# ATTron/astroz

Hardware: AMD Instinct MI355X
Metric: propagations/sec, 13,478 sats x 1,440 times, at 1/2/4/8 MI355X (higher is better)
Workload: dtype f64

## Files before the change

astroz_amd/_native.py:

```python
import ctypes as C
import os

import numpy as np

_HERE = os.path.dirname(os.path.abspath(__file__))
LIB_PATH = os.environ.get("ASTROZ_AMD_LIB") or os.path.join(_HERE, "libastroz_hip.so")

WGS84, WGS72 = 0, 1
OUT_TEME, OUT_ECEF, OUT_GEODETIC, OUT_TOPOCENTRIC = 0, 1, 2, 3
SAT_MAJOR, TIME_MAJOR = 0, 1
OUTPUT_MODES = {"teme": OUT_TEME, "ecef": OUT_ECEF, "geodetic": OUT_GEODETIC, "topocentric": OUT_TOPOCENTRIC}
PASS_DTYPE = np.dtype([("t_rise_min", "<f8"), ("t_culm_min", "<f8"), ("t_set_min", "<f8"), ("max_elevation_rad", "<f8"),
                       ("rise_azimuth_rad", "<f8"), ("set_azimuth_rad", "<f8"), ("flags", "<u4"), ("grid_rise", "<u4"),
                       ("grid_culm", "<u4"), ("grid_set", "<u4")])
PASS_UP_AT_START, PASS_UP_AT_END, PASS_CUT_BY_ERROR = 1, 2, 4
ECLIPSE_DTYPE = np.dtype([("t_entry_min", "<f8"), ("t_exit_min", "<f8"), ("flags", "<u4"), ("grid_entry", "<u4"),
                          ("grid_exit", "<u4"), ("reserved", "<u4")])
ECLIPSE_IN_AT_START, ECLIPSE_IN_AT_END, ECLIPSE_CUT_BY_ERROR = 1, 2, 4
SHADOW_UMBRA, SHADOW_PENUMBRA = 0, 1
SHADOW_KINDS = {"umbra": SHADOW_UMBRA, "penumbra": SHADOW_PENUMBRA}
ACCESS_DTYPE = np.dtype([("t_start_min", "<f8"), ("t_end_min", "<f8"), ("min_range_km", "<f8"), ("flags", "<u4"),
                         ("grid_start", "<u4"), ("grid_end", "<u4"), ("grid_min_range", "<u4")])
ACCESS_OPEN_AT_START, ACCESS_OPEN_AT_END, ACCESS_CUT_BY_ERROR = 1, 2, 4
CONJUNCTION_DTYPE = np.dtype([("t_tca_min", "<f8"), ("miss_km", "<f8"), ("rel_speed_km_s", "<f8"), ("target", "<u4"),
                              ("sat", "<u4"), ("grid_index", "<u4"), ("reserved", "<u4")])

COVERAGE_DTYPE = np.dtype([("mean_in_view", "<f8"), ("max_gap_min", "<f8"), ("n_covered", "<u4"), ("min_in_view", "<u4"),
                           ("max_in_view", "<u4"), ("n_gaps", "<u4"), ("grid_gap_start", "<u4"), ("grid_gap_end", "<u4"),
                           ("flags", "<u4"), ("reserved", "<u4")])
COVERAGE_GAP_AT_START, COVERAGE_GAP_AT_END = 1, 2

AZ_ERR_HIP = -200
PATH_ROWS_FAST, PATH_TILES_FAST, PATH_ROWS_GENERIC, PATH_LANE_SAT, PATH_DEEP_ROWS, PATH_QUASI_UNIFORM, PATH_COLS_FAST, PATH_HOST_STEP = 1, 2, 4, 8, 16, 32, 64, 128

EXPORTS = [
    "astroz_version", "astroz_init", "astroz_deinit", "tle_parse", "tle_free",
    "tle_get_satellite_number", "tle_get_epoch", "tle_get_inclination", "tle_get_eccentricity",
    "tle_get_mean_motion", "sgp4_init", "sgp4_free", "sgp4_propagate", "sgp4_propagate_batch",
    "azh_device_count", "azh_last_error", "azh_parse_tle_lines", "azh_constellation_from_tle_text",
    "azh_constellation_from_tle_lines", "azh_constellation_from_elements", "azh_constellation_subset", "azh_constellation_free",
    "azh_num_satellites", "azh_num_sgp4", "azh_num_sdp4", "azh_get_epochs", "azh_get_status",
    "azh_get_field", "azh_propagate_host", "azh_propagate_device", "azh_propagate_device_cached", "azh_propagate_device_window",
    "azh_propagate_jd_host", "azh_synchronize", "azh_propagate_one_host", "azh_set_time_tile", "azh_set_timing", "azh_set_fast_path", "azh_set_tile_kernel", "azh_set_graphs", "azh_set_f32_arithmetic", "azh_set_f32_mode",
    "azh_last_kernel_ms", "azh_last_path", "azh_last_one_stats", "azh_set_host_copy_threads", "azh_set_host_points", "azh_get_host_points", "azh_selftest_coords", "azh_selftest_host_step", "azh_host_alloc", "azh_host_free", "azh_host_pool_stats", "azh_host_pool_trim", "azh_propagate_device_f32", "azh_propagate_device_cached_f32",
    "azh_screen_target_host", "azh_screen_target_device", "azh_coarse_screen_device", "azh_coarse_screen_host",
    "azh_screen_all_host", "azh_constellation_from_omm_json", "azh_propagate_one_device", "azh_selftest_math",
    "azh_parse_tle_text", "azh_parse_omm_json", "azh_set_parse_threads", "coords_julian_to_gmst",
    "azh_group_create_from_tle_text", "azh_group_create_from_omm_json", "azh_group_free", "azh_group_num_satellites",
    "azh_group_num_devices", "azh_group_padded_rows", "azh_group_get_epochs", "azh_group_propagate_host",
    "azh_group_propagate_allgather", "azh_group_screen_target_host", "azh_group_screen_target_device", "azh_group_shard_size",
    "azh_group_shard_rows", "azh_group_synchronize", "azh_screen_track_device", "coords_eci_to_ecef", "coords_ecef_to_geodetic",
    "orbital_hohmann", "orbital_velocity", "orbital_period", "orbital_escape_velocity",
    "azh_coords_topocentric", "azh_set_observer", "azh_find_passes_host", "azh_find_passes_device",
    "azh_find_passes_stations_host", "azh_find_passes_stations_device",
    "azh_coverage_host", "azh_coverage_device",
    "azh_sun_position_teme", "azh_selftest_sun", "azh_shadow_state", "azh_find_eclipses_host", "azh_find_eclipses_device",
    "azh_line_of_sight", "azh_find_access_host", "azh_find_access_device", "azh_find_access_track_device",
    "azh_closest_approach", "azh_find_conjunctions_host", "azh_find_conjunctions_device",
]


def _stations(stations, min_elevation_deg):
    st = np.ascontiguousarray(stations, dtype=np.float64).reshape(-1, 3)
    mk = np.ascontiguousarray(np.broadcast_to(np.asarray(min_elevation_deg, dtype=np.float64), (len(st),)))
    return st, mk


def _targets(targets):
    a = np.atleast_1d(np.asarray(targets))
    if a.ndim != 1 or a.size == 0 or a.dtype == np.bool_ or not np.issubdtype(a.dtype, np.integer) or (a < 0).any():
        raise ValueError("targets must be a satellite index or a non-empty sequence of them")
    return np.ascontiguousarray(a, dtype=np.uintp)


def _min_satellites(k):
    if isinstance(k, bool) or not isinstance(k, (int, np.integer)) or not 1 <= int(k) <= 0xFFFFFFFF:
        raise ValueError("min_satellites must be an integer >= 1")
    return int(k)


class NativeError(RuntimeError):
    def __init__(self, code, what):
        self.code = code
        super().__init__("%s failed with code %d%s" % (what, code, _detail(code)))


_lib = None


def _detail(code):
    if _lib is not None and code == AZ_ERR_HIP:
        msg = _lib.azh_last_error().decode(errors="replace")
        return " (%s)" % msg if msg else " (HIP runtime error: is an MI355X visible?)"
    return ""


def _share_hip_runtime_with_torch():
    if os.environ.get("ASTROZ_AMD_SYSTEM_HIP"):
        return
    import importlib.util
    try:
        spec = importlib.util.find_spec("torch")
    except (ImportError, ValueError):
        spec = None
    if spec is None or not spec.origin:
        return
    cand = os.path.join(os.path.dirname(spec.origin), "lib", "libamdhip64.so")
    if os.path.exists(cand):
        C.CDLL(cand, mode=C.RTLD_GLOBAL)


def lib():
    global _lib
    if _lib is not None:
        return _lib
    if not os.path.exists(LIB_PATH):
        raise ImportError(
            "astroz_amd: %s not found -- build it with `python -c 'import __graft_entry__ as g; "
            "g.build()'` (hipcc --offload-arch=gfx950). There is no CPU fallback." % LIB_PATH)
    _share_hip_runtime_with_torch()
    L = C.CDLL(LIB_PATH)
    vp, sz, dbl, i32, u32 = C.c_void_p, C.c_size_t, C.c_double, C.c_int32, C.c_uint32
    L.astroz_version.restype = u32
    L.tle_parse.argtypes = [C.c_char_p, C.POINTER(vp)]
    L.tle_parse.restype = i32
    L.tle_free.argtypes = [vp]
    L.tle_get_satellite_number.argtypes = [vp]
    L.tle_get_satellite_number.restype = u32
    for f in ("tle_get_epoch", "tle_get_inclination", "tle_get_eccentricity", "tle_get_mean_motion"):
        getattr(L, f).argtypes = [vp]
        getattr(L, f).restype = dbl
    L.sgp4_init.argtypes = [vp, i32, C.POINTER(vp)]
    L.sgp4_init.restype = i32
    L.sgp4_free.argtypes = [vp]
    L.sgp4_propagate.argtypes = [vp, dbl, vp, vp]
    L.sgp4_propagate.restype = i32
    L.sgp4_propagate_batch.argtypes = [vp, vp, vp, u32]
    L.sgp4_propagate_batch.restype = i32
    L.azh_device_count.restype = C.c_int
    L.azh_last_error.restype = C.c_char_p
    L.azh_parse_tle_lines.argtypes = [C.c_char_p, C.c_char_p, vp]
    L.azh_parse_tle_lines.restype = i32
    L.azh_constellation_from_tle_text.argtypes = [C.c_char_p, sz, i32, i32, C.POINTER(vp)]
    L.azh_constellation_from_tle_text.restype = i32
    for f in ("azh_parse_tle_text", "azh_parse_omm_json"):
        getattr(L, f).argtypes = [C.c_char_p, sz, vp, sz, C.POINTER(sz)]
        getattr(L, f).restype = i32
    L.azh_set_parse_threads.argtypes = [i32]
    L.azh_set_parse_threads.restype = None
    for f in ("azh_group_create_from_tle_text", "azh_group_create_from_omm_json"):
        getattr(L, f).argtypes = [C.c_char_p, sz, i32, vp, i32, i32, C.POINTER(vp)]
        getattr(L, f).restype = i32
    L.azh_group_free.argtypes = [vp]
    L.azh_group_num_satellites.argtypes = [vp]
    L.azh_group_num_satellites.restype = sz
    L.azh_group_num_devices.argtypes = [vp]
    L.azh_group_num_devices.restype = i32
    L.azh_group_padded_rows.argtypes = [vp]
    L.azh_group_padded_rows.restype = sz
    L.azh_group_get_epochs.argtypes = [vp, vp]
    L.azh_group_get_epochs.restype = i32
    L.azh_group_propagate_host.argtypes = [vp, vp, sz, vp, sz, vp, vp, i32, dbl, vp]
    L.azh_group_propagate_host.restype = i32
    L.azh_group_propagate_allgather.argtypes = [vp, vp, sz, vp, sz, vp, vp]
    L.azh_group_propagate_allgather.restype = i32
    L.azh_group_screen_target_host.argtypes = [vp, vp, sz, vp, sz, sz, dbl, dbl, vp, vp]
    L.azh_group_screen_target_host.restype = i32
    L.azh_group_screen_target_device.argtypes = [vp, vp, sz, vp, sz, sz, dbl, dbl, vp, vp]
    L.azh_group_screen_target_device.restype = i32
    L.azh_group_shard_size.argtypes = [vp, i32]
    L.azh_group_shard_size.restype = sz
    L.azh_group_shard_rows.argtypes = [vp, i32, vp]
    L.azh_group_shard_rows.restype = i32
    L.azh_group_synchronize.argtypes = [vp]
    L.azh_group_synchronize.restype = i32
    L.azh_constellation_from_omm_json.argtypes = [C.c_char_p, sz, i32, i32, C.POINTER(vp)]
    L.azh_constellation_from_omm_json.restype = i32
    L.azh_propagate_one_device.argtypes = [vp, sz, vp, sz, vp, vp, vp, vp]
    L.azh_propagate_one_device.restype = i32
    L.azh_selftest_math.argtypes = [vp, sz, vp, i32]
    L.azh_selftest_math.restype = i32
    L.coords_julian_to_gmst.argtypes = [dbl]
    L.coords_julian_to_gmst.restype = dbl
    L.coords_eci_to_ecef.argtypes = [vp, dbl, vp]
    L.coords_eci_to_ecef.restype = None
    L.coords_ecef_to_geodetic.argtypes = [vp, vp]
    L.coords_ecef_to_geodetic.restype = None
    L.azh_constellation_from_tle_lines.argtypes = [vp, vp, sz, i32, i32, C.POINTER(vp)]
    L.azh_constellation_from_tle_lines.restype = i32
    L.azh_constellation_from_elements.argtypes = [sz] + [vp] * 8 + [i32, i32, C.POINTER(vp)]
    L.azh_constellation_from_elements.restype = i32
    L.azh_constellation_subset.argtypes = [vp, vp, sz, i32, C.POINTER(vp)]
    L.azh_constellation_subset.restype = i32
    L.azh_constellation_free.argtypes = [vp]
    for f in ("azh_num_satellites", "azh_num_sgp4", "azh_num_sdp4"):
        getattr(L, f).argtypes = [vp]
        getattr(L, f).restype = sz
    L.azh_get_epochs.argtypes = [vp, vp]
    L.azh_get_epochs.restype = i32
    L.azh_get_status.argtypes = [vp, vp, vp, vp]
    L.azh_get_status.restype = i32
    L.azh_get_field.argtypes = [vp, C.c_char_p, vp]
    L.azh_get_field.restype = i32
    L.azh_propagate_host.argtypes = [vp, vp, sz, vp, vp, vp, i32, dbl, vp, i32, sz, vp]
    L.azh_propagate_host.restype = i32
    L.azh_propagate_device.argtypes = [vp, vp, sz, vp, vp, vp, i32, dbl, vp, i32, sz, vp, vp]
    L.azh_propagate_device.restype = i32
    L.azh_propagate_device_cached.argtypes = [vp, vp, vp, i32, sz, vp, vp]
    L.azh_propagate_device_cached.restype = i32
    L.azh_propagate_device_window.argtypes = [vp, sz, sz, vp, vp, i32, sz, vp, vp]
    L.azh_propagate_device_window.restype = i32
    L.azh_propagate_jd_host.argtypes = [vp, vp, vp, sz, vp, vp, i32, i32, vp]
    L.azh_propagate_jd_host.restype = i32
    L.azh_synchronize.argtypes = [vp]
    L.azh_synchronize.restype = i32
    L.azh_propagate_one_host.argtypes = [vp, sz, vp, sz, vp, vp, vp]
    L.azh_propagate_one_host.restype = i32
    L.azh_set_time_tile.argtypes = [vp, u32, u32]
    L.azh_set_time_tile.restype = i32
    L.azh_set_timing.argtypes = [vp, i32]
    L.azh_set_timing.restype = i32
    L.azh_set_fast_path.argtypes = [vp, i32]
    L.azh_set_fast_path.restype = i32
    L.azh_set_tile_kernel.argtypes = [vp, i32]
    L.azh_set_tile_kernel.restype = i32
    L.azh_set_graphs.argtypes = [vp, i32]
    L.azh_set_graphs.restype = i32
    L.azh_set_f32_arithmetic.argtypes = [vp, i32]
    L.azh_set_f32_arithmetic.restype = i32
    L.azh_set_f32_mode.argtypes = [vp, i32]
    L.azh_set_f32_mode.restype = i32
    L.azh_last_kernel_ms.argtypes = [vp]
    L.azh_last_kernel_ms.restype = dbl
    L.azh_set_host_copy_threads.argtypes = [i32]
    L.azh_set_host_copy_threads.restype = None
    L.azh_set_host_points.argtypes = [sz]
    L.azh_set_host_points.restype = None
    L.azh_get_host_points.argtypes = []
    L.azh_get_host_points.restype = sz
    L.azh_host_alloc.argtypes = [C.c_size_t, C.POINTER(C.c_void_p)]
    L.azh_host_alloc.restype = i32
    L.azh_host_free.argtypes = [C.c_void_p]
    L.azh_host_free.restype = None
    L.azh_host_pool_stats.argtypes = [C.POINTER(C.c_size_t), C.POINTER(C.c_size_t)]
    L.azh_host_pool_stats.restype = None
    L.azh_host_pool_trim.argtypes = []
    L.azh_host_pool_trim.restype = None
    L.azh_last_path.argtypes = [vp]
    L.azh_last_path.restype = u32
    L.azh_last_one_stats.argtypes = [vp, vp, vp]
    L.azh_last_one_stats.restype = C.c_int32
    L.azh_propagate_device_f32.argtypes = L.azh_propagate_device.argtypes
    L.azh_propagate_device_f32.restype = i32
    L.azh_propagate_device_cached_f32.argtypes = L.azh_propagate_device_cached.argtypes
    L.azh_propagate_device_cached_f32.restype = i32
    L.azh_screen_target_host.argtypes = [vp, vp, sz, vp, sz, dbl, dbl, vp, vp]
    L.azh_screen_target_host.restype = i32
    L.azh_screen_target_device.argtypes = [vp, vp, sz, vp, sz, dbl, dbl, vp, vp, vp]
    L.azh_screen_target_device.restype = i32
    L.azh_screen_track_device.argtypes = [vp, vp, sz, vp, vp, sz, dbl, vp, vp, vp]
    L.azh_screen_track_device.restype = i32
    L.azh_coarse_screen_device.argtypes = [vp, sz, sz, i32, sz, dbl, vp, vp, vp, sz, C.POINTER(sz), vp]
    L.azh_coarse_screen_device.restype = i32
    L.azh_coarse_screen_host.argtypes = [vp, sz, sz, i32, sz, dbl, vp, vp, vp, sz, C.POINTER(sz), i32]
    L.azh_coarse_screen_host.restype = i32
    L.azh_screen_all_host.argtypes = [vp, vp, sz, vp, dbl, vp, vp, sz, C.POINTER(sz)]
    L.azh_screen_all_host.restype = i32
    L.azh_coords_topocentric.argtypes = [vp, vp, dbl, vp, vp, vp]
    L.azh_coords_topocentric.restype = None
    L.azh_set_observer.argtypes = [vp, dbl, dbl, dbl]
    L.azh_set_observer.restype = i32
    L.azh_find_passes_host.argtypes = [vp, vp, sz, vp, dbl, dbl, vp, sz, vp]
    L.azh_find_passes_host.restype = i32
    L.azh_find_passes_device.argtypes = [vp, vp, sz, vp, dbl, dbl, vp, sz, vp, vp]
    L.azh_find_passes_device.restype = i32
    L.azh_find_passes_stations_host.argtypes = [vp, vp, sz, vp, dbl, vp, vp, sz, vp, sz, vp]
    L.azh_find_passes_stations_host.restype = i32
    L.azh_find_passes_stations_device.argtypes = [vp, vp, sz, vp, dbl, vp, vp, sz, vp, sz, vp, vp]
    L.azh_find_passes_stations_device.restype = i32
    L.azh_coverage_host.argtypes = [vp, vp, sz, vp, dbl, vp, vp, sz, u32, vp, vp]
    L.azh_coverage_host.restype = i32
    L.azh_coverage_device.argtypes = [vp, vp, sz, vp, dbl, vp, vp, sz, u32, vp, vp, vp]
    L.azh_coverage_device.restype = i32
    L.azh_sun_position_teme.argtypes = [dbl, vp]
    L.azh_sun_position_teme.restype = None
    L.azh_selftest_sun.argtypes = [vp, sz, vp, i32]
    L.azh_selftest_sun.restype = i32
    L.azh_shadow_state.argtypes = [vp, vp, vp, vp]
    L.azh_shadow_state.restype = i32
    L.azh_find_eclipses_host.argtypes = [vp, vp, sz, vp, dbl, i32, vp, sz, vp, vp]
    L.azh_find_eclipses_host.restype = i32
    L.azh_find_eclipses_device.argtypes = [vp, vp, sz, vp, dbl, i32, vp, sz, vp, vp, vp]
    L.azh_find_eclipses_device.restype = i32
    L.azh_line_of_sight.argtypes = [vp, vp, dbl, vp, vp]
    L.azh_line_of_sight.restype = i32
    L.azh_find_access_host.argtypes = [vp, vp, sz, vp, sz, dbl, dbl, vp, sz, vp, vp]
    L.azh_find_access_host.restype = i32
    L.azh_find_access_device.argtypes = [vp, vp, sz, vp, sz, dbl, dbl, vp, sz, vp, vp, vp]
    L.azh_find_access_device.restype = i32
    L.azh_find_access_track_device.argtypes = [vp, vp, sz, vp, vp, vp, sz, dbl, dbl, vp, sz, vp, vp, vp]
    L.azh_find_access_track_device.restype = i32
    L.azh_closest_approach.argtypes = [vp, vp, vp, vp, dbl, vp, vp, vp]
    L.azh_closest_approach.restype = i32
    L.azh_find_conjunctions_host.argtypes = [vp, vp, sz, vp, vp, sz, dbl, vp, sz, vp]
    L.azh_find_conjunctions_host.restype = i32
    L.azh_find_conjunctions_device.argtypes = [vp, vp, sz, vp, vp, sz, dbl, vp, sz, vp, vp]
    L.azh_find_conjunctions_device.restype = i32
    L.orbital_hohmann.argtypes = [dbl, dbl, dbl, vp]
    L.orbital_hohmann.restype = i32
    for f, n in (("orbital_velocity", 3), ("orbital_period", 2), ("orbital_escape_velocity", 2)):
        getattr(L, f).argtypes = [dbl] * n
        getattr(L, f).restype = dbl
    _lib = L
    return L


def check(code, what):
    if code != 0:
        raise NativeError(code, what)


def _f64(a):
    return np.ascontiguousarray(a, dtype=np.float64)


def _ptr(a):
    return None if a is None else a.ctypes.data


class DeviceConstellation:

    def __init__(self, handle):
        self._h = handle
        L = lib()
        self.n = L.azh_num_satellites(handle)
        self.n_sgp4 = L.azh_num_sgp4(handle)
        self.n_sdp4 = L.azh_num_sdp4(handle)
        self._epochs = None
        self._status = None

    @classmethod
    def from_tle_text(cls, text, grav=WGS72, device=0):
        b = text.encode() if isinstance(text, str) else bytes(text)
        h = C.c_void_p()
        check(lib().azh_constellation_from_tle_text(b, len(b), grav, device, C.byref(h)),
              "azh_constellation_from_tle_text")
        return cls(h)

    @classmethod
    def from_omm_json(cls, text, grav=WGS72, device=0):
        b = text.encode() if isinstance(text, str) else bytes(text)
        h = C.c_void_p()
        check(lib().azh_constellation_from_omm_json(b, len(b), grav, device, C.byref(h)),
              "azh_constellation_from_omm_json")
        return cls(h)

    @classmethod
    def from_tle_lines(cls, pairs, grav=WGS72, device=0):
        n = len(pairs)
        a1 = (C.c_char_p * n)(*[p[0].encode() for p in pairs])
        a2 = (C.c_char_p * n)(*[p[1].encode() for p in pairs])
        h = C.c_void_p()
        check(lib().azh_constellation_from_tle_lines(a1, a2, n, grav, device, C.byref(h)),
              "azh_constellation_from_tle_lines")
        return cls(h)

    @classmethod
    def from_elements(cls, epoch_jd, mm_revday, ecc, incl_deg, raan_deg, argp_deg, ma_deg, bstar,
                      grav=WGS72, device=0):
        cols = [_f64(x) for x in (epoch_jd, mm_revday, ecc, incl_deg, raan_deg, argp_deg, ma_deg, bstar)]
        n = len(cols[0])
        assert all(len(c) == n for c in cols)
        h = C.c_void_p()
        check(lib().azh_constellation_from_elements(n, *[c.ctypes.data for c in cols], grav, device,
                                                    C.byref(h)), "azh_constellation_from_elements")
        return cls(h)

    def subset(self, indices, device=-1):
        idx = np.ascontiguousarray(indices, dtype=np.uint32)
        h = C.c_void_p()
        check(lib().azh_constellation_subset(self._h, idx.ctypes.data, len(idx), device, C.byref(h)),
              "azh_constellation_subset")
        return type(self)(h)

    def handle_address(self):
        return int(self._h.value)

    def close(self):
        if getattr(self, "_h", None):
            lib().azh_constellation_free(self._h)
            self._h = None

    def __del__(self):
        try:
            self.close()
        except Exception:
            pass

    @property
    def epochs(self):
        if self._epochs is None:
            e = np.empty(self.n, dtype=np.float64)
# ... 132 lines not shown
                                                    stream), "azh_find_passes_stations_device")

    def coverage(self, times_min, offsets_min, points, min_elevation_deg, *, reference_jd=0.0, min_satellites=1, counts=False):
        times = _f64(times_min)
        off = None if offsets_min is None else _f64(offsets_min)
        if off is not None and len(off) < self.n:
            raise ValueError("epoch_offsets must have at least num_satellites elements")
        pt, mk = _stations(points, min_elevation_deg)
        stats = np.zeros(len(pt), dtype=COVERAGE_DTYPE)
        cnt = np.zeros((len(pt), len(times)), dtype=np.uint32) if counts else None
        check(lib().azh_coverage_host(self._h, times.ctypes.data, len(times), _ptr(off), float(reference_jd), pt.ctypes.data,
                                      mk.ctypes.data, len(pt), _min_satellites(min_satellites), stats.ctypes.data,
                                      None if cnt is None else cnt.ctypes.data), "azh_coverage_host")
        return (stats, cnt) if counts else stats

    def coverage_device(self, times_min, offsets_min, points, min_elevation_deg, d_stats, d_counts=None, *, reference_jd=0.0,
                        min_satellites=1, stream=None):
        times = _f64(times_min)
        off = None if offsets_min is None else _f64(offsets_min)
        if off is not None and len(off) < self.n:
            raise ValueError("epoch_offsets must have at least num_satellites elements")
        pt, mk = _stations(points, min_elevation_deg)
        check(lib().azh_coverage_device(self._h, times.ctypes.data, len(times), _ptr(off), float(reference_jd), pt.ctypes.data,
                                        mk.ctypes.data, len(pt), _min_satellites(min_satellites), d_stats, d_counts, stream),
              "azh_coverage_device")

    def find_eclipses(self, times_min, offsets_min=None, *, reference_jd, kind=SHADOW_UMBRA, max_eclipses=32, state=False):
        times = _f64(times_min)
        off = None if offsets_min is None else _f64(offsets_min)
        if off is not None and len(off) < self.n:
            raise ValueError("epoch_offsets must have at least num_satellites elements")
        out = np.zeros((self.n, int(max_eclipses)), dtype=ECLIPSE_DTYPE)
        cnt = np.zeros(self.n, dtype=np.uint32)
        st = np.zeros((self.n, len(times)), dtype=np.uint8) if state else None
        check(lib().azh_find_eclipses_host(self._h, times.ctypes.data, len(times), _ptr(off), float(reference_jd), int(kind),
                                           out.ctypes.data if max_eclipses else None, int(max_eclipses), cnt.ctypes.data,
                                           st.ctypes.data if state and st.size else None), "azh_find_eclipses_host")
        return (out, cnt, st) if state else (out, cnt)

    def find_eclipses_device(self, times_min, offsets_min, d_out, max_eclipses, d_n_eclipses, *, reference_jd, kind=SHADOW_UMBRA,
                             d_state=None, stream=None):
        times = _f64(times_min)
        off = None if offsets_min is None else _f64(offsets_min)
        check(lib().azh_find_eclipses_device(self._h, times.ctypes.data, len(times), _ptr(off), float(reference_jd), int(kind),
                                             d_out, int(max_eclipses), d_n_eclipses, d_state, stream), "azh_find_eclipses_device")

    def find_access(self, times_min, target, offsets_min=None, *, grazing_alt_km=0.0, max_range_km=None, max_windows=32,
                    state=False):
        times = _f64(times_min)
        off = None if offsets_min is None else _f64(offsets_min)
        if off is not None and len(off) < self.n:
            raise ValueError("epoch_offsets must have at least num_satellites elements")
        out = np.zeros((self.n, int(max_windows)), dtype=ACCESS_DTYPE)
        cnt = np.zeros(self.n, dtype=np.uint32)
        st = np.zeros((self.n, len(times)), dtype=np.uint8) if state else None
        check(lib().azh_find_access_host(self._h, times.ctypes.data, len(times), _ptr(off), int(target), float(grazing_alt_km),
                                         _max_range(max_range_km), out.ctypes.data if max_windows else None, int(max_windows),
                                         cnt.ctypes.data, st.ctypes.data if state and st.size else None), "azh_find_access_host")
        return (out, cnt, st) if state else (out, cnt)

    def find_access_device(self, times_min, target, offsets_min, d_out, max_windows, d_n_windows, *, grazing_alt_km=0.0,
                           max_range_km=None, d_state=None, stream=None):
        times = _f64(times_min)
        off = None if offsets_min is None else _f64(offsets_min)
        check(lib().azh_find_access_device(self._h, times.ctypes.data, len(times), _ptr(off), int(target), float(grazing_alt_km),
                                           _max_range(max_range_km), d_out, int(max_windows), d_n_windows, d_state, stream),
              "azh_find_access_device")

    def find_access_track_device(self, times_min, d_track_pos, d_track_vel, offsets_min, d_out, max_windows, d_n_windows, *,
                                 exclude=None, grazing_alt_km=0.0, max_range_km=None, d_state=None, stream=None):
        times = _f64(times_min)
        off = None if offsets_min is None else _f64(offsets_min)
        ex = C.c_size_t(-1).value if exclude is None else int(exclude)
        check(lib().azh_find_access_track_device(self._h, times.ctypes.data, len(times), _ptr(off), d_track_pos, d_track_vel, ex,
                                                 float(grazing_alt_km), _max_range(max_range_km), d_out, int(max_windows),
                                                 d_n_windows, d_state, stream), "azh_find_access_track_device")

    def find_conjunctions(self, times_min, targets, threshold_km, offsets_min=None, *, max_events=65536):
        times = _f64(times_min)
        off = None if offsets_min is None else _f64(offsets_min)
        if off is not None and len(off) < self.n:
            raise ValueError("epoch_offsets must have at least num_satellites elements")
        tg = _targets(targets)
        out = np.zeros(int(max_events), dtype=CONJUNCTION_DTYPE)
        cnt = np.zeros(1, dtype=np.uint32)
        check(lib().azh_find_conjunctions_host(self._h, times.ctypes.data, len(times), _ptr(off), tg.ctypes.data, len(tg),
                                               float(threshold_km), out.ctypes.data if max_events else None, int(max_events),
                                               cnt.ctypes.data), "azh_find_conjunctions_host")
        return out[:min(int(cnt[0]), int(max_events))], int(cnt[0])

    def find_conjunctions_device(self, times_min, targets, threshold_km, offsets_min, d_out, max_events, d_n_events, *, stream=None):
        times = _f64(times_min)
        off = None if offsets_min is None else _f64(offsets_min)
        tg = _targets(targets)
        check(lib().azh_find_conjunctions_device(self._h, times.ctypes.data, len(times), _ptr(off), tg.ctypes.data, len(tg),
                                                 float(threshold_km), d_out, int(max_events), d_n_events, stream),
              "azh_find_conjunctions_device")

    def screen_all(self, times_min, threshold=10.0, offsets_min=None, max_results=10_000_000):
        times = _f64(times_min)
        off = None if offsets_min is None else _f64(offsets_min)
        pairs = np.empty((max_results, 2), dtype=np.uint32)
        tt = np.empty(max_results, dtype=np.uint32)
        k = C.c_size_t(0)
        check(lib().azh_screen_all_host(self._h, times.ctypes.data, len(times), _ptr(off), float(threshold),
                                        pairs.ctypes.data, tt.ctypes.data, max_results, C.byref(k)),
              "azh_screen_all_host")
        return pairs[:k.value].copy(), tt[:k.value].copy()

    def propagate_one(self, sat_index, tsince_min):
        t = _f64(np.atleast_1d(tsince_min))
        n = len(t)
        pos = result_empty((n, 3))
        vel = result_empty((n, 3))
        err = result_empty((n,), np.uint8)
        check(lib().azh_propagate_one_host(self._h, sat_index, t.ctypes.data, n, pos.ctypes.data, vel.ctypes.data,
                                           err.ctypes.data), "azh_propagate_one_host")
        return err, pos, vel

    def propagate_one_device(self, sat_index, d_tsince, n, d_pos, d_vel=None, d_err=None, stream=None):
        check(lib().azh_propagate_one_device(self._h, sat_index, d_tsince, n, d_pos, d_vel, d_err, stream),
              "azh_propagate_one_device")

    F32_MODES = {"mixed": 0, "packed": 1, "fp64": 2}

    def set_f32_arithmetic(self, mode):
        if isinstance(mode, (bool, np.bool_)):
            check(lib().azh_set_f32_arithmetic(self._h, 1 if mode else 0), "azh_set_f32_arithmetic")
            return
        m = self.F32_MODES[mode] if isinstance(mode, str) else int(mode)
        check(lib().azh_set_f32_mode(self._h, m), "azh_set_f32_mode")

    def set_fast_path(self, enabled):
        check(lib().azh_set_fast_path(self._h, 1 if enabled else 0), "azh_set_fast_path")

    def set_tile_kernel(self, enabled):
        check(lib().azh_set_tile_kernel(self._h, int(enabled) if not isinstance(enabled, bool) else (1 if enabled else 0)), "azh_set_tile_kernel")

    def set_graphs(self, enabled):
        check(lib().azh_set_graphs(self._h, 1 if enabled else 0), "azh_set_graphs")

    def set_timing(self, enabled):
        check(lib().azh_set_timing(self._h, 1 if enabled else 0), "azh_set_timing")

    def synchronize(self):
        check(lib().azh_synchronize(self._h), "azh_synchronize")

    def last_kernel_ms(self):
        return lib().azh_last_kernel_ms(self._h)

    def last_path(self):
        return int(lib().azh_last_path(self._h))

    def last_one_stats(self):
        a, b = C.c_uint32(0), C.c_uint32(0)
        check(lib().azh_last_one_stats(self._h, C.byref(a), C.byref(b)), "azh_last_one_stats")
        return int(a.value), int(b.value)


class DeviceGroup:

    def __init__(self, text, devices, grav=WGS72, n_chunks=4):
        b = text.encode() if isinstance(text, str) else bytes(text)
        dv = (C.c_int32 * len(devices))(*devices)
        h = C.c_void_p()
        fn = lib().azh_group_create_from_omm_json if b.lstrip()[:1] in (b"{", b"[") else lib().azh_group_create_from_tle_text
        check(fn(b, len(b), grav, dv, len(devices), n_chunks, C.byref(h)), "azh_group_create")
        self._h = h
        self.n = lib().azh_group_num_satellites(h)
        self.n_devices = lib().azh_group_num_devices(h)
        self.padded_rows = lib().azh_group_padded_rows(h)
        self.epochs = np.empty(self.n)
        check(lib().azh_group_get_epochs(h, self.epochs.ctypes.data), "azh_group_get_epochs")

    def close(self):
        if getattr(self, "_h", None):
            lib().azh_group_free(self._h)
            self._h = None

    def __del__(self):
        try:
            self.close()
        except Exception:
            pass

    def _offsets(self, offsets_min):
        if offsets_min is None:
            return None
        off = _f64(offsets_min)
        if off.ndim != 1 or len(off) < self.n:
            raise ValueError("epoch_offsets must have at least num_satellites elements")
        return off

    def propagate_host(self, times_min, offsets_min=None, *, velocities=True, mode=OUT_TEME, reference_jd=0.0, errors=False):
        t = _f64(times_min)
        off = self._offsets(offsets_min)
        pos = result_empty((self.n, len(t), 3))
        vel = result_empty((self.n, len(t), 3)) if velocities else None
        big = self.n * len(t) >= PINNED_MIN_BYTES
        err = (result_empty((self.n, len(t)), np.uint8) if big else np.zeros((self.n, len(t)), dtype=np.uint8)) if errors else None
        check(lib().azh_group_propagate_host(self._h, t.ctypes.data, len(t), _ptr(off), 0 if off is None else len(off), pos.ctypes.data, _ptr(vel), mode,
                                             float(reference_jd), _ptr(err)), "azh_group_propagate_host")
        return pos, vel, err

    def screen_target(self, times_min, target, threshold_km, offsets_min=None, reference_jd=0.0):
        t = _f64(times_min)
        off = self._offsets(offsets_min)
        d = np.empty(self.n)
        ti = np.empty(self.n, dtype=np.uint32)
        check(lib().azh_group_screen_target_host(self._h, t.ctypes.data, len(t), _ptr(off), 0 if off is None else len(off), int(target),
                                                 float(threshold_km), float(reference_jd), d.ctypes.data, ti.ctypes.data),
              "azh_group_screen_target_host")
        return d, ti

    def screen_target_device(self, times_min, target, threshold_km, d_dist_ptrs, d_t_ptrs, offsets_min=None):
        t = _f64(times_min)
        off = self._offsets(offsets_min)
        dd = (C.c_void_p * self.n_devices)(*d_dist_ptrs)
        tt = (C.c_void_p * self.n_devices)(*d_t_ptrs)
        check(lib().azh_group_screen_target_device(self._h, t.ctypes.data, len(t), _ptr(off), 0 if off is None else len(off), int(target),
                                                   float(threshold_km), 0.0, dd, tt), "azh_group_screen_target_device")

    def shard_size(self, slot):
        return int(lib().azh_group_shard_size(self._h, int(slot)))

    def shard_rows(self, slot):
        out = np.empty(self.shard_size(slot), dtype=np.uint32)
        check(lib().azh_group_shard_rows(self._h, int(slot), out.ctypes.data), "azh_group_shard_rows")
        return out

    def synchronize(self):
        check(lib().azh_group_synchronize(self._h), "azh_group_synchronize")

    def propagate_allgather(self, times_min, offsets_min, d_pos_ptrs, d_vel_ptrs=None):
        t = _f64(times_min)
        off = self._offsets(offsets_min)
        pp = (C.c_void_p * self.n_devices)(*d_pos_ptrs)
        vv = (C.c_void_p * self.n_devices)(*d_vel_ptrs) if d_vel_ptrs is not None else None
        check(lib().azh_group_propagate_allgather(self._h, t.ctypes.data, len(t), _ptr(off), 0 if off is None else len(off), pp, vv),
              "azh_group_propagate_allgather")


class _PinnedBlock:
    __slots__ = ("ptr", "_free", "__weakref__")

    def __init__(self, nbytes):
        self.ptr = None
        q = C.c_void_p(0)
        check(lib().azh_host_alloc(int(nbytes), C.byref(q)), "azh_host_alloc")
        self.ptr, self._free = q.value, lib().azh_host_free

    def __del__(self):
        if self.ptr:
            self._free(self.ptr)
            self.ptr = None


_PINNED_RESULTS = True
PINNED_MIN_BYTES = 8 << 20
_PINNED_LIVE_BUDGET = int(os.environ.get("ASTROZ_AMD_PINNED_LIVE_MB", "8192")) << 20


def set_pinned_budget(nbytes):
    global _PINNED_LIVE_BUDGET
    _PINNED_LIVE_BUDGET = max(0, int(nbytes))


def set_pinned_results(enabled):
    global _PINNED_RESULTS
    _PINNED_RESULTS = bool(enabled)


def result_empty(shape, dtype=np.float64, pinned=None):
    n = 1
    for d in shape:
        n *= int(d)
    if n * 8 < PINNED_MIN_BYTES and dtype is np.float64:
        return np.empty(shape)
    dt = np.dtype(dtype)
    nbytes = n * dt.itemsize
    use = _PINNED_RESULTS if pinned is None else pinned
    if not use or nbytes < PINNED_MIN_BYTES:
        return np.empty(shape, dtype=dt)
    if host_pool_stats()[0] + nbytes > _PINNED_LIVE_BUDGET:
        return np.empty(shape, dtype=dt)
    try:
        blk = _PinnedBlock(nbytes)
    except NativeError:
        return np.empty(shape, dtype=dt)
    buf = (C.c_char * nbytes).from_address(blk.ptr)
    buf._az_owner = blk
    return np.frombuffer(buf, dtype=dt).reshape(shape)


_fast_mod = False


def fast_scalar():
    global _fast_mod
    if _fast_mod is False:
        try:
            from . import _azfast
            _azfast.bind(C.cast(lib().azh_propagate_one_host, C.c_void_p).value)
            _fast_mod = _azfast
        except Exception:
            _fast_mod = None
# ... 156 lines not shown
```

astroz_amd/csrc/astroz_hip.hip:

```cpp
#include "../../include/astroz_hip.h"

#include <hip/hip_runtime.h>
#include <dlfcn.h>
#include <rccl/rccl.h>

#include <algorithm>
#include <atomic>
#include <cmath>
#include <condition_variable>
#include <deque>
#include <map>
#include <cstdio>
#include <cstdlib>
#include <cstring>
#include <mutex>
#include <new>
#include <memory>
#include <string>
#include <thread>
#include <type_traits>
#include <vector>

#include "kernels.h"
#include "passes_kernel.h"
// ... 20 lines not shown
}
#define HIP_TRY(expr)                                                                                       \
    do {                                                                                                    \
        if (!hip_ok((expr), #expr)) return AZ_ERR_HIP;                                                      \
    } while (0)

AzGrav make_grav(int which)
{
    AzGrav g;
    if (which == AZ_WGS72) {
        g.radius_km = 6378.135;
        g.j2 = 0.001082616;
        g.j4 = -0.00000165597;
        g.xke = 0.0743669161331734132;
        g.j3oj2 = -0.00234506972242078;
    } else {
        g.radius_km = 6378.137;
        g.j2 = 0.00108262998905;
        g.j4 = -0.00000161098761;
        g.xke = 0.07436685316871385;
        g.j3oj2 = -0.00233899967218727;
    }
    g.vkmpersec = g.xke * g.radius_km / 60.0;
    g.half_j2 = 0.5 * g.j2;
    return g;
}

const char *const kFieldNames[] = {
#define X(n) #n,
    AZ_SGP4_FIELDS(X) AZ_DEEP_FIELDS(X)
#undef X
};


template <class T>
struct DevBuf {
    T *p = nullptr;
    size_t cap = 0;
    DevBuf() = default;
    DevBuf(DevBuf &&o) noexcept { swap(o); }
    DevBuf &operator=(DevBuf &&o) noexcept { swap(o); return *this; }
    ~DevBuf() { if (p) (void)hipFree(p); }
    void swap(DevBuf &o) noexcept { std::swap(p, o.p); std::swap(cap, o.cap); }
    int ensure(size_t n)
    {
        if (n <= cap) return AZ_OK;
        if (p) (void)hipFree(p);
        p = nullptr;
        cap = 0;
        size_t want = std::max<size_t>(n, 64);
        if (!hip_ok(hipMalloc((void **)&p, want * sizeof(T)), "hipMalloc")) return AZ_ERR_HIP;
        cap = want;
        return AZ_OK;
    }
};

struct PinnedBuf {
    void *p = nullptr;
    size_t cap = 0;
    PinnedBuf() = default;
    PinnedBuf(PinnedBuf &&o) noexcept { swap(o); }
    PinnedBuf &operator=(PinnedBuf &&o) noexcept { swap(o); return *this; }
    ~PinnedBuf() { if (p) (void)hipHostFree(p); }
    void swap(PinnedBuf &o) noexcept { std::swap(p, o.p); std::swap(cap, o.cap); }
    int32_t ensure(size_t bytes)
    {
        if (bytes <= cap) return AZ_OK;
        size_t want = std::max<size_t>(cap, 65536);
        while (want < bytes) want *= 2;
        if (p) (void)hipHostFree(p);
        p = nullptr;
        cap = 0;
        if (!hip_ok(hipHostMalloc(&p, want, hipHostMallocDefault), "hipHostMalloc")) return AZ_ERR_HIP;
        cap = want;
        return AZ_OK;
    }
};

template <class H, hipError_t (*Create)(H *, unsigned), hipError_t (*Destroy)(H)>
class HipHandle {
  public:
    HipHandle() = default;
    HipHandle(HipHandle &&o) noexcept { swap(o); }
    HipHandle &operator=(HipHandle &&o) noexcept { swap(o); return *this; }
    ~HipHandle() { reset(); }
    void swap(HipHandle &o) noexcept { std::swap(h_, o.h_); std::swap(own_, o.own_); }
    hipError_t create(unsigned flags)
    {
        reset();
        own_ = true;
        return Create(&h_, flags);
    }
    void borrow(H h)
    {
        reset();
        h_ = h;
        own_ = false;
    }
    void reset()
    {
        if (h_ && own_) (void)Destroy(h_);
        h_ = nullptr;
    }
    bool owned() const { return h_ && own_; }
    operator H() const { return h_; }

  private:
    H h_ = nullptr;
    bool own_ = false;
};
using Stream = HipHandle<hipStream_t, hipStreamCreateWithFlags, hipStreamDestroy>;
using Event = HipHandle<hipEvent_t, hipEventCreateWithFlags, hipEventDestroy>;

constexpr int kStageSlots = 3;
constexpr size_t kStageChunk = size_t(16) << 20;
struct HostStager {
    Event ev[kStageSlots];
    PinnedBuf slot[kStageSlots];
    int32_t ensure()
    {
        for (int k = 0; k < kStageSlots; ++k) {
            if (slot[k].ensure(kStageChunk) != AZ_OK) return AZ_ERR_HIP;
            if (!ev[k] && !hip_ok(ev[k].create(hipEventDisableTiming), "hipEventCreate")) return AZ_ERR_HIP;
        }
        return AZ_OK;
    }
};
}

struct azh_constellation {
    int device = 0;
    size_t n = 0, n_pad = 0;
    AzGrav g{};
    Stream s_main, s_deep, s_ecc;
    Event ev_fork, ev_join, ev_fork2, ev_join2, ev_t0, ev_t1;
    Event ev_one;
    Event ev_graph;
    DevBuf<double> d_el;
    DevBuf<unsigned> d_flags;
    std::vector<unsigned> h_flags;
    std::vector<double> h_epoch;
    std::vector<double> h_raw[AZ_NUM_RAW];
    DevBuf<unsigned> d_list;
    std::vector<unsigned> h_list;
    unsigned n_sgp4 = 0, n_sdp4 = 0, n_bad = 0;
    DevBuf<double> d_times, d_offsets, d_sin, d_cos, d_seeds;
    DevBuf<double> d_node_cache;
    struct FastPlan {
        bool valid = false, mixed32 = false;
        unsigned tile_c = 0, tile_e = 0, n_list = 0, n_seg = 0, parity = 0;
        DevBuf<double> win;
        DevBuf<unsigned char> flag;
        DevBuf<unsigned> redo;
    } plan[4];
    DevBuf<double> d_inc;
    DevBuf<double> d_fast_rec;
    double uniform_step = 0.0;
    DevBuf<float> d_delta;
    double delta_max = 0.0;
    std::vector<float> h_delta;
    DevBuf<double> d_delta64;
    std::vector<double> h_delta64;
    bool delta_wide = false;
    double grid_t0 = 0.0;
    unsigned last_path = 0;
    DevBuf<double> d_tgt, d_part_d2, d_out_d;
    DevBuf<unsigned> d_part_t, d_out_t;
    DevBuf<double> d_one_t, d_one_o;
    DevBuf<unsigned char> d_one_e;
    DevBuf<unsigned> d_one_items;
    unsigned one_segments = 0;
    PinnedBuf h_stage;
    std::vector<double> h_times, h_offsets;
    std::vector<uint8_t> h_mask;
    double staged_ref_jd = 0.0;
    hipStream_t staged_stream = nullptr;
    bool staged_valid = false;
    PinnedBuf h_small;
    HostStager stager;
    bool seeds_valid = false;
    unsigned seeds_tile = 0;
    bool seeds_rows = false;
    DevBuf<unsigned char> d_mask;
    DevBuf<double> d_host_pos, d_host_vel;
    DevBuf<unsigned char> d_host_err;
    bool have_offsets = false, have_mask = false;
    AzObserver obs{};
    DevBuf<AzObserver> d_obs;
    bool have_observer = false, obs_dirty = false;
    DevBuf<double> d_pass_pos, d_pass_vel;
    DevBuf<unsigned char> d_pass_err;
    DevBuf<azh_pass> d_pass_out;
    DevBuf<uint32_t> d_pass_n;
    std::vector<AzStation> h_stations;
    DevBuf<AzStation> d_stations;
    DevBuf<azh_coverage> d_cov_stats;
    DevBuf<uint32_t> d_cov_counts;
    DevBuf<AzSunPoint> d_sun;
    DevBuf<azh_eclipse> d_ecl_out;
    DevBuf<unsigned char> d_ecl_state;
    DevBuf<double> d_acc_track;
    DevBuf<azh_access> d_acc_out;
    DevBuf<unsigned char> d_acc_state;
    DevBuf<double> d_conj_track;
    std::vector<unsigned> h_conj_slots;
    DevBuf<unsigned> d_conj_slots;
    DevBuf<azh_conjunction> d_conj_out;
    unsigned cached_n_times = 0;
    int cached_mode = 0;
    unsigned off_cat = 0;
    unsigned off_deep_cat = 0;
    unsigned off_rowmap = 0;
    unsigned off_rowmap2 = 0;
    struct LaunchGraph {
        const void *pos, *vel, *err;
        int layout, f32;
        size_t stride, row_lo, row_hi;
        hipStream_t st;
        unsigned sig_before, sig_after;
        unsigned path;
        unsigned seen;
        unsigned fails;
        hipGraph_t graph;
        hipGraphExec_t exec;
    };
    std::vector<LaunchGraph> graphs;
    int graphs_on = 0;
    bool capturing = false;
    int cols_kernel = 0;
    DevBuf<double> d_deep_tmp;
    bool tile_kernel = true;
    unsigned off_circ = 0, n_circ = 0;
    bool timed = false;
    bool timing = true;
    unsigned tile_sgp4 = 0, tile_sdp4 = 0;
    int f32_mode = 0;
    bool fast_path = true;
    std::vector<double> h_el;
    std::vector<std::pair<size_t, std::vector<double>>> h_cols;
    size_t h_cols_next = 0;
    ~azh_constellation();
};

namespace {

constexpr size_t kHostMirrorPad = 64;
constexpr size_t kHostCols = 256;
constexpr size_t kHostColsBeforeTable = 8;
constexpr size_t kHostTableMax = size_t(64) << 20;
std::atomic<size_t> g_host_points{[] {
    const char *e = getenv("ASTROZ_AMD_HOST_POINTS");
    return e ? (size_t)strtoull(e, nullptr, 10) : size_t(128);
}()};
inline size_t host_points() { return azhost::cpu_ok() ? g_host_points.load(std::memory_order_relaxed) : 0; }

constexpr int32_t AZ_RC_EAGER = 0x7a5eca9;
int set_device(const azh_constellation *c) { return hip_ok(hipSetDevice(c->device), "hipSetDevice") ? AZ_OK : AZ_ERR_HIP; }

hipStream_t small_stream(int device)
{
    static std::mutex mu;
    static std::map<int, hipStream_t> streams;
    std::lock_guard<std::mutex> lk(mu);
    auto it = streams.find(device);
    if (it != streams.end()) return it->second;
    hipStream_t s = nullptr;
    if (!hip_ok(hipStreamCreateWithFlags(&s, hipStreamNonBlocking), "hipStreamCreate")) return nullptr;
    streams[device] = s;
    return s;
}

void drop_graphs(azh_constellation *c);

int32_t build(const std::vector<double> (&cols)[AZ_NUM_RAW], size_t n, int grav, int device, azh_constellation **out)
{
    if (!out) return AZ_ERR_NULL_POINTER;
    *out = nullptr;
    if (n == 0) return AZ_ERR_VALUE;
    if (n > 0x7fffffffu) return AZ_ERR_VALUE;
    int ndev = 0;
    HIP_TRY(hipGetDeviceCount(&ndev));
    if (device < 0 || device >= ndev) {
        g_last_error = "no such HIP device";
        return AZ_ERR_HIP;
    }
    std::unique_ptr<azh_constellation> c(new (std::nothrow) azh_constellation());
    if (!c) return AZ_ERR_ALLOC_FAILED;
    c->device = device;
    c->n = n;
    c->n_pad = (n + 63) / 64 * 64;
    c->g = make_grav(grav);
    if (set_device(c.get()) != AZ_OK) return AZ_ERR_HIP;
    if (n > 16) {
        if (!hip_ok(c->s_main.create(hipStreamNonBlocking), "hipStreamCreate") ||
            !hip_ok(c->s_deep.create(hipStreamNonBlocking), "hipStreamCreate") ||
            !hip_ok(c->s_ecc.create(hipStreamNonBlocking), "hipStreamCreate") ||
            !hip_ok(c->ev_graph.create(hipEventDisableTiming | hipEventDisableSystemFence), "hipEventCreate"))
            return AZ_ERR_HIP;
    } else {
        c->s_main.borrow(small_stream(device));
        if (!c->s_main) return AZ_ERR_HIP;
        c->s_deep.borrow(c->s_main);
        c->s_ecc.borrow(c->s_main);
    }
    for (Event *e : {&c->ev_fork2, &c->ev_join2, &c->ev_fork, &c->ev_join, &c->ev_one})
        if (!hip_ok(e->create(hipEventDisableTiming), "hipEventCreate")) return AZ_ERR_HIP;
    if (!hip_ok(c->ev_t0.create(hipEventDefault), "hipEventCreate") || !hip_ok(c->ev_t1.create(hipEventDefault), "hipEventCreate"))
        return AZ_ERR_HIP;
    const size_t np = c->n_pad;
    DevBuf<double> d_raw;
    if (c->d_el.ensure((size_t)AZ_NUM_FIELDS * np) != AZ_OK || c->d_flags.ensure(np) != AZ_OK || d_raw.ensure((size_t)AZ_NUM_RAW * np) != AZ_OK)
        return AZ_ERR_HIP;
    std::vector<double> staging((size_t)AZ_NUM_RAW * np, 0.0);
    for (int k = 0; k < AZ_NUM_RAW; ++k) memcpy(&staging[(size_t)k * np], cols[k].data(), sizeof(double) * n);
    if (!hip_ok(hipMemcpyAsync(d_raw.p, staging.data(), sizeof(double) * staging.size(), hipMemcpyHostToDevice, c->s_main), "H2D raw") ||
        !hip_ok(hipMemsetAsync(c->d_el.p, 0, sizeof(double) * AZ_NUM_FIELDS * np, c->s_main), "memset el") ||
        !hip_ok(hipMemsetAsync(c->d_flags.p, 0, sizeof(unsigned) * np, c->s_main), "memset flags"))
        return AZ_ERR_HIP;
    hipLaunchKernelGGL(k_init, dim3((unsigned)(np / 64)), dim3(64), 0, c->s_main, d_raw.p, n, np, c->g, c->d_el.p, c->d_flags.p);
    if (!hip_ok(hipGetLastError(), "k_init launch")) return AZ_ERR_HIP;
    c->h_flags.resize(n);
    if (np <= kHostMirrorPad) {
        c->h_el.resize((size_t)AZ_NUM_FIELDS * np);
        if (!hip_ok(hipMemcpyAsync(c->h_el.data(), c->d_el.p, sizeof(double) * c->h_el.size(), hipMemcpyDeviceToHost, c->s_main), "D2H el"))
            return AZ_ERR_HIP;
    }
    if (!hip_ok(hipMemcpyAsync(c->h_flags.data(), c->d_flags.p, sizeof(unsigned) * n, hipMemcpyDeviceToHost, c->s_main), "D2H flags") ||
        !hip_ok(hipStreamSynchronize(c->s_main), "sync(init)"))
        return AZ_ERR_HIP;
    c->h_epoch = cols[R_epoch_jd];
    for (int k = 0; k < AZ_NUM_RAW; ++k) c->h_raw[k] = cols[k];
    std::vector<unsigned> list;
    list.reserve(n);
    for (size_t s = 0; s < n; ++s)
        if (AZ_FLAG_ERR(c->h_flags[s]) == 0 && !(c->h_flags[s] & AZ_FLAG_DEEP)) list.push_back((unsigned)s);
    c->n_sgp4 = (unsigned)list.size();
    for (size_t g0 = 0; g0 < list.size(); g0 += AZ_BLOCK) {
        const size_t g1 = std::min(g0 + (size_t)AZ_BLOCK, list.size());
        std::stable_sort(list.begin() + g0, list.begin() + g1, [&](unsigned x, unsigned y) {
            return AZ_FLAG_ECLASS(c->h_flags[x]) < AZ_FLAG_ECLASS(c->h_flags[y]);
        });
    }
    {
        std::vector<unsigned> deep;
        for (size_t s = 0; s < n; ++s)
            if (AZ_FLAG_ERR(c->h_flags[s]) == 0 && (c->h_flags[s] & AZ_FLAG_DEEP)) deep.push_back((unsigned)s);
        const std::vector<double> &incl = cols[R_incl_deg];
        auto key = [&](unsigned s) {
            const unsigned f = c->h_flags[s];
            const unsigned low = incl[s] < 12.5 ? 1u : 0u;
            return (AZ_FLAG_IREZ(f) << 4) | (low << 2) | AZ_FLAG_ECLASS(f);
        };
        std::stable_sort(deep.begin(), deep.end(), [&](unsigned x, unsigned y) { return key(x) < key(y); });
        list.insert(list.end(), deep.begin(), deep.end());
    }
    c->n_sdp4 = (unsigned)list.size() - c->n_sgp4;
    for (size_t s = 0; s < n; ++s)
        if (AZ_FLAG_ERR(c->h_flags[s]) != 0) list.push_back((unsigned)s);
    c->n_bad = (unsigned)list.size() - c->n_sgp4 - c->n_sdp4;
    c->off_circ = (unsigned)list.size();
    for (size_t s = 0; s < n; ++s)
        if (AZ_FLAG_ERR(c->h_flags[s]) == 0 && !(c->h_flags[s] & AZ_FLAG_DEEP) && AZ_FLAG_ECLASS(c->h_flags[s]) == 0)
            list.push_back((unsigned)s);
    c->n_circ = (unsigned)list.size() - c->off_circ;
    for (size_t s = 0; s < n; ++s)
        if (AZ_FLAG_ERR(c->h_flags[s]) == 0 && !(c->h_flags[s] & AZ_FLAG_DEEP) && AZ_FLAG_ECLASS(c->h_flags[s]) != 0)
            list.push_back((unsigned)s);
    c->off_cat = (unsigned)list.size();
    for (size_t s = 0; s < n; ++s)
        if (AZ_FLAG_ERR(c->h_flags[s]) == 0 && !(c->h_flags[s] & AZ_FLAG_DEEP)) list.push_back((unsigned)s);
    c->off_deep_cat = (unsigned)list.size();
    for (size_t s = 0; s < n; ++s)
        if (AZ_FLAG_ERR(c->h_flags[s]) == 0 && (c->h_flags[s] & AZ_FLAG_DEEP)) list.push_back((unsigned)s);
    c->off_rowmap = (unsigned)list.size();
    {
        unsigned near = 0, deepn = 0;
        for (size_t s = 0; s < n; ++s) {
            const unsigned f = c->h_flags[s];
            if (AZ_FLAG_ERR(f) != 0) list.push_back((unsigned)AZ_ROW_ZERO << 30);
            else if (f & AZ_FLAG_DEEP) list.push_back(((unsigned)AZ_ROW_COPY << 30) | deepn++);
            else list.push_back(((unsigned)AZ_ROW_NEAR << 30) | near++);
        }
    }
    c->off_rowmap2 = (unsigned)list.size();
    {
        unsigned circ = 0, eccn = 0, deepn = 0;
        for (size_t s = 0; s < n; ++s) {
            const unsigned f = c->h_flags[s];
            if (AZ_FLAG_ERR(f) != 0) list.push_back((unsigned)AZ_ROW_ZERO << 30);
            else if (f & AZ_FLAG_DEEP) list.push_back(((unsigned)AZ_ROW_COPY << 30) | deepn++);
            else if (AZ_FLAG_ECLASS(f) == 0) list.push_back(((unsigned)AZ_ROW_NEAR << 30) | circ++);
            else list.push_back(((unsigned)AZ_ROW_NEAR << 30) | (c->n_circ + eccn++));
        }
    }
    if (const char *e = getenv("ASTROZ_AMD_COLS")) c->cols_kernel = atoi(e);
    if (const char *e = getenv("ASTROZ_AMD_GRAPHS")) c->graphs_on = atoi(e);
    c->h_list = list;
    if (c->d_list.ensure(list.size()) != AZ_OK ||
        !hip_ok(hipMemcpy(c->d_list.p, list.data(), sizeof(unsigned) * list.size(), hipMemcpyHostToDevice), "H2D list"))
        return AZ_ERR_HIP;
    *out = c.release();
    return AZ_OK;
}

int32_t build_from_records(const std::vector<azh::TleRecord> &recs, int grav, int device, azh_constellation **out)
{
    std::vector<double> cols[AZ_NUM_RAW];
    for (auto &v : cols) v.resize(recs.size());
    azh::parallel_ranges(recs.size(), azh::parse_threads_for(recs.size() * 140), [&](size_t a, size_t b) {
        for (size_t i = a; i < b; ++i) {
            const azh::TleRecord &r = recs[i];
            cols[R_epoch_jd][i] = r.epoch_jd;
            cols[R_mm_revday][i] = r.mm_revday;
            cols[R_ecc][i] = r.ecc;
            cols[R_incl_deg][i] = r.incl_deg;
            cols[R_raan_deg][i] = r.raan_deg;
            cols[R_argp_deg][i] = r.argp_deg;
            cols[R_ma_deg][i] = r.ma_deg;
            cols[R_bstar][i] = r.bstar;
        }
    });
    return build(cols, recs.size(), grav, device, out);
}

unsigned auto_tile(unsigned n_list, unsigned n_times, unsigned forced, unsigned min_tile)
{
    if (forced) return std::min(std::max(forced, 1u), std::max(n_times, 1u));
    const unsigned waves_x = (n_list + 63) / 64;
    unsigned n_tiles = (16384 + waves_x - 1) / std::max(waves_x, 1u);
    n_tiles = std::max(1u, std::min(n_tiles, n_times));
    unsigned tile = (n_times + n_tiles - 1) / n_tiles;
    tile = std::max(tile, std::min(min_tile, n_times));
    return std::max(tile, 1u);
}

inline unsigned pad8(unsigned n) { return (n + 7) / 8 * 8; }
inline unsigned cgrid_y(unsigned n_times, unsigned tile) { return (n_times + tile - 1) / tile; }

template <int V>
using int_c = std::integral_constant<int, V>;
template <class F>
void with_bool(bool b, F &&f)
{
    if (b) f(std::true_type{});
    else f(std::false_type{});
}
template <class F>
void with_vel_frame(bool vel, int mode, F &&f)
{
    const int frame = mode == AZ_OUT_TOPOCENTRIC ? 3 : (mode == AZ_OUT_GEODETIC ? 2 : (mode != AZ_OUT_TEME ? 1 : 0));
    with_bool(vel, [&](auto VEL) {
        if (frame == 3) f(VEL, int_c<3>{});
        else if (frame == 2) f(VEL, int_c<2>{});
        else if (frame == 1) f(VEL, int_c<1>{});
        else f(VEL, int_c<0>{});
    });
}
constexpr int gen_frame(int frame) { return frame == 3 ? 3 : (frame != 0 ? 1 : 0); }
template <class F>
void with_outputs(const PropArgs &a, bool vel, F &&f)
{
    if (a.screen_target) return f(std::false_type{}, int_c<0>{}, int_c<AZ_SINK_SCREEN>{});
    with_vel_frame(vel, a.mode, [&](auto VEL, auto FRAME) {
        if (a.f32) f(VEL, FRAME, int_c<AZ_SINK_F32>{});
        else f(VEL, FRAME, int_c<AZ_SINK_F64>{});
    });
}
template <class F>
void with_delta(int form, F &&f)
{
    if (form == 2) f(int_c<2>{});
    else if (form == 1) f(int_c<1>{});
    else f(int_c<0>{});
}

int32_t stream_after(hipStream_t to, hipStream_t from, hipEvent_t ev)
{
    HIP_TRY(hipEventRecord(ev, from));
    HIP_TRY(hipStreamWaitEvent(to, ev, 0));
    return AZ_OK;
}

unsigned rows_tile(unsigned n_list, unsigned n_times, unsigned forced)
{
    unsigned segs = std::max(1u, std::min((16384u + n_list - 1) / std::max(n_list, 1u), (n_times + 255) / 256));
    if (forced) segs = std::max(1u, (n_times + forced - 1) / forced);
    return ((n_times + segs - 1) / segs + 63) / 64 * 64;
}

bool use_rows(const PropArgs &a, int layout, bool deep)
{
    if (deep && layout == AZ_LAYOUT_TIME_MAJOR && a.n_times >= 32) return true;
    return (layout == AZ_LAYOUT_SAT_MAJOR || a.screen_target) && a.n_times >= 32;
}

unsigned screen_parts(const PropArgs &a, bool deep)
{
    if (use_rows(a, AZ_LAYOUT_SAT_MAJOR, deep)) {
        unsigned tile = rows_tile(a.n_list, a.n_times, a.tile_forced);
        if (deep) tile = std::min(tile, 64u * (unsigned)AZ_DEEP_SEED_MAX);
        return cgrid_y(a.n_times, tile);
    }
    return cgrid_y(a.n_times, a.tile);
}

struct EccSide {
    hipStream_t stream = nullptr;
    hipEvent_t fork = nullptr, join = nullptr;
};

struct FastShape {
    unsigned tile_c = 0, tile_e = 0;
    bool packed32 = false;
    bool mixed32 = false;
    int kind = 0;
};
unsigned fast_window_cap(double step)
{
    const double span = 3000.0 / std::max(std::fabs(step), 1e-9);
    return span >= 4.0e9 ? 0xffffffc0u : std::max(64u, (unsigned)span / 64u * 64u);
}
FastShape fast_shape_rows(const PropArgs &a, unsigned n_sgp4, unsigned n_circ)
{
    FastShape f;
    const unsigned cap = fast_window_cap(a.uniform_step);
    const unsigned n_ecc = n_sgp4 - n_circ;
    f.tile_c = std::min(rows_tile(n_sgp4, a.n_times, a.tile_forced), cap);
    f.tile_e = n_circ >= 4u * n_ecc ? f.tile_c : std::min(rows_tile(std::max(n_ecc, 1u), a.n_times, 256), cap);
    if (a.delta || a.delta64) {
        f.tile_c = std::min(f.tile_c, (unsigned)AZ_DELTA_SEG);
        f.tile_e = std::min(f.tile_e, (unsigned)AZ_DELTA_SEG);
    }
    f.packed32 = a.f32 && a.mode == AZ_OUT_TEME && a.arith32 != 2 && cap >= 128u && !a.delta_wide;
    f.mixed32 = f.packed32 && a.arith32 == 0;
    if (f.packed32) f.tile_c = std::max(128u, f.tile_c / 128u * 128u);
    f.kind = f.packed32 ? 1 : 0;
    return f;
}
FastShape fast_shape_tiles(const PropArgs &a, unsigned n_rows)
{
    FastShape f;
    unsigned tile = std::min(rows_tile(std::max((n_rows + 15u) / 16u, 1u) * 16u, a.n_times, a.tile_forced), fast_window_cap(a.uniform_step));
    if (a.mode != AZ_OUT_TEME) tile = std::min(tile, (unsigned)AZ_TILE_SEG_MAX);
    if (a.delta || a.delta64) tile = std::min(tile, (unsigned)AZ_DELTA_SEG);
    f.tile_c = f.tile_e = tile;
    f.kind = 2;
    return f;
}

template <bool VEL, int FRAME, int SINK, bool ECC>
void launch_rows_fast(const PropArgs &a, unsigned n_slots, hipStream_t st)
{
    with_delta(a.delta_wide ? 2 : (a.delta ? 1 : 0), [&](auto DELTA) {
        hipLaunchKernelGGL((k_rows_fast<VEL, FRAME, SINK, ECC, DELTA>), dim3(pad8(n_slots), cgrid_y(a.n_times, a.tile)), dim3(64), 0, st, a);
    });
}
PropArgs ecc_part(const PropArgs &a, unsigned tile)
{
    PropArgs e = a;
    e.list = a.list + a.n_circ;
    e.n_list = a.n_list - a.n_circ;
    e.tile = tile;
    e.redo_slot0 = a.n_circ;
    return e;
}
template <bool VEL, int FRAME, int SINK>
void launch_redo(const PropArgs &a, dim3 grid, hipStream_t st)
{
    hipLaunchKernelGGL((k_rows<VEL, gen_frame(FRAME), SINK, true>), grid, dim3(64), 0, st, a);
}

int32_t launch_near_fast(const PropArgs &a, bool vel, const FastShape &shape, dim3 rgrid, hipStream_t st, const EccSide &side)
{
    PropArgs e = ecc_part(a, shape.tile_e), c = a;
    c.n_list = a.n_circ;
    c.tile = shape.tile_c;
    unsigned n_e = e.n_list, n_c = c.n_list;
    if (a.row_lo > 0 || a.row_hi < a.n_rows) {
        c.slot_lo = a.win_circ_lo; c.slot_hi = a.win_circ_hi; n_c = c.slot_hi - c.slot_lo;
        e.slot_lo = a.win_ecc_lo; e.slot_hi = a.win_ecc_hi; n_e = e.slot_hi - e.slot_lo;
        if (c.slot_hi == 0) c.n_list = n_c = 0;
        if (e.slot_hi == 0) e.n_list = n_e = 0;
    }
    const bool beside = side.stream != nullptr && n_c;
    const hipStream_t se = beside ? side.stream : st;
    if (beside)
        if (int32_t rc = stream_after(se, st, side.fork); rc != AZ_OK) return rc;
    with_outputs(a, vel, [&](auto VEL, auto FRAME, auto SINK) {
        if (n_e) launch_rows_fast<VEL, FRAME, SINK, true>(e, n_e, se);
        launch_redo<VEL, FRAME, SINK>(a, rgrid, se);
        if (n_c && FRAME == 0 && shape.packed32)
            with_bool(shape.mixed32, [&](auto MIXED) {
                with_bool(a.delta != nullptr, [&](auto DELTA) {
                    hipLaunchKernelGGL((k_rows_fast32<VEL, MIXED, DELTA>), dim3(pad8(n_c), cgrid_y(a.n_times, c.tile)), dim3(64), 0, st, c);
                });
            });
        else if (n_c)
            launch_rows_fast<VEL, FRAME, SINK, false>(c, n_c, st);
    });
    return beside ? stream_after(st, se, side.join) : AZ_OK;
}

void launch_tiles(const PropArgs &a0, bool vel, hipStream_t st, const FastShape &shape)
{
    PropArgs a = a0, r = a0;
    a.tile = r.tile = shape.tile_c;
    r.tm_rows = 1;
    const dim3 grid(pad8((a.n_rows + 15u) / 16u), cgrid_y(a.n_times, a.tile));
    with_vel_frame(vel, a.mode, [&](auto VEL, auto FRAME) {
        with_bool(a.delta64 != nullptr, [&](auto WIDE) {
            hipLaunchKernelGGL((k_tiles_fast<VEL, FRAME, WIDE ? 2 : 0>), grid, dim3(1024), 0, st, a);
        });
        launch_redo<VEL, FRAME, AZ_SINK_F64>(r, dim3(256, 4), st);
    });
}
unsigned cols_tile(unsigned n_rows, unsigned n_times, unsigned forced, double step)
{
    const unsigned cap = fast_window_cap(step);
    if (forced) return std::min(std::max(forced, 1u), std::min(std::max(n_times, 1u), cap));
    const unsigned groups = (n_rows + 63u) / 64u, places = 1024u * (unsigned)AZ_COLS_WAVES;
    const unsigned segs = std::max(1u, places / std::max(groups, 1u));
    unsigned tile = (n_times + segs - 1u) / segs;
    if (tile < 32u) tile = std::min(128u, std::max(n_times, 1u));
    return std::max(1u, std::min(tile, cap));
}
FastShape fast_shape_cols(const PropArgs &a, unsigned n_rows, unsigned n_sgp4, unsigned n_circ)
{
    FastShape f = fast_shape_rows(a, n_sgp4, n_circ);
    f.tile_e = std::min(rows_tile(std::max(n_sgp4 - n_circ, 1u), a.n_times, a.tile_forced ? a.tile_forced : 256u), fast_window_cap(a.uniform_step));
    if (a.delta || a.delta64) f.tile_e = std::min(f.tile_e, (unsigned)AZ_DELTA_SEG);
    f.tile_c = cols_tile(n_rows, a.n_times, a.tile_forced, a.uniform_step);
    f.packed32 = f.mixed32 = false;
    f.kind = 3;
    return f;
}
int32_t launch_cols(const PropArgs &a0, bool vel, hipStream_t st, const FastShape &shape, const EccSide &side, unsigned ecc_row0)
{
    PropArgs a = a0;
    PropArgs e = ecc_part(a, shape.tile_e);
    e.pos = const_cast<double *>(a.tmp_pos);
    e.vel = vel ? const_cast<double *>(a.tmp_vel) : nullptr;
    e.rows_compact = 1;
    e.ecc_row0 = ecc_row0;
    if (e.n_list) {
        const hipStream_t se = side.stream ? side.stream : st;
        if (se != st)
            if (int32_t rc = stream_after(se, st, side.fork); rc != AZ_OK) return rc;
        with_vel_frame(vel, a.mode, [&](auto VEL, auto FRAME) { launch_rows_fast<VEL, FRAME, AZ_SINK_F64, true>(e, e.n_list, se); });
        if (se != st)
            if (int32_t rc = stream_after(st, se, side.join); rc != AZ_OK) return rc;
    }
    a.tile = shape.tile_c;
    a.ecc_row0 = ecc_row0;
    PropArgs r = a;
    r.tm_rows = 1;
    const dim3 grid(pad8((a.n_rows + 63u) / 64u), cgrid_y(a.n_times, a.tile));
    with_vel_frame(vel, a.mode, [&](auto VEL, auto FRAME) {
        with_bool(a.delta64 != nullptr, [&](auto WIDE) {
            hipLaunchKernelGGL((k_cols_fast<VEL, FRAME, WIDE ? 2 : 0>), grid, dim3(64), 0, st, a);
        });
        launch_redo<VEL, FRAME, AZ_SINK_F64>(r, dim3(256, 4), st);
    });
    return AZ_OK;
}

unsigned launch_propagate(const PropArgs &a, int layout, bool vel, bool deep, hipStream_t st)
{
    if (use_rows(a, layout, deep)) {
        PropArgs b = a;
        b.tile = rows_tile(a.n_list, a.n_times, a.tile_forced);
        if (deep) b.tile = std::min(b.tile, 64u * (unsigned)AZ_DEEP_SEED_MAX);
        const unsigned n_slots = a.slot_hi ? a.slot_hi - a.slot_lo : a.n_list;
        const dim3 grid(pad8(n_slots), cgrid_y(a.n_times, b.tile));
        with_outputs(a, vel, [&](auto VEL, auto FRAME, auto SINK) {
            if (deep) hipLaunchKernelGGL((k_rows_deep<VEL, gen_frame(FRAME), SINK>), grid, dim3(64), 0, st, b);
            else hipLaunchKernelGGL((k_rows<VEL, gen_frame(FRAME), SINK>), grid, dim3(64), 0, st, b);
        });
        return deep ? AZH_PATH_DEEP_ROWS : AZH_PATH_ROWS_GENERIC;
    }
    const dim3 grid(pad8((a.n_list + AZ_BLOCK - 1) / AZ_BLOCK), cgrid_y(a.n_times, a.tile));
    with_bool(deep, [&](auto DEEP) {
        if (a.screen_target)
            hipLaunchKernelGGL((k_propagate<0, false, DEEP, 0, true>), grid, dim3(AZ_BLOCK), 0, st, a);
        else
            with_bool(layout == AZ_LAYOUT_TIME_MAJOR, [&](auto TIME_MAJOR) {
                with_vel_frame(vel, a.mode, [&](auto VEL, auto FRAME) {
                    hipLaunchKernelGGL((k_propagate<TIME_MAJOR, VEL, DEEP, gen_frame(FRAME)>), grid, dim3(AZ_BLOCK), 0, st, a);
                });
            });
    });
    return AZH_PATH_LANE_SAT;
}

int32_t stage_inputs(azh_constellation *c, const double *times, size_t n_times, const double *offsets,
                     const uint8_t *mask, int mode, double reference_jd, hipStream_t st)
{
    if (n_times > 0xffffffffu) return AZ_ERR_VALUE;
    {
        const bool same = c->staged_valid && st == c->staged_stream && n_times == c->h_times.size() && mode == c->cached_mode &&
                          (mode == AZ_OUT_TEME || reference_jd == c->staged_ref_jd) &&
                          (offsets != nullptr) == c->have_offsets && (mask != nullptr) == c->have_mask &&
                          (n_times == 0 || memcmp(times, c->h_times.data(), sizeof(double) * n_times) == 0) &&
                          (!offsets || (c->h_offsets.size() == c->n && memcmp(offsets, c->h_offsets.data(), sizeof(double) * c->n) == 0)) &&
                          (!mask || (c->h_mask.size() == c->n && memcmp(mask, c->h_mask.data(), c->n) == 0));
        if (same) return AZ_OK;
        c->staged_valid = false;
    }
    if (c->d_times.ensure(n_times) != AZ_OK) return AZ_ERR_HIP;
    HIP_TRY(hipMemcpyAsync(c->d_times.p, times, sizeof(double) * n_times, hipMemcpyHostToDevice, st));
    c->have_offsets = offsets != nullptr;
    if (offsets) {
        if (c->d_offsets.ensure(c->n) != AZ_OK) return AZ_ERR_HIP;
        HIP_TRY(hipMemcpyAsync(c->d_offsets.p, offsets, sizeof(double) * c->n, hipMemcpyHostToDevice, st));
    }
    c->have_mask = mask != nullptr;
    if (mask) {
        if (c->d_mask.ensure(c->n) != AZ_OK) return AZ_ERR_HIP;
        HIP_TRY(hipMemcpyAsync(c->d_mask.p, mask, c->n, hipMemcpyHostToDevice, st));
    }
    if (mode != AZ_OUT_TEME) {
        if (c->d_sin.ensure(n_times) != AZ_OK || c->d_cos.ensure(n_times) != AZ_OK) return AZ_ERR_HIP;
        hipLaunchKernelGGL(k_gmst, dim3((unsigned)((n_times + 255) / 256)), dim3(256), 0, st, c->d_times.p,
                           (unsigned)n_times, reference_jd, c->d_sin.p, c->d_cos.p);
        HIP_TRY(hipGetLastError());
    }
    c->cached_n_times = (unsigned)n_times;
    c->cached_mode = mode;
    c->seeds_valid = false;
    drop_graphs(c);
    for (auto &pl : c->plan) pl.valid = false;
    c->uniform_step = 0.0;
    c->delta_max = 0.0;
    c->delta_wide = false;
    c->grid_t0 = n_times ? times[0] : 0.0;
    if (n_times >= 2) {
        double t0 = times[0], step = (times[n_times - 1] - t0) / (double)(n_times - 1);
        double tmax = std::max(std::fabs(t0), std::fabs(times[n_times - 1]));
        const double tol = 4.0 * 2.220446049250313e-16 * std::max(tmax, std::fabs(step));
        bool uni = std::isfinite(step) && step != 0.0;
        double dmax = 0.0;
        for (size_t i = 1; uni && i < n_times; ++i) {
            dmax = std::max(dmax, std::fabs(times[i] - std::fma((double)i, step, t0)));
            uni = dmax <= AZ_DELTA_MAX;
        }
        if (uni && dmax > tol) {
            c->h_delta.assign(n_times + AZ_DELTA_SEG, 0.0f);
            for (size_t i = 0; i < n_times; ++i) c->h_delta[i] = (float)(times[i] - std::fma((double)i, step, t0));
            if (c->d_delta.ensure(c->h_delta.size()) != AZ_OK) return AZ_ERR_HIP;
            HIP_TRY(hipMemcpyAsync(c->d_delta.p, c->h_delta.data(), sizeof(float) * c->h_delta.size(), hipMemcpyHostToDevice, st));
            c->h_delta64.assign(n_times + AZ_DELTA_SEG, 0.0);
            for (size_t i = 0; i < n_times; ++i) c->h_delta64[i] = times[i] - std::fma((double)i, step, t0);
            if (c->d_delta64.ensure(c->h_delta64.size()) != AZ_OK) return AZ_ERR_HIP;
            HIP_TRY(hipMemcpyAsync(c->d_delta64.p, c->h_delta64.data(), sizeof(double) * c->h_delta64.size(), hipMemcpyHostToDevice, st));
            c->delta_max = dmax * (1.0 + 1e-6) + 1e-12;
        }
        if (!uni && n_times >= 64) {
            const double nn = (double)n_times, im = 0.5 * (nn - 1.0);
            double tm = 0.0;
            for (size_t i = 0; i < n_times; ++i) tm += times[i];
            tm /= nn;
            double sxy = 0.0, sxx = 0.0;
            for (size_t i = 0; i < n_times; ++i) {
                sxy += ((double)i - im) * (times[i] - tm);
                sxx += ((double)i - im) * ((double)i - im);
            }
            step = sxy / sxx;
            t0 = tm - step * im;
            bool ok = std::isfinite(step) && std::isfinite(t0) && step != 0.0;
            dmax = 0.0;
            for (size_t i = 0; ok && i < n_times; ++i) {
                dmax = std::max(dmax, std::fabs(times[i] - std::fma((double)i, step, t0)));
                ok = dmax <= AZ_DELTA_WIDE_MAX;
            }
            if (ok && dmax <= 0.5 * std::fabs(step)) {
                c->h_delta64.assign(n_times + AZ_DELTA_SEG, 0.0);
                for (size_t i = 0; i < n_times; ++i) c->h_delta64[i] = times[i] - std::fma((double)i, step, t0);
                if (c->d_delta64.ensure(c->h_delta64.size()) != AZ_OK) return AZ_ERR_HIP;
                HIP_TRY(hipMemcpyAsync(c->d_delta64.p, c->h_delta64.data(), sizeof(double) * c->h_delta64.size(), hipMemcpyHostToDevice, st));
                c->delta_max = dmax * (1.0 + 1e-6) + 1e-12;
                c->delta_wide = true;
                c->grid_t0 = t0;
                uni = true;
            }
        }
        if (uni) {
            if (c->d_inc.ensure((size_t)2 * AZ_INC_NUM * c->n_pad) != AZ_OK) return AZ_ERR_HIP;
            hipLaunchKernelGGL(k_prep_inc, dim3((unsigned)((c->n + 255) / 256)), dim3(256), 0, st, c->d_el.p, c->n, c->n_pad,
                               step, c->d_inc.p);
            HIP_TRY(hipGetLastError());
            if (c->d_fast_rec.ensure((size_t)FR_NUM * c->n_pad) != AZ_OK) return AZ_ERR_HIP;
            hipLaunchKernelGGL(k_prep_rec, dim3((unsigned)((c->n + 255) / 256)), dim3(256), 0, st, c->d_el.p, c->d_flags.p, c->n, c->n_pad,
                               c->d_inc.p, c->d_fast_rec.p);
            HIP_TRY(hipGetLastError());
            c->uniform_step = step;
        }
    }
    try {
        c->h_times.assign(times, times + n_times);
        if (offsets) c->h_offsets.assign(offsets, offsets + c->n);
        if (mask) c->h_mask.assign(mask, mask + c->n);
        c->staged_ref_jd = reference_jd;
        c->staged_stream = st;
        c->staged_valid = true;
    } catch (const std::bad_alloc &) {
        c->staged_valid = false;
    }
    return AZ_OK;
}

int32_t prepare_deep(azh_constellation *c, PropArgs &d, hipStream_t st, bool rows, bool beside_bulk = false)
{
    const unsigned n_times = d.n_times;
    d.list = c->d_list.p + (rows ? c->off_deep_cat : c->n_sgp4);
    d.n_list = c->n_sdp4;
    d.tile = auto_tile(c->n_sdp4, n_times, c->tile_sdp4, 8);
    d.tile_forced = c->tile_sdp4 ? c->tile_sdp4 : (rows && beside_bulk && c->n_sgp4 >= 4u * c->n_sdp4 ? rows_tile(c->n_sgp4, n_times, c->tile_sgp4) : 0u);
    const unsigned seed_tile = rows ? 64u : d.tile;
    const unsigned n_tiles = (n_times + seed_tile - 1) / seed_tile;
    if (!c->seeds_valid || c->seeds_tile != seed_tile || c->seeds_rows != rows) {
        if (c->capturing) return AZ_RC_EAGER;
        drop_graphs(c);
        if (c->d_seeds.ensure((size_t)n_tiles * 3 * c->n_sdp4) != AZ_OK) return AZ_ERR_HIP;
        if (c->d_node_cache.p == nullptr) {
            if (c->d_node_cache.ensure(3 * c->n_pad) != AZ_OK) return AZ_ERR_HIP;
            HIP_TRY(hipMemsetAsync(c->d_node_cache.p, 0, sizeof(double) * 3 * c->n_pad, st));
        }
        hipLaunchKernelGGL(k_deep_seed, dim3((c->n_sdp4 + 63) / 64), dim3(64), 0, st, c->d_el.p, c->d_flags.p, c->n_pad,
                           d.list, c->n_sdp4, d.times, n_times, d.offsets, seed_tile, c->d_seeds.p, rows ? 1 : 0, c->d_node_cache.p);
        HIP_TRY(hipGetLastError());
        c->seeds_valid = true;
        c->seeds_tile = seed_tile;
        c->seeds_rows = rows;
    }
    d.seeds = c->d_seeds.p;
    return AZ_OK;
}

int32_t ensure_plan(azh_constellation *c, PropArgs &a, const FastShape &shape, hipStream_t st)
{
    azh_constellation::FastPlan &pl = c->plan[shape.kind];
    const unsigned n_list = a.n_list;
    const unsigned n_seg = (a.n_times + std::min(shape.tile_c, shape.tile_e) - 1) / std::min(shape.tile_c, shape.tile_e);
    if (!pl.valid || pl.tile_c != shape.tile_c || pl.tile_e != shape.tile_e || pl.n_list != n_list || pl.mixed32 != shape.mixed32) {
        if (c->capturing) return AZ_RC_EAGER;
        drop_graphs(c);
        const size_t items = (size_t)n_list * n_seg + ((size_t)a.n_times + 63) / 64 * (c->n_sgp4 - c->n_circ);
        if (pl.redo.cap < 4 + 3 * items || pl.win.cap < (size_t)n_list * n_seg * AZ_PLAN_NUM) HIP_TRY(hipStreamSynchronize(st));
        if (pl.redo.ensure(4 + 3 * items) != AZ_OK || pl.win.ensure((size_t)n_list * n_seg * AZ_PLAN_NUM) != AZ_OK ||
            pl.flag.ensure((size_t)n_list * n_seg) != AZ_OK)
            return AZ_ERR_HIP;
        HIP_TRY(hipMemsetAsync(pl.redo.p, 0, 4 * sizeof(unsigned), st));
        PlanArgs q{};
        q.el = a.el; q.flags = a.flags; q.n_pad = a.n_pad; q.list = a.list; q.n_list = n_list; q.n_circ = a.n_circ;
        q.n_times = a.n_times; q.tile_c = shape.tile_c; q.tile_e = shape.tile_e; q.by_flags = shape.kind == 2 ? 1u : 0u;
        q.times = a.times; q.offsets = a.offsets; q.inc = a.inc; q.step = a.uniform_step; q.dt_mult = shape.kind == 1 ? 128.0 : 64.0;
        q.delta_max = (a.delta || a.delta64) ? a.delta_max : 0.0;
        q.grid_t0 = a.grid_t0;
        q.f32_mixed = shape.mixed32 ? 1u : 0u;
        q.win = pl.win.p; q.flag = pl.flag.p;
        q.redo_static = pl.redo.p + 2; q.redo_c0 = pl.redo.p; q.redo_c1 = pl.redo.p + 1; q.redo_items = pl.redo.p + 4;
        q.g = a.g;
        hipLaunchKernelGGL(k_plan_windows, dim3((n_list + 255) / 256, n_seg), dim3(256), 0, st, q);
        hipLaunchKernelGGL(k_plan_arm, dim3(1), dim3(64), 0, st, q.redo_static, q.redo_c0, q.redo_c1);
        HIP_TRY(hipGetLastError());
        pl.valid = true;
        pl.tile_c = shape.tile_c; pl.tile_e = shape.tile_e; pl.n_list = n_list; pl.n_seg = n_seg; pl.parity = 0; pl.mixed32 = shape.mixed32;
    }
    a.plan_win = pl.win.p;
    a.plan_flag = pl.flag.p;
    a.plan_stride = n_list;
    a.redo_static = pl.redo.p + 2;
    a.redo_count = pl.redo.p + pl.parity;
    a.redo_next = pl.redo.p + (pl.parity ^ 1u);
    a.redo_items = pl.redo.p + 4;
    pl.parity ^= 1u;
    return AZ_OK;
}

void drop_graphs(azh_constellation *c)
{
    if (c->graphs.empty()) return;
    if (hipEventSynchronize(c->ev_graph) != hipSuccess) (void)hipGetLastError();
    for (auto &g : c->graphs) {
        if (g.exec) (void)hipGraphExecDestroy(g.exec);
        if (g.graph) (void)hipGraphDestroy(g.graph);
    }
    c->graphs.clear();
}
}

azh_constellation::~azh_constellation()
{
    (void)hipSetDevice(device);
    drop_graphs(this);
}

namespace {
unsigned plan_sig(const azh_constellation *c)
{
    unsigned s = 0;
    for (unsigned k = 0; k < 4; ++k) s |= (c->plan[k].parity & 1u) << k;
    return s;
}

int32_t launch_all(azh_constellation *c, double *d_pos, double *d_vel, int layout, size_t stride, uint8_t *d_err,
                   hipStream_t st, int f32 = 0, size_t row_lo = 0, size_t row_hi = ~(size_t)0)
{
    const unsigned n_times = c->cached_n_times;
    if (n_times == 0) return AZ_OK;
    row_hi = std::min(row_hi, c->n);
    if (row_lo >= row_hi) return AZ_OK;
    if (stride == 0) stride = c->n;
    if (layout == AZ_LAYOUT_TIME_MAJOR && stride < c->n) return AZ_ERR_VALUE;

    PropArgs a{};
    a.el = c->d_el.p;
    a.flags = c->d_flags.p;
    a.n_pad = c->n_pad;
    a.times = c->d_times.p;
    a.n_times = n_times;
    a.offsets = c->have_offsets ? c->d_offsets.p : nullptr;
    a.pos = d_pos;
    a.vel = d_vel;
    a.sin_g = c->d_sin.p;
    a.cos_g = c->d_cos.p;
    a.mask = c->have_mask ? c->d_mask.p : nullptr;
    a.err = d_err;
    a.stride_sats = stride;
    a.mode = c->cached_mode;
    if (a.mode == AZ_OUT_TOPOCENTRIC) {
        if (c->obs_dirty) {
            if (c->capturing) return AZ_RC_EAGER;
            if (c->d_obs.ensure(1) != AZ_OK) return AZ_ERR_HIP;
            HIP_TRY(hipMemcpyAsync(c->d_obs.p, &c->obs, sizeof(AzObserver), hipMemcpyHostToDevice, st));
            c->obs_dirty = false;
        }
        a.obs = c->d_obs.p;
    }
    a.f32 = f32;
    a.arith32 = f32 ? c->f32_mode : 2;
    a.g = c->g;
    a.uniform_step = c->fast_path ? c->uniform_step : 0.0;
    a.inc = (a.uniform_step != 0.0) ? c->d_inc.p : nullptr;
    a.fast_rec = (a.uniform_step != 0.0) ? c->d_fast_rec.p : nullptr;
    a.delta = (a.uniform_step != 0.0 && c->delta_max > 0.0 && !c->delta_wide) ? c->d_delta.p : nullptr;
    a.delta64 = (a.uniform_step != 0.0 && c->delta_max > 0.0) ? c->d_delta64.p : nullptr;
    a.delta_wide = c->delta_wide ? 1 : 0;
    a.grid_t0 = c->grid_t0;
    a.delta_max = c->delta_max;
    a.grid_exact_uniform = (c->uniform_step != 0.0 && c->delta_max == 0.0) ? 1 : 0;
    a.row_lo = (unsigned)row_lo;
    a.row_hi = (unsigned)row_hi;
    const bool windowed = row_lo > 0 || row_hi < c->n;
    auto slots_of = [&](unsigned off, unsigned cnt, unsigned &lo, unsigned &hi) {
        const unsigned *b = c->h_list.data() + off, *e = b + cnt;
        lo = (unsigned)(std::lower_bound(b, e, (unsigned)row_lo) - b);
        hi = (unsigned)(std::lower_bound(b, e, (unsigned)row_hi) - b);
    };
    unsigned deep_lo = 0, deep_hi = 0;
    if (windowed) {
        slots_of(c->off_circ, c->n_circ, a.win_circ_lo, a.win_circ_hi);
        slots_of(c->off_circ + c->n_circ, c->n_sgp4 - c->n_circ, a.win_ecc_lo, a.win_ecc_hi);
        slots_of(c->off_deep_cat, c->n_sdp4, deep_lo, deep_hi);
    }

    unsigned path = 0;
    if (c->timing) HIP_TRY(hipEventRecord(c->ev_t0, st));
    if (d_err) HIP_TRY(hipMemsetAsync(d_err + row_lo * (size_t)n_times, 0, (row_hi - row_lo) * (size_t)n_times, st));
    const bool tiles = c->n_sgp4 > 0 && c->tile_kernel && a.inc != nullptr && layout == AZ_LAYOUT_TIME_MAJOR && !f32 &&
                       n_times >= 64 &&
                       (size_t)stride * 64 * 24 < 0xf0000000ull;
    const bool cols = tiles && c->cols_kernel != 0 && a.mask == nullptr;
    const unsigned n_ecc = c->n_sgp4 - c->n_circ;
    const size_t scratch_rows = (size_t)c->n_sdp4 + (cols ? n_ecc : 0u);
    const size_t scratch_per = scratch_rows * n_times * 3, scratch_words = f32 ? (scratch_per + 1) / 2 : scratch_per;
    auto ensure_scratch = [&](hipStream_t user) -> int32_t {
        if (c->capturing && c->d_deep_tmp.cap < scratch_words * (d_vel ? 2 : 1)) return AZ_RC_EAGER;
        if (c->d_deep_tmp.cap < scratch_words * (d_vel ? 2 : 1)) {
            drop_graphs(c);
            HIP_TRY(hipStreamSynchronize(user));
        }
        if (c->d_deep_tmp.ensure(scratch_words * (d_vel ? 2 : 1)) != AZ_OK) return AZ_ERR_HIP;
        a.tmp_pos = c->d_deep_tmp.p;
        a.tmp_vel = d_vel ? c->d_deep_tmp.p + scratch_words : nullptr;
        return AZ_OK;
    };
    const bool fork = c->n_sdp4 > 0;
    if (cols && !fork && n_ecc)
        if (int32_t rc = ensure_scratch(st); rc != AZ_OK) return rc;
    if (fork) {
        if (int32_t rc = stream_after(c->s_deep, st, c->ev_fork); rc != AZ_OK) return rc;
        PropArgs d = a;
        const bool deep_rows = use_rows(d, layout, true);
        const bool deep_skip = windowed && deep_rows && deep_hi == deep_lo;
        if (windowed && deep_rows) { d.slot_lo = deep_lo; d.slot_hi = deep_hi; }
        if (int32_t rc = prepare_deep(c, d, c->s_deep, deep_rows, !tiles && a.inc != nullptr); rc != AZ_OK) return rc;
        if (deep_rows && layout == AZ_LAYOUT_TIME_MAJOR) {
            if (int32_t rc = ensure_scratch(c->s_deep); rc != AZ_OK) return rc;
            PropArgs t = d;
            t.pos = const_cast<double *>(a.tmp_pos);
            t.vel = const_cast<double *>(a.tmp_vel);
            t.rows_compact = 1;
            if (!deep_skip) path |= launch_propagate(t, AZ_LAYOUT_SAT_MAJOR, d_vel != nullptr, true, c->s_deep);
            HIP_TRY(hipGetLastError());
            dim3 tg((c->n_sdp4 + AZ_TR_ROWS - 1) / AZ_TR_ROWS, (n_times + 63) / 64);
            if (tiles || deep_skip) {  }
            else if (f32)
                hipLaunchKernelGGL((k_deep_transpose<float>), tg, dim3(192), 0, c->s_deep, reinterpret_cast<const float *>(t.pos),
                                   reinterpret_cast<const float *>(t.vel), reinterpret_cast<float *>(d_pos), reinterpret_cast<float *>(d_vel),
                                   d.list, c->n_sdp4, n_times, stride, d.mask, d.row_lo, d.row_hi);
            else
                hipLaunchKernelGGL((k_deep_transpose<double>), tg, dim3(192), 0, c->s_deep, t.pos, t.vel, d_pos, d_vel, d.list, c->n_sdp4,
                                   n_times, stride, d.mask, d.row_lo, d.row_hi);
        } else if (!deep_skip) {
            path |= launch_propagate(d, layout, d_vel != nullptr, true, c->s_deep);
        }
        HIP_TRY(hipGetLastError());
        HIP_TRY(hipEventRecord(c->ev_join, c->s_deep));
    }
    if (c->n_sgp4 > 0) {
        a.list = c->d_list.p;
        a.n_list = c->n_sgp4;
        a.tile = auto_tile(c->n_sgp4, n_times, c->tile_sgp4, 8);
        a.tile_forced = c->tile_sgp4;
        if (tiles && fork) HIP_TRY(hipStreamWaitEvent(st, c->ev_join, 0));
        if (tiles && !cols) a.list = c->d_list.p + c->off_cat;
        FastShape shape;
        const bool fast = a.inc != nullptr && (tiles || use_rows(a, layout, false));
        if (fast) {
            if (!tiles || cols) a.list = c->d_list.p + c->off_circ;
            a.n_list = c->n_sgp4;
            a.n_circ = c->n_circ;
            a.rowmap = c->d_list.p + (cols ? c->off_rowmap2 : c->off_rowmap);
            a.n_rows = (unsigned)c->n;
            shape = cols ? fast_shape_cols(a, (unsigned)c->n, c->n_sgp4, c->n_circ)
                         : (tiles ? fast_shape_tiles(a, (unsigned)c->n) : fast_shape_rows(a, c->n_sgp4, c->n_circ));
            if (int32_t rc = ensure_plan(c, a, shape, st); rc != AZ_OK) return rc;
        }
        const EccSide side{c->s_ecc, c->ev_fork2, c->ev_join2};
        if (a.n_list > 0 && cols) {
            if (int32_t rc = launch_cols(a, d_vel != nullptr, st, shape, side, c->n_sdp4); rc != AZ_OK) return rc;
            path |= AZH_PATH_COLS_FAST;
        } else if (a.n_list > 0 && tiles) {
            launch_tiles(a, d_vel != nullptr, st, shape);
            path |= AZH_PATH_TILES_FAST;
        } else if (a.n_list > 0 && fast) {
            const dim3 rgrid(std::min(8192u, std::max(256u, (a.n_list * cgrid_y(a.n_times, shape.tile_c) + 63u) / 64u)), 4);
            if (int32_t rc = launch_near_fast(a, d_vel != nullptr, shape, rgrid, st, side); rc != AZ_OK) return rc;
            path |= AZH_PATH_ROWS_FAST;
        } else if (a.n_list > 0) {
            path |= launch_propagate(a, layout, d_vel != nullptr, false, st);
        }
        if ((a.delta || a.delta64) && (path & (AZH_PATH_TILES_FAST | AZH_PATH_ROWS_FAST | AZH_PATH_COLS_FAST))) path |= AZH_PATH_QUASI_UNIFORM;
        HIP_TRY(hipGetLastError());
    }
    if (c->n_bad > 0) {
        hipLaunchKernelGGL(k_fill_bad, dim3((n_times + 255) / 256, c->n_bad), dim3(256), 0, st,
                           c->d_list.p + c->n_sgp4 + c->n_sdp4, c->n_bad, c->d_flags.p, n_times, d_pos, d_vel, d_err,
                           c->have_mask ? c->d_mask.p : nullptr, layout, stride, f32, a.row_lo, a.row_hi);
        HIP_TRY(hipGetLastError());
    }
    if (fork && !tiles) HIP_TRY(hipStreamWaitEvent(st, c->ev_join, 0));
    c->last_path = path;
    if (c->timing) {
        HIP_TRY(hipEventRecord(c->ev_t1, st));
        c->timed = true;
    }
    return AZ_OK;
}

int32_t launch_cached(azh_constellation *c, double *d_pos, double *d_vel, int layout, size_t stride, uint8_t *d_err, hipStream_t st,
                      int f32 = 0, size_t row_lo = 0, size_t row_hi = ~(size_t)0)
{
    if (!c->graphs_on || c->timing || c->cached_n_times == 0 || !c->s_main.owned()) return launch_all(c, d_pos, d_vel, layout, stride, d_err, st, f32, row_lo, row_hi);
    const unsigned sig = plan_sig(c);
    azh_constellation::LaunchGraph *hit = nullptr, *pending = nullptr;
    for (auto &g : c->graphs)
        if (g.pos == d_pos && g.vel == d_vel && g.err == d_err && g.layout == layout && g.f32 == f32 && g.stride == stride &&
            g.row_lo == row_lo && g.row_hi == row_hi && g.st == st) {
            if (g.fails >= 2) return launch_all(c, d_pos, d_vel, layout, stride, d_err, st, f32, row_lo, row_hi);
            if (g.exec && g.sig_before == sig) { hit = &g; break; }
            if (!g.exec && g.sig_before == sig) pending = &g;
        }
    if (hit) {
        HIP_TRY(hipGraphLaunch(hit->exec, st));
        for (unsigned k = 0; k < 4; ++k) c->plan[k].parity = (hit->sig_after >> k) & 1u;
        c->last_path = hit->path;
        HIP_TRY(hipEventRecord(c->ev_graph, st));
        return AZ_OK;
    }
    if (!pending) {
        if (c->graphs.size() >= 24) drop_graphs(c);
        const int32_t rc = launch_all(c, d_pos, d_vel, layout, stride, d_err, st, f32, row_lo, row_hi);
        if (rc == AZ_OK) {
            try {
                c->graphs.push_back({d_pos, d_vel, d_err, layout, f32, stride, row_lo, row_hi, st, sig, plan_sig(c), c->last_path, 1u, 0u, nullptr, nullptr});
            } catch (const std::bad_alloc &) {
            }
        }
        return rc;
    }
    if (hipStreamBeginCapture(st, hipStreamCaptureModeThreadLocal) != hipSuccess) {
        (void)hipGetLastError();
        return launch_all(c, d_pos, d_vel, layout, stride, d_err, st, f32, row_lo, row_hi);
    }
    unsigned parity0[4];
    for (unsigned k = 0; k < 4; ++k) parity0[k] = c->plan[k].parity;
    c->capturing = true;
    const int32_t rc = launch_all(c, d_pos, d_vel, layout, stride, d_err, st, f32, row_lo, row_hi);
    c->capturing = false;
    hipGraph_t graph = nullptr;
    const hipError_t e_end = hipStreamEndCapture(st, &graph);
    hipGraphExec_t exec = nullptr;
    if (rc != AZ_OK || e_end != hipSuccess || !graph || hipGraphInstantiate(&exec, graph, nullptr, nullptr, 0) != hipSuccess) {
        (void)hipGetLastError();
        if (graph) (void)hipGraphDestroy(graph);
        for (unsigned k = 0; k < 4; ++k) c->plan[k].parity = parity0[k];
        pending->fails += 1;
        if (rc != AZ_OK && rc != AZ_RC_EAGER) return rc;
        return launch_all(c, d_pos, d_vel, layout, stride, d_err, st, f32, row_lo, row_hi);
    }
    pending->graph = graph;
    pending->exec = exec;
    pending->sig_after = plan_sig(c);
    pending->path = c->last_path;
    HIP_TRY(hipGraphLaunch(exec, st));
    HIP_TRY(hipEventRecord(c->ev_graph, st));
    return AZ_OK;
}

class HostPool {
  public:
    int32_t alloc(size_t bytes, void **out)
    {
        if (!out) return AZ_ERR_NULL_POINTER;
        *out = nullptr;
        const size_t need = std::max<size_t>((bytes + kGrain - 1) / kGrain * kGrain, kGrain);
        {
            std::lock_guard<std::mutex> lock(mu_);
            auto it = free_.lower_bound(need);
            if (it != free_.end() && it->first <= need + need / 4 + kGrain) {
                void *q = it->second;
                free_bytes_ -= it->first;
                live_[static_cast<char *>(q)] = it->first;
                free_.erase(it);
                *out = q;
                return AZ_OK;
            }
        }
        void *q = nullptr;
        if (hipHostMalloc(&q, need, hipHostMallocPortable) != hipSuccess || !q) {
            (void)hipGetLastError();
            trim(0);
            if (!hip_ok(hipHostMalloc(&q, need, hipHostMallocPortable), "hipHostMalloc(result)")) return AZ_ERR_ALLOC_FAILED;
        }
        std::lock_guard<std::mutex> lock(mu_);
        live_[static_cast<char *>(q)] = need;
        *out = q;
        return AZ_OK;
    }
    void release(void *q)
    {
        if (!q) return;
        {
            std::lock_guard<std::mutex> lock(mu_);
            auto it = live_.find(static_cast<char *>(q));
            if (it == live_.end()) return;
            free_.emplace(it->second, q);
            free_bytes_ += it->second;
            live_.erase(it);
        }
        trim(cap());
    }
    bool owns(const void *q, size_t len)
    {
        if (!q) return false;
        std::lock_guard<std::mutex> lock(mu_);
        auto it = live_.upper_bound(const_cast<char *>(static_cast<const char *>(q)));
        if (it == live_.begin()) return false;
        --it;
        return static_cast<const char *>(q) + len <= it->first + it->second;
    }
    void stats(size_t *live_bytes, size_t *free_bytes)
    {
        std::lock_guard<std::mutex> lock(mu_);
        size_t l = 0;
        for (auto &kv : live_) l += kv.second;
        if (live_bytes) *live_bytes = l;
        if (free_bytes) *free_bytes = free_bytes_;
    }
    void trim(size_t keep)
    {
        std::vector<void *> drop;
        {
            std::lock_guard<std::mutex> lock(mu_);
            while (free_bytes_ > keep && !free_.empty()) {
                auto it = std::prev(free_.end());
                drop.push_back(it->second);
                free_bytes_ -= it->first;
                free_.erase(it);
            }
        }
        for (void *q : drop) (void)hipHostFree(q);
    }

  private:
    static constexpr size_t kGrain = size_t(2) << 20;
    static size_t cap()
    {
        static const size_t c = [] {
            const char *e = getenv("ASTROZ_AMD_HOST_POOL_MB");
            return (size_t)(e ? std::max(0L, atol(e)) : 4096L) << 20;
        }();
        return c;
    }
    std::mutex mu_;
    std::map<char *, size_t> live_;
    std::multimap<size_t, void *> free_;
    size_t free_bytes_ = 0;
};
HostPool &host_pool()
{
    static HostPool *p = new HostPool();
    return *p;
}

class CopyPool {
  public:
    explicit CopyPool(unsigned k)
    {
        for (unsigned i = 0; i < k; ++i) {
            try {
                th_.emplace_back([this, i] { work(i); });
            } catch (const std::system_error &) {
                break;
            }
        }
    }
    unsigned size() const { return (unsigned)th_.size(); }
    size_t submit(char *dst, const char *src, size_t len)
    {
        std::lock_guard<std::mutex> lock(mu_);
        jobs_.push_back({dst, src, len, (unsigned)th_.size()});
        cv_.notify_all();
        return jobs_.size() - 1;
    }
    void wait(size_t ticket)
    {
        std::unique_lock<std::mutex> lock(mu_);
        done_cv_.wait(lock, [&] { return jobs_[ticket].left == 0; });
    }
    ~CopyPool()
    {
        {
            std::lock_guard<std::mutex> lock(mu_);
            stop_ = true;
            cv_.notify_all();
        }
        for (auto &t : th_) t.join();
    }

  private:
    struct Job {
        char *dst;
        const char *src;
        size_t len;
        unsigned left;
    };
    void work(unsigned me)
    {
        size_t next = 0;
        for (;;) {
            Job j;
            {
                std::unique_lock<std::mutex> lock(mu_);
                cv_.wait(lock, [&] { return stop_ || next < jobs_.size(); });
                if (next >= jobs_.size()) return;
                j = jobs_[next];
// ... 505 lines not shown
{
    if (!c) return AZ_ERR_NULL_POINTER;
    c->graphs_on = enabled != 0;
    if (!c->graphs_on) drop_graphs(c);
    return AZ_OK;
}

static int32_t propagate_device(azh_constellation *c, const double *times, size_t n_times, const double *offsets, double *d_pos,
                                double *d_vel, int32_t mode, double reference_jd, const uint8_t *mask, int32_t layout, size_t stride,
                                uint8_t *d_err, void *stream, int f32)
{
    return guarded([&]() -> int32_t {
        if (!c || !d_pos || (n_times && !times)) return AZ_ERR_NULL_POINTER;
        if (mode < 0 || mode > AZ_OUT_TOPOCENTRIC || layout < 0 || layout > 1) return AZ_ERR_VALUE;
        if (mode == AZ_OUT_TOPOCENTRIC && !c->have_observer) return AZ_ERR_VALUE;
        if (n_times == 0) return AZ_OK;
        if (set_device(c) != AZ_OK) return AZ_ERR_HIP;
        hipStream_t st = stream ? (hipStream_t)stream : c->s_main;
        int32_t rc = stage_inputs(c, times, n_times, offsets, mask, mode, reference_jd, st);
        if (rc != AZ_OK) return rc;
        return launch_all(c, d_pos, d_vel, layout, stride, d_err, st, f32);
    });
}
int32_t azh_propagate_device(azh_constellation *c, const double *times, size_t n_times, const double *offsets,
                             double *d_pos, double *d_vel, int32_t mode, double reference_jd, const uint8_t *mask,
                             int32_t layout, size_t stride, uint8_t *d_err, void *stream)
{
    return propagate_device(c, times, n_times, offsets, d_pos, d_vel, mode, reference_jd, mask, layout, stride, d_err, stream, 0);
}
int32_t azh_propagate_device_f32(azh_constellation *c, const double *times, size_t n_times, const double *offsets,
                                 float *d_pos, float *d_vel, int32_t mode, double reference_jd, const uint8_t *mask,
                                 int32_t layout, size_t stride, uint8_t *d_err, void *stream)
{
    return propagate_device(c, times, n_times, offsets, reinterpret_cast<double *>(d_pos), reinterpret_cast<double *>(d_vel), mode,
                            reference_jd, mask, layout, stride, d_err, stream, 1);
}

static int32_t propagate_cached(azh_constellation *c, size_t row_lo, size_t row_hi, double *d_pos, double *d_vel, int32_t layout,
                                size_t stride, uint8_t *d_err, void *stream, int f32)
{
    return guarded([&]() -> int32_t {
        if (!c || !d_pos) return AZ_ERR_NULL_POINTER;
        if (layout < 0 || layout > 1) return AZ_ERR_VALUE;
        if (c->cached_n_times == 0) return AZ_ERR_NOT_INITIALIZED;
        if (set_device(c) != AZ_OK) return AZ_ERR_HIP;
        return launch_cached(c, d_pos, d_vel, layout, stride, d_err, stream ? (hipStream_t)stream : c->s_main, f32, row_lo, row_hi);
    });
}
int32_t azh_propagate_device_cached(azh_constellation *c, double *d_pos, double *d_vel, int32_t layout,
                                    size_t stride, uint8_t *d_err, void *stream)
{
    return propagate_cached(c, 0, ~(size_t)0, d_pos, d_vel, layout, stride, d_err, stream, 0);
}
int32_t azh_propagate_device_window(azh_constellation *c, size_t row_lo, size_t row_hi, double *d_pos, double *d_vel,
                                    int32_t layout, size_t stride, uint8_t *d_err, void *stream)
{
    return propagate_cached(c, row_lo, row_hi, d_pos, d_vel, layout, stride, d_err, stream, 0);
}
int32_t azh_propagate_device_cached_f32(azh_constellation *c, float *d_pos, float *d_vel, int32_t layout, size_t stride,
                                        uint8_t *d_err, void *stream)
{
    return propagate_cached(c, 0, ~(size_t)0, reinterpret_cast<double *>(d_pos), reinterpret_cast<double *>(d_vel), layout, stride,
                            d_err, stream, 1);
}

constexpr size_t kNoTarget = ~(size_t)0;
static int32_t screen_core(azh_constellation *c, const double *times, size_t n_times, const double *offsets, size_t target,
                           const double *d_track, double threshold_km, double *d_min_dist, uint32_t *d_min_t, void *stream)
{
    if (!c || !d_min_dist || !d_min_t || (n_times && !times)) return AZ_ERR_NULL_POINTER;
    if (!d_track && target >= c->n) return AZ_ERR_VALUE;
    if (d_track && target != kNoTarget && target >= c->n) return AZ_ERR_VALUE;
    if (set_device(c) != AZ_OK) return AZ_ERR_HIP;
    hipStream_t st = stream ? (hipStream_t)stream : c->s_main;
    int32_t rc = AZ_OK;
    if (n_times > 0 && (rc = stage_inputs(c, times, n_times, offsets, nullptr, AZ_OUT_TEME, 0.0, st)) != AZ_OK) return rc;
    const unsigned nt = (unsigned)n_times;
    if (c->timing) HIP_TRY(hipEventRecord(c->ev_t0, st));
    const unsigned nb_fill = ((unsigned)c->n + 255) / 256;
    if (nt == 0) {
        hipLaunchKernelGGL(k_screen_prep, dim3(nb_fill), dim3(64), 0, st, c->d_el.p, c->d_flags.p, c->n_pad, 0u, (const double *)nullptr, 0u,
                           (const double *)nullptr, c->g, (double *)nullptr, 0u, (size_t)0, (double *)nullptr, (unsigned *)nullptr, 0u,
                           (unsigned)c->n, threshold_km, d_min_dist, d_min_t);
        HIP_TRY(hipGetLastError());
    }
    if (nt > 0) {
        if (!d_track && c->d_tgt.ensure((size_t)nt * 3) != AZ_OK) return AZ_ERR_HIP;
        PropArgs a{};
        a.el = c->d_el.p;
        a.flags = c->d_flags.p;
        a.n_pad = c->n_pad;
        a.times = c->d_times.p;
        a.n_times = nt;
        a.offsets = c->have_offsets ? c->d_offsets.p : nullptr;
        a.stride_sats = c->n;
        a.mode = AZ_OUT_TEME;
        a.g = c->g;
        a.uniform_step = c->fast_path ? c->uniform_step : 0.0;
        a.inc = (a.uniform_step != 0.0) ? c->d_inc.p : nullptr;
        a.fast_rec = (a.uniform_step != 0.0) ? c->d_fast_rec.p : nullptr;
        a.delta = (a.uniform_step != 0.0 && c->delta_max > 0.0 && !c->delta_wide) ? c->d_delta.p : nullptr;
        a.delta64 = (a.uniform_step != 0.0 && c->delta_max > 0.0) ? c->d_delta64.p : nullptr;
        a.delta_wide = c->delta_wide ? 1 : 0;
        a.grid_t0 = c->grid_t0;
        a.delta_max = c->delta_max;
        a.grid_exact_uniform = (c->uniform_step != 0.0 && c->delta_max == 0.0) ? 1 : 0;
        a.row_lo = 0;
        a.row_hi = 0xffffffffu;
        a.screen_target = d_track ? d_track : c->d_tgt.p;
        PropArgs near = a, deep = a;
        unsigned parts_near = 0, parts_deep = 0;
        c->last_path = 0;
        const bool fast_screen = c->n_sgp4 > 0 && a.inc != nullptr && nt >= 32;
        FastShape shape;
        if (c->n_sgp4 > 0) {
            near.list = c->d_list.p;
            near.n_list = c->n_sgp4;
            near.tile = auto_tile(c->n_sgp4, nt, c->tile_sgp4, 8);
            near.tile_forced = c->tile_sgp4;
            parts_near = screen_parts(near, false);
            if (fast_screen) {
                near.list = c->d_list.p + c->off_circ;
                near.n_circ = c->n_circ;
                shape = fast_shape_rows(near, c->n_sgp4, c->n_circ);
                if ((rc = ensure_plan(c, near, shape, st)) != AZ_OK) return rc;
                near.tile = shape.tile_c;
                near.tile_e = shape.tile_e;
                near.screen_nseg = cgrid_y(nt, std::min(shape.tile_c, shape.tile_e));
                parts_near = 5u * near.screen_nseg;
            }
        }
        if (c->n_sdp4 > 0) {
            if ((rc = prepare_deep(c, deep, st, use_rows(deep, AZ_LAYOUT_SAT_MAJOR, true))) != AZ_OK) return rc;
            parts_deep = screen_parts(deep, true);
        }
        const size_t np_near = (size_t)parts_near * c->n_sgp4, np_deep = (size_t)parts_deep * c->n_sdp4;
        if (c->d_part_d2.ensure(np_near + np_deep) != AZ_OK || c->d_part_t.ensure(np_near + np_deep) != AZ_OK) return AZ_ERR_HIP;
        const double thr2 = threshold_km * threshold_km;
        near.part_d2 = c->d_part_d2.p;
        near.part_t = c->d_part_t.p;
        deep.part_d2 = c->d_part_d2.p + np_near;
        deep.part_t = c->d_part_t.p + np_near;
        {
            const unsigned nb_track = d_track ? 0u : (nt + 63) / 64;
            const size_t n_clear = fast_screen ? np_near : 0;
            const unsigned nb_clear = (unsigned)((n_clear + 255) / 256);
            hipLaunchKernelGGL(k_screen_prep, dim3(nb_track + nb_clear + nb_fill), dim3(64), 0, st, c->d_el.p, c->d_flags.p, c->n_pad,
                               (unsigned)(d_track ? 0 : target), c->d_times.p, nt, c->have_offsets ? c->d_offsets.p : (const double *)nullptr, c->g,
                               c->d_tgt.p, nb_track, n_clear, near.part_d2, near.part_t, nb_clear, (unsigned)c->n, threshold_km, d_min_dist, d_min_t);
            HIP_TRY(hipGetLastError());
        }
        if (c->n_sgp4 > 0) {
            if (fast_screen) {
                if ((rc = launch_near_fast(near, false, shape, dim3(256, 4), st, EccSide{c->s_ecc, c->ev_fork2, c->ev_join2})) != AZ_OK) return rc;
                c->last_path = AZH_PATH_ROWS_FAST | ((near.delta || near.delta64) ? AZH_PATH_QUASI_UNIFORM : 0u);
            } else {
                c->last_path = launch_propagate(near, AZ_LAYOUT_SAT_MAJOR, false, false, st);
            }
            HIP_TRY(hipGetLastError());
        }
        if (c->n_sdp4 > 0) {
            c->last_path |= launch_propagate(deep, AZ_LAYOUT_SAT_MAJOR, false, true, st);
            HIP_TRY(hipGetLastError());
        }
        const unsigned n_fin = c->n_sgp4 + c->n_sdp4;
        if (n_fin > 0) {
            hipLaunchKernelGGL(k_screen_finalize2, dim3((n_fin + 255) / 256), dim3(256), 0, st, near.part_d2, near.part_t, parts_near, near.list, c->n_sgp4,
                               deep.part_d2, deep.part_t, parts_deep, deep.list, c->n_sdp4, thr2, (unsigned)target, d_min_dist, d_min_t);
            HIP_TRY(hipGetLastError());
        }
    }
    if (c->timing) {
        HIP_TRY(hipEventRecord(c->ev_t1, st));
        c->timed = true;
    }
    return AZ_OK;
}
int32_t azh_screen_target_device(azh_constellation *c, const double *times, size_t n_times, const double *offsets,
                                 size_t target, double threshold_km, double reference_jd, double *d_min_dist,
                                 uint32_t *d_min_t, void *stream)
{
    (void)reference_jd;
    return guarded([&]() -> int32_t {
        if (c && target >= c->n) return AZ_ERR_VALUE;
        return screen_core(c, times, n_times, offsets, target, nullptr, threshold_km, d_min_dist, d_min_t, stream);
    });
}
int32_t azh_screen_track_device(azh_constellation *c, const double *times, size_t n_times, const double *offsets, const double *d_track,
                                size_t exclude_index, double threshold_km, double *d_min_dist, uint32_t *d_min_t, void *stream)
{
    return guarded([&]() -> int32_t {
        if (!d_track) return AZ_ERR_NULL_POINTER;
        return screen_core(c, times, n_times, offsets, exclude_index, d_track, threshold_km, d_min_dist, d_min_t, stream);
    });
}

int32_t azh_screen_target_host(azh_constellation *c, const double *times, size_t n_times, const double *offsets,
                               size_t target, double threshold_km, double reference_jd, double *min_dist,
                               uint32_t *min_t)
{
    return guarded([&]() -> int32_t {
        if (!c || !min_dist || !min_t) return AZ_ERR_NULL_POINTER;
        if (set_device(c) != AZ_OK) return AZ_ERR_HIP;
        const size_t small_total = c->n * (sizeof(double) + sizeof(uint32_t)) + 64;
        if (small_total <= kSmallOut) {
            if (c->h_small.cap < small_total) HIP_TRY(hipStreamSynchronize(c->s_main));
            if (c->h_small.ensure(small_total) != AZ_OK) return AZ_ERR_HIP;
            double *hd = static_cast<double *>(c->h_small.p);
            uint32_t *ht = reinterpret_cast<uint32_t *>(hd + ((c->n + 7) & ~size_t(7)));
            double *dd = nullptr;
            HIP_TRY(hipHostGetDevicePointer((void **)&dd, hd, 0));
            uint32_t *dt = reinterpret_cast<uint32_t *>(dd + (reinterpret_cast<double *>(ht) - hd));
            int32_t rc = azh_screen_target_device(c, times, n_times, offsets, target, threshold_km, reference_jd, dd, dt, nullptr);
            if (rc != AZ_OK) return rc;
            HIP_TRY(hipStreamSynchronize(c->s_main));
            memcpy(min_dist, hd, sizeof(double) * c->n);
            memcpy(min_t, ht, sizeof(uint32_t) * c->n);
            return AZ_OK;
        }
        if (c->d_out_d.ensure(c->n) != AZ_OK || c->d_out_t.ensure(c->n) != AZ_OK) return AZ_ERR_HIP;
        int32_t rc = azh_screen_target_device(c, times, n_times, offsets, target, threshold_km, reference_jd, c->d_out_d.p,
                                              c->d_out_t.p, nullptr);
        if (rc != AZ_OK) return rc;
        HIP_TRY(hipMemcpyAsync(min_dist, c->d_out_d.p, sizeof(double) * c->n, hipMemcpyDeviceToHost, c->s_main));
        HIP_TRY(hipMemcpyAsync(min_t, c->d_out_t.p, sizeof(uint32_t) * c->n, hipMemcpyDeviceToHost, c->s_main));
        HIP_TRY(hipStreamSynchronize(c->s_main));
        return AZ_OK;
    });
}

namespace {
int32_t coarse_screen(const double *d_pos, size_t n_sats, size_t n_times, int32_t layout, size_t stride,
                      double threshold_km, const uint8_t *valid_mask, uint32_t *out_pairs, uint32_t *out_t,
                      size_t max_results, size_t *n_found, void *stream, int skip_zero)
{
    if (!d_pos || !n_found || (max_results && (!out_pairs || !out_t))) return AZ_ERR_NULL_POINTER;
    *n_found = 0;
    if (layout < 0 || layout > 1 || !(threshold_km > 0.0)) return AZ_ERR_VALUE;
    if (n_sats == 0 || n_times == 0) return AZ_OK;
    if (n_sats > 0x7fffffffu || n_times > 0xffffffffu) return AZ_ERR_VALUE;
    if (stride == 0) stride = n_sats;
    hipStream_t st = (hipStream_t)stream;
    if (st == nullptr) HIP_TRY(hipDeviceSynchronize());
    unsigned bits = 16;
    while (bits < 24 && ((size_t)1 << bits) < 2 * n_sats) ++bits;
    const size_t table = (size_t)1 << bits;
    const unsigned chunk = (unsigned)std::max<size_t>(1, std::min<size_t>(std::min<size_t>(n_times, 64), ((size_t)1 << 25) / (table + n_sats)));
    int dev_id = 0;
    HIP_TRY(hipGetDevice(&dev_id));
    struct Scratch {
        std::mutex mu;
        DevBuf<unsigned> head, occupied, next, pairs, t;
        DevBuf<unsigned long long> count;
        DevBuf<uint8_t> valid;
    };
    static std::mutex table_mu;
    static auto *per_device = new std::map<int, std::unique_ptr<Scratch>>();
    Scratch *S = nullptr;
    {
        std::lock_guard<std::mutex> lk(table_mu);
        auto &slot = (*per_device)[dev_id];
        if (!slot) slot.reset(new Scratch());
        S = slot.get();
    }
    std::lock_guard<std::mutex> lock(S->mu);
    int32_t rc = AZ_OK;
    std::vector<uint32_t> hp, ht;
    size_t cap = std::max<size_t>(std::min<size_t>(max_results, (size_t)1 << 20), 1 << 16);
    unsigned long long total = 0;
    do {
        if (S->head.ensure(table * chunk) != AZ_OK || S->occupied.ensure(table / 32 * chunk) != AZ_OK || S->next.ensure(n_sats * chunk) != AZ_OK ||
            S->count.ensure(1) != AZ_OK) { rc = AZ_ERR_HIP; break; }
        uint8_t *d_valid = nullptr;
        if (valid_mask) {
            if (S->valid.ensure(n_sats) != AZ_OK ||
                !hip_ok(hipMemcpyAsync(S->valid.p, valid_mask, n_sats, hipMemcpyHostToDevice, st), "H2D valid")) { rc = AZ_ERR_HIP; break; }
            d_valid = S->valid.p;
        }
        for (int pass = 0; pass < 2 && rc == AZ_OK; ++pass) {
            if (S->pairs.ensure(2 * cap) != AZ_OK || S->t.ensure(cap) != AZ_OK ||
                !hip_ok(hipMemsetAsync(S->count.p, 0, sizeof(unsigned long long), st), "memset count")) { rc = AZ_ERR_HIP; break; }
            CellArgs a{};
            a.pos = d_pos;
            a.n_sats = (unsigned)n_sats;
            a.n_times = (unsigned)n_times;
            a.layout = layout;
            a.stride_sats = stride;
            a.valid = d_valid;
            a.inv_cell = 1.0 / threshold_km;
            a.thr2 = threshold_km * threshold_km;
            a.table_mask = (unsigned)(table - 1);
            a.head = S->head.p;
            a.occupied = S->occupied.p;
            a.next = S->next.p;
            a.out_pairs = S->pairs.p;
            a.out_t = S->t.p;
            a.count = S->count.p;
            a.max_results = cap;
            a.skip_zero = skip_zero;
            for (size_t t0 = 0; t0 < n_times && rc == AZ_OK; t0 += chunk) {
                a.t0 = (unsigned)t0;
                a.n_steps = (unsigned)std::min<size_t>(chunk, n_times - t0);
                if (!hip_ok(hipMemsetAsync(S->head.p, 0xff, sizeof(unsigned) * table * a.n_steps, st), "memset head")) { rc = AZ_ERR_HIP; break; }
                dim3 grid(8u * (unsigned)((n_sats + 255) / 256) * ((a.n_steps + 7u) / 8u));
                hipLaunchKernelGGL(k_cells_build, grid, dim3(256), 0, st, a);
                hipLaunchKernelGGL(k_cells_bits, dim3((unsigned)(table * a.n_steps / 256)), dim3(256), 0, st, S->head.p, S->occupied.p, table * a.n_steps);
                hipLaunchKernelGGL(k_cells_probe, grid, dim3(256), (table / 32 <= AZ_CELL_BITMAP_WORDS) ? (unsigned)(table / 32 * sizeof(unsigned)) : 0u, st, a);
// ... 779 lines not shown
{
    return guarded([&]() -> int32_t {
        if (int32_t rc = conjunction_args(times, n_times, n_targets, threshold_km, max_events); rc != AZ_OK) return rc;
        if (!c || !n_events || !targets || (n_times && !times) || (max_events && !out)) return AZ_ERR_NULL_POINTER;
        if (int32_t rc = conjunction_targets(c, targets, n_targets); rc != AZ_OK) return rc;
        if (set_device(c) != AZ_OK) return AZ_ERR_HIP;
        if (c->d_conj_out.cap < max_events || c->d_pass_n.cap < 1) HIP_TRY(hipStreamSynchronize(c->s_main));
        if ((max_events && c->d_conj_out.ensure(max_events) != AZ_OK) || c->d_pass_n.ensure(1) != AZ_OK) return AZ_ERR_HIP;
        int32_t rc = find_conjunctions(c, times, n_times, offsets, targets, n_targets, threshold_km, max_events ? c->d_conj_out.p : nullptr,
                                       max_events, c->d_pass_n.p, c->s_main);
        if (rc == AZ_OK && !hip_ok(hipMemcpyAsync(n_events, c->d_pass_n.p, sizeof(uint32_t), hipMemcpyDeviceToHost, c->s_main), "D2H"))
            rc = AZ_ERR_HIP;
        if (!hip_ok(hipStreamSynchronize(c->s_main), "sync") && rc == AZ_OK) rc = AZ_ERR_HIP;
        if (rc != AZ_OK) return rc;
        const size_t kept = std::min<size_t>(*n_events, max_events);
        if (kept == 0) return AZ_OK;
        HIP_TRY(hipMemcpyAsync(out, c->d_conj_out.p, sizeof(azh_conjunction) * kept, hipMemcpyDeviceToHost, c->s_main));
        HIP_TRY(hipStreamSynchronize(c->s_main));
        std::sort(out, out + kept, [](const azh_conjunction &a, const azh_conjunction &b) {
            if (a.target != b.target) return a.target < b.target;
            if (a.sat != b.sat) return a.sat < b.sat;
            return a.t_tca_min < b.t_tca_min;
        });
        return AZ_OK;
    });
}

int32_t azh_propagate_host(azh_constellation *c, const double *times, size_t n_times, const double *offsets,
                           double *pos, double *vel, int32_t mode, double reference_jd, const uint8_t *mask,
                           int32_t layout, size_t stride, uint8_t *err)
{
    return guarded([&]() -> int32_t {
        if (!c || !pos || (n_times && !times)) return AZ_ERR_NULL_POINTER;
        if (n_times == 0) return AZ_OK;
        if (set_device(c) != AZ_OK) return AZ_ERR_HIP;
        if (stride == 0) stride = c->n;
        const size_t rows = (layout == AZ_LAYOUT_TIME_MAJOR) ? stride : c->n;
        const size_t bytes = rows * n_times * 3 * sizeof(double);
        const size_t words = bytes / sizeof(double);
        if (c->n > 1 && !c->h_el.empty() && mode == AZ_OUT_TEME && mask == nullptr && host_points() > 0) {
            size_t cost = 0;
            for (size_t sidx = 0; sidx < c->n; ++sidx) cost += n_times * ((c->h_flags[sidx] & AZ_FLAG_DEEP) ? 2 : 1);
            if (cost <= host_points()) {
                std::vector<double> ts(n_times), p(3 * n_times), v(3 * n_times);
                std::vector<uint8_t> e(n_times);
                for (size_t sidx = 0; sidx < c->n; ++sidx) {
                    const double o = offsets ? offsets[sidx] : 0.0;
                    for (size_t t = 0; t < n_times; ++t) ts[t] = times[t] + o;
                    azhost::propagate_points(c->h_el.data(), c->n_pad, sidx, c->h_flags[sidx], c->g, ts.data(), n_times, 0, nullptr, p.data(),
                                             vel ? v.data() : nullptr, e.data());
                    for (size_t t = 0; t < n_times; ++t) {
                        const size_t at = (layout == AZ_LAYOUT_TIME_MAJOR ? t * stride + sidx : sidx * n_times + t) * 3;
                        memcpy(pos + at, &p[3 * t], 3 * sizeof(double));
                        if (vel) memcpy(vel + at, &v[3 * t], 3 * sizeof(double));
                        if (err) err[sidx * n_times + t] = e[t];
                    }
                }
                c->last_path = AZH_PATH_HOST_STEP;
                c->cached_n_times = 0;
                c->staged_valid = false;
                c->timed = false;
                return AZ_OK;
            }
        }
        if (c->n == 1 && mode == AZ_OUT_TEME && mask == nullptr && (layout == AZ_LAYOUT_SAT_MAJOR || stride <= 1) && n_times <= kOneStage &&
            AZ_FLAG_ERR(c->h_flags[0]) == 0) {
            std::vector<double> ts(times, times + n_times);
            if (offsets)
                for (auto &t : ts) t += offsets[0];
            c->last_path = 0;
            c->cached_n_times = 0;
            c->staged_valid = false;
            c->timed = false;
            return run_one_satellite(c, 0, ts.data(), n_times, 0, nullptr, pos, vel, err);
        }
        const size_t err_bytes = err ? c->n * n_times : 0, small_total = bytes * (vel ? 2 : 1) + ((err_bytes + 63) & ~size_t(63));
        if (small_total <= kSmallOut && mask == nullptr && !(layout == AZ_LAYOUT_TIME_MAJOR && stride > c->n)) {
            if (c->h_small.ensure(small_total) != AZ_OK) return AZ_ERR_HIP;
            char *dev = nullptr;
            HIP_TRY(hipHostGetDevicePointer((void **)&dev, c->h_small.p, 0));
            const size_t o_vel = bytes, o_err = bytes * (vel ? 2 : 1);
            int32_t rc = azh_propagate_device(c, times, n_times, offsets, reinterpret_cast<double *>(dev), vel ? reinterpret_cast<double *>(dev + o_vel) : nullptr,
                                              mode, reference_jd, mask, layout, stride, err ? reinterpret_cast<uint8_t *>(dev + o_err) : nullptr, nullptr);
            if (rc == AZ_OK && !hip_ok(hipStreamSynchronize(c->s_main), "sync")) rc = AZ_ERR_HIP;
            if (rc != AZ_OK) {
                (void)hipStreamSynchronize(c->s_main);
                return rc;
            }
            const char *h = static_cast<const char *>(c->h_small.p);
            memcpy(pos, h, bytes);
            if (vel) memcpy(vel, h + o_vel, bytes);
            if (err) memcpy(err, h + o_err, err_bytes);
            return AZ_OK;
        }
        if (c->d_host_pos.ensure(words) != AZ_OK || (vel && c->d_host_vel.ensure(words) != AZ_OK) ||
            (err && c->d_host_err.ensure(c->n * n_times) != AZ_OK))
            return AZ_ERR_HIP;
        double *d_pos = c->d_host_pos.p, *d_vel = vel ? c->d_host_vel.p : nullptr;
        uint8_t *d_err = err ? c->d_host_err.p : nullptr;
        int32_t rc = AZ_OK;
        do {
            const bool partial = mask != nullptr || (layout == AZ_LAYOUT_TIME_MAJOR && stride > c->n);
            if (partial) {
                if (!hip_ok(hipMemcpyAsync(d_pos, pos, bytes, hipMemcpyHostToDevice, c->s_main), "H2D pos")) { rc = AZ_ERR_HIP; break; }
                if (vel && !hip_ok(hipMemcpyAsync(d_vel, vel, bytes, hipMemcpyHostToDevice, c->s_main), "H2D vel")) { rc = AZ_ERR_HIP; break; }
            }
            rc = azh_propagate_device(c, times, n_times, offsets, d_pos, d_vel, mode, reference_jd, mask, layout, stride, d_err, nullptr);
            if (rc != AZ_OK) break;
            void *const dst[3] = {pos, vel, err};
            const void *const src[3] = {d_pos, d_vel, d_err};
            const size_t len[3] = {bytes, vel ? bytes : 0, err ? c->n * n_times : 0};
            const unsigned thr = host_copy_threads();
            const bool pinned_out = host_pool().owns(pos, bytes) && (!vel || host_pool().owns(vel, bytes));
            if (!pinned_out && thr > 0 && len[0] + len[1] + len[2] >= (size_t(8) << 20)) {
                if ((rc = copy_back_staged(c->stager, dst, src, len, 3, c->s_main, thr)) != AZ_OK) break;
            } else {
                for (int k = 0; k < 3 && rc == AZ_OK; ++k)
                    if (len[k] && !hip_ok(hipMemcpyAsync(dst[k], src[k], len[k], hipMemcpyDeviceToHost, c->s_main), "D2H")) rc = AZ_ERR_HIP;
                if (rc != AZ_OK) break;
            }
            if (!hip_ok(hipStreamSynchronize(c->s_main), "sync")) { rc = AZ_ERR_HIP; break; }
        } while (0);
        if (rc != AZ_OK) (void)hipStreamSynchronize(c->s_main);
        return rc;
    });
}

int32_t azh_propagate_jd_host(azh_constellation *c, const double *jd, const double *fr, size_t n_times, double *pos,
                              double *vel, int32_t mode, int32_t layout, uint8_t *err)
{
    return guarded([&]() -> int32_t {
        if (!c || !jd || !fr || !pos) return AZ_ERR_NULL_POINTER;
        double ref = c->h_epoch.empty() ? 0.0 : c->h_epoch[0];
        for (size_t s = 0; s < c->n; ++s)
            if (AZ_FLAG_ERR(c->h_flags[s]) == 0 && !(c->h_flags[s] & AZ_FLAG_DEEP)) { ref = c->h_epoch[s]; break; }
        std::vector<double> times(n_times), offs(c->n);
        for (size_t t = 0; t < n_times; ++t) times[t] = ((jd[t] + fr[t]) - ref) * 1440.0;
        for (size_t s = 0; s < c->n; ++s) offs[s] = (ref - c->h_epoch[s]) * 1440.0;
        return azh_propagate_host(c, times.data(), n_times, offs.data(), pos, vel, mode, ref, nullptr, layout, 0, err);
    });
}

int32_t azh_synchronize(azh_constellation *c)
{
    if (!c) return AZ_ERR_NULL_POINTER;
    if (set_device(c) != AZ_OK) return AZ_ERR_HIP;
    HIP_TRY(hipStreamSynchronize(c->s_deep));
    HIP_TRY(hipStreamSynchronize(c->s_ecc));
    HIP_TRY(hipStreamSynchronize(c->s_main));
    return AZ_OK;
}

uint32_t azh_last_path(const azh_constellation *c) { return c ? c->last_path : 0u; }

int32_t azh_last_one_stats(azh_constellation *c, uint32_t *n_segments, uint32_t *n_handed_over)
{
    if (!c || !n_segments || !n_handed_over) return AZ_ERR_NULL_POINTER;
    *n_segments = c->one_segments;
    *n_handed_over = 0;
    if (c->one_segments == 0) return AZ_OK;
    if (set_device(c) != AZ_OK) return AZ_ERR_HIP;
    HIP_TRY(hipEventSynchronize(c->ev_one));
    unsigned head[AZ_ONE_HEAD];
    HIP_TRY(hipMemcpy(head, c->d_one_items.p, sizeof(head), hipMemcpyDeviceToHost));
    unsigned cnt = 0;
    for (unsigned k = 0; k < AZ_ONE_LISTS; ++k) cnt += head[32u * k];
    *n_handed_over = cnt;
    return AZ_OK;
}

double azh_last_kernel_ms(azh_constellation *c)
{
    if (!c || !c->timed) return -1.0;
    float ms = -1.0f;
    if (hipEventElapsedTime(&ms, c->ev_t0, c->ev_t1) != hipSuccess) {
        (void)hipGetLastError();
        return -1.0;
    }
    return (double)ms;
}

int32_t azh_propagate_one_host(azh_constellation *c, size_t sat, const double *tsince, size_t n, double *pos,
                               double *vel, uint8_t *err)
{
    return guarded([&]() -> int32_t {
        if (!c || !tsince || !pos) return AZ_ERR_NULL_POINTER;
        if (sat >= c->n) return AZ_ERR_VALUE;
        if (n == 0) return AZ_OK;
        return run_one_satellite(c, sat, tsince, n, 0, nullptr, pos, vel, err);
    });
}

int32_t azh_propagate_one_device(azh_constellation *c, size_t sat, const double *d_tsince, size_t n, double *d_pos,
                                 double *d_vel, uint8_t *d_err, void *stream)
{
    return guarded([&]() -> int32_t {
        if (!c || !d_tsince || !d_pos) return AZ_ERR_NULL_POINTER;
        if (sat >= c->n || n > 0xffffffffu) return AZ_ERR_VALUE;
        if (n == 0) return AZ_OK;
        if (set_device(c) != AZ_OK) return AZ_ERR_HIP;
        hipStream_t st = stream ? (hipStream_t)stream : c->s_main;
        if (c->timing) HIP_TRY(hipEventRecord(c->ev_t0, st));
        if (int32_t lrc = launch_one(c, sat, d_tsince, n, d_pos, d_vel, d_err, 0, st); lrc != AZ_OK) return lrc;
        if (c->timing) {
            HIP_TRY(hipEventRecord(c->ev_t1, st));
            c->timed = true;
        }
        return AZ_OK;
    });
}

int32_t azh_selftest_math(const double *x, size_t n, double *out6n, int32_t device)
{
    if (!x || !out6n) return AZ_ERR_NULL_POINTER;
    if (n == 0) return AZ_OK;
    HIP_TRY(hipSetDevice(device));
    DevBuf<double> d;
    if (d.ensure(7 * n) != AZ_OK) return AZ_ERR_HIP;
    if (!hip_ok(hipMemcpy(d.p, x, sizeof(double) * n, hipMemcpyHostToDevice), "H2D")) return AZ_ERR_HIP;
    hipLaunchKernelGGL(k_math_kat, dim3((unsigned)((n + 63) / 64)), dim3(64), 0, nullptr, d.p, (unsigned)n, d.p + n);
    if (!hip_ok(hipGetLastError(), "k_math_kat") ||
        !hip_ok(hipMemcpy(out6n, d.p + n, sizeof(double) * 6 * n, hipMemcpyDeviceToHost), "D2H"))
        return AZ_ERR_HIP;
    return AZ_OK;
}

int32_t azh_selftest_host_step(const double *el, size_t n_pad, size_t sat, uint32_t flags, int32_t grav, const double *tsince_min,
                               size_t n, double *out6n, uint8_t *err)
{
    if (!el || !tsince_min || !out6n) return AZ_ERR_NULL_POINTER;
    if (sat >= n_pad) return AZ_ERR_VALUE;
    if (!azhost::cpu_ok()) return AZ_ERR_UNKNOWN;
    azhost::propagate_points(el, n_pad, sat, flags, make_grav(grav), tsince_min, n, 1, out6n, nullptr, nullptr, err);
    return AZ_OK;
}

struct azh_group {
    int n_dev = 0;
    size_t n = 0, rows = 0, n_chunks = 1;
    std::vector<int> devices;
    std::vector<std::unique_ptr<azh_constellation>> shard;
    std::vector<std::vector<uint32_t>> members;
    std::vector<std::vector<double>> off_stage;
    std::vector<double> track_stage;
    std::vector<ncclComm_t> comms;
    std::vector<Stream> s_comm;
    std::vector<Event> ev;
    size_t cell_lo(size_t chunk, int d) const { return std::min((chunk * n_dev + d) * rows, n); }
    size_t cell_hi(size_t chunk, int d) const { return std::min((chunk * n_dev + d) * rows + rows, n); }
    size_t padded() const { return n_chunks * n_dev * rows; }
    ~azh_group();
};

namespace {

struct Rccl {
    void *h = nullptr;
    decltype(&ncclCommInitAll) CommInitAll = nullptr;
    decltype(&ncclCommDestroy) CommDestroy = nullptr;
    decltype(&ncclAllGather) AllGather = nullptr;
    decltype(&ncclGroupStart) GroupStart = nullptr;
    decltype(&ncclGroupEnd) GroupEnd = nullptr;
    decltype(&ncclGetErrorString) GetErrorString = nullptr;
    bool ok = false;
};

Rccl &rccl()
{
    static Rccl r;
    static std::once_flag once;
    std::call_once(once, [] {
        for (const char *name : {"librccl.so.1", "librccl.so", "/opt/rocm/lib/librccl.so.1"}) {
            r.h = dlopen(name, RTLD_NOW | RTLD_GLOBAL);
            if (r.h) break;
        }
        if (!r.h) return;
#define AZ_SYM(f) r.f = reinterpret_cast<decltype(r.f)>(dlsym(r.h, "nccl" #f))
        AZ_SYM(CommInitAll); AZ_SYM(CommDestroy); AZ_SYM(AllGather); AZ_SYM(GroupStart); AZ_SYM(GroupEnd); AZ_SYM(GetErrorString);
#undef AZ_SYM
        r.ok = r.CommInitAll && r.CommDestroy && r.AllGather && r.GroupStart && r.GroupEnd;
    });
    return r;
}

bool nccl_ok(ncclResult_t e, const char *what)
{
    if (e == ncclSuccess) return true;
    g_last_error = std::string(what) + ": " + (rccl().GetErrorString ? rccl().GetErrorString(e) : "RCCL error");
    return false;
}

}

azh_group::~azh_group()
{
    for (ncclComm_t comm : comms)
        if (comm) (void)rccl().CommDestroy(comm);
    for (size_t d = 0; d < s_comm.size(); ++d) {
        (void)hipSetDevice(devices[d]);
        s_comm[d].reset();
        ev[d].reset();
    }
}

namespace {

// ... 567 lines not shown
```

astroz_amd/csrc/kernels.h:

```cpp
#pragma once
#include <hip/hip_runtime.h>

#include <type_traits>

#include "init_device.h"
#include "propagate_device.h"
#include "fast_step.h"
#include "fast_step_f32.h"

#ifndef AZ_BLOCK
#define AZ_BLOCK 256
#endif
#ifndef AZ_PROP_FAST
#define AZ_PROP_FAST 1
#endif
#ifndef AZ_MIN_WAVES
#define AZ_MIN_WAVES 1
#endif
#ifndef AZ_ROWS_WAVES
#define AZ_ROWS_WAVES 3
#endif
#ifndef AZ_DEEP_WAVES
#define AZ_DEEP_WAVES 2
#endif
#define AZ_RESEED 256
#ifndef AZ_SM_CHUNK
#define AZ_SM_CHUNK 4
#endif

struct PropArgs {
    const double *el;
    const unsigned *flags;
    size_t n_pad;
    const unsigned *list;
    unsigned n_list;
    const double *times;
    unsigned n_times;
    const double *offsets;
    double *pos, *vel;
    const double *sin_g, *cos_g;
    const unsigned char *mask;
    unsigned char *err;
    size_t stride_sats;
    unsigned tile;
    unsigned tile_e, screen_nseg;
    unsigned tile_forced;
    const double *seeds;
    int mode;
    int f32;
    int tm_rows;
    int rows_compact;
    unsigned ecc_row0;
    const double *screen_target;
    union {
        double *part_d2;
        const AzObserver *obs;
    };
    unsigned *part_t;
    double uniform_step;
    int grid_exact_uniform;
    const float *delta;
    double delta_max;
    const double *delta64;
    int delta_wide;
    double grid_t0;
    const double *inc;
    const double *fast_rec;
    unsigned row_lo, row_hi;
    unsigned slot_lo, slot_hi;
    unsigned win_circ_lo, win_circ_hi, win_ecc_lo, win_ecc_hi;
    int arith32;
    unsigned n_circ;
    unsigned redo_slot0;
    unsigned *redo_count;
    unsigned *redo_next;
    unsigned *redo_items;
    const unsigned *rowmap;
    const double *tmp_pos, *tmp_vel;
    unsigned n_rows;
    const double *plan_win;
    const unsigned char *plan_flag;
    unsigned plan_stride;
    const unsigned *redo_static;
    AzGrav g;
};
enum { AZ_ROW_NEAR = 0, AZ_ROW_COPY = 1, AZ_ROW_ZERO = 2 };
enum { AZ_PLAN_sOc, AZ_PLAN_cOc, AZ_PLAN_sdU, AZ_PLAN_cdU, AZ_PLAN_s1U, AZ_PLAN_c1U, AZ_PLAN_NUM };
#define AZ_PLAN_OK 1u
#define AZ_PLAN_TC 2u

template <class T>
__device__ __forceinline__ void az_put3(T *o, const double r[3])
{
    o[0] = (T)r[0];
    o[1] = (T)r[1];
    o[2] = (T)r[2];
}
typedef double az_d2s __attribute__((ext_vector_type(2), aligned(8)));
typedef float az_f3s __attribute__((ext_vector_type(3), aligned(4)));
#ifndef AZ_ROWS_NT
#define AZ_ROWS_NT 1
#endif
__device__ __forceinline__ void az_put3_stream(double *o, const double r[3])
{
#if AZ_ROWS_NT
    const az_d2s a = {r[0], r[1]};
    __builtin_nontemporal_store(a, reinterpret_cast<az_d2s *>(o));
    __builtin_nontemporal_store(r[2], o + 2);
#else
    az_put3(o, r);
#endif
}
__device__ __forceinline__ void az_put3_stream(float *o, const double r[3])
{
#if AZ_ROWS_NT
    const az_f3s a = {(float)r[0], (float)r[1], (float)r[2]};
    __builtin_nontemporal_store(a, reinterpret_cast<az_f3s *>(o));
#else
    az_put3(o, r);
#endif
}

__device__ __forceinline__ void az_epilogue(double r[3], double v[3], int mode, bool vel, const double *sin_g,
                                            const double *cos_g, unsigned i)
{
    if (mode != 0) {
        const double sg = sin_g[i], cg = cos_g[i];
        az_to_ecef(r, sg, cg);
        if (vel) az_to_ecef(v, sg, cg);
        if (mode == 2) az_ecef_to_geodetic(r);
    }
}
template <bool VEL>
__device__ __forceinline__ void az_epilogue_topo(double r[3], double v[3], const PropArgs &p, unsigned i)
{
    const double sg = p.sin_g[i], cg = p.cos_g[i];
    az_to_ecef(r, sg, cg);
    if (VEL) az_to_ecef(v, sg, cg);
    az_topocentric<VEL>(r, v, *p.obs);
}

#define AZ_TM_ROW 256
#define AZ_SM_ROW (AZ_SM_CHUNK * 3 + 1)

typedef double az_d2 __attribute__((ext_vector_type(2)));

#if defined(AZ_STORE_POLICY) && AZ_STORE_POLICY == 1
#define AZ_ST1(ptr, val) __builtin_nontemporal_store((val), (ptr))
#define AZ_ST2(ptr, val) __builtin_nontemporal_store((val), (ptr))
#else
#define AZ_ST1(ptr, val) (*(ptr) = (val))
#define AZ_ST2(ptr, val) (*(ptr) = (val))
#endif

__device__ __forceinline__ double az_readlane_f64(double x, unsigned lane_uniform)
{
    const int lo = __builtin_amdgcn_readlane(__double2loint(x), (int)lane_uniform);
    const int hi = __builtin_amdgcn_readlane(__double2hiint(x), (int)lane_uniform);
    return __hiloint2double(hi, lo);
}

__device__ __forceinline__ void az_wave_lds_fence()
{
    __builtin_amdgcn_fence(__ATOMIC_RELEASE, "wavefront");
    __builtin_amdgcn_wave_barrier();
    __builtin_amdgcn_fence(__ATOMIC_ACQUIRE, "wavefront");
}

__device__ __forceinline__ void az_tm_flush(const double *L, double *row, size_t pitch, unsigned lane, unsigned par, bool last)
{
    const az_d2 *lp = reinterpret_cast<const az_d2 *>(L);
    az_d2 *g = reinterpret_cast<az_d2 *>(row);
    if (par == 0u) {
// ... 952 lines not shown
                const unsigned en = (f_row >> (24u + 2u * m)) & 3u;
                if (f_lds[m] == 0xffffffffu || en == 0u || (!full && base + ((f_row >> (8u * m)) & 63u) >= t_hi)) continue;
                const az_d2s val = *reinterpret_cast<const az_d2s *>(bufc + f_lds[m]);
                double *g = reinterpret_cast<double *>((((f_row >> (8u * m)) & 128u) ? vel_b : pos_b) + f_out[m]);
                if (en == 3u) *reinterpret_cast<az_d2s *>(g) = val;
                else if (en == 1u) g[0] = val.x;
                else g[1] = val.y;
            }
        }
    }
}

#include "cols_kernel.h"

__device__ __forceinline__ unsigned az_lds_address(const void *p)
{
    return (unsigned)(size_t)(__attribute__((address_space(3))) const void *)p;
}
__device__ __forceinline__ void az_stage_pair3(unsigned a, const az_f2 q[3])
{
    asm volatile("ds_write2_b32 %0, %1, %2 offset1:3\n\t"
                 "ds_write2_b32 %0, %3, %4 offset0:1 offset1:4\n\t"
                 "ds_write2_b32 %0, %5, %6 offset0:2 offset1:5"
                 :
                 : "v"(a), "v"(q[0].x), "v"(q[0].y), "v"(q[1].x), "v"(q[1].y), "v"(q[2].x), "v"(q[2].y));
}
__device__ __forceinline__ void az_flush_pair3(unsigned a, float *out, unsigned lane)
{
    az_f4 lo, hi;
    asm volatile("ds_read_b128 %0, %2\n\t"
                 "ds_read_b128 %1, %2 offset:1024\n\t"
                 "s_waitcnt lgkmcnt(0)"
                 : "=&v"(lo), "=&v"(hi)
                 : "v"(a));
    az_f4 *dst = reinterpret_cast<az_f4 *>(out);
    __builtin_nontemporal_store(lo, dst + lane);
    if (lane < 32) __builtin_nontemporal_store(hi, dst + lane + 64);
}

template <bool VEL, bool MIXED = false, bool DELTA = false>
__global__ void __launch_bounds__(64, MIXED ? AZ_ROWSF32P_WAVES : AZ_ROWSF32_WAVES) k_rows_fast32(PropArgs p)
{
    const unsigned lane = threadIdx.x;
    const unsigned row = az_list_slot(p);
    if (row >= az_list_end(p)) return;
    const unsigned s = p.list[row];
    const unsigned fl = p.flags[s];
    if ((p.mask != nullptr && p.mask[s] == 0) || s < p.row_lo || s >= p.row_hi) return;
    const unsigned t_lo = blockIdx.y * p.tile;
    const unsigned t_hi = min(t_lo + p.tile, p.n_times);
    unsigned base = t_lo;
    if (AZ_FLAG_ECLASS(fl) == 0) {
        __shared__ __attribute__((aligned(16))) float rows_stage[2 * 128 * 3];
        const double off = az_uniform(p.offsets ? p.offsets[s] : 0.0);
        float *prow = reinterpret_cast<float *>(p.pos) + (size_t)s * p.n_times * 3;
        float *vrow = VEL ? reinterpret_cast<float *>(p.vel) + (size_t)s * p.n_times * 3 : nullptr;
        const bool staged = AZ_ROWS_LDS_STORE &&
                            (((reinterpret_cast<size_t>(prow) | (VEL ? reinterpret_cast<size_t>(vrow) : 0)) & 15u) == 0);
        const double step = p.uniform_step;
        const double t_first = p.grid_t0 + off;
        __shared__ float once_lds[F32_NUM];
        FastK32Bcast k;
        FastCarry32 fc;
        bool window_ok;
        const unsigned stage_w = az_lds_address(rows_stage) + lane * 24, stage_r = az_lds_address(rows_stage) + lane * 16;
        {
            const double w_a = fma((double)t_lo, step, t_first), w_b = fma((double)(t_hi - 1), step, t_first);
            FastK k0, k1;
            az_load_fast(p.el, p.n_pad, s, fl, p.inc, 0, k0);
            az_double_increments(k0);
            window_ok = az_plan_window(p, blockIdx.y, row + p.redo_slot0, w_a, w_b, k0);
            if (!window_ok) return;
            az_fast_udot(k0);
            az_load_fast(p.el, p.n_pad, s, fl, p.inc, 1, k1);
            {
                const double *w = p.plan_win + ((size_t)blockIdx.y * p.plan_stride + row + p.redo_slot0) * AZ_PLAN_NUM;
                k1.sdU_ = w[AZ_PLAN_s1U]; k1.cdU_ = w[AZ_PLAN_c1U];
                k1.tc_ = k0.tc_; k1.tmid_ = k0.tmid_; k1.sOc_ = k0.sOc_; k1.cOc_ = k0.cOc_;
            }
            FastK32 kk;
            az_load_fast32(k0, k1, step, p.g, kk);
#define X(n) if (lane == 0) once_lds[F32_##n] = kk.n##_;
            AZ_F32_ONCE(X)
#undef X
#define X(n) k.n##_ = az_uniform32(kk.n##_);
            AZ_F32_MANY(X)
#undef X
#define U(n) k.n = az_uniform(kk.n);
            U(sab64) U(sdU) U(cdU) U(tc) U(tmid) U(s1U) U(c1U)
            if (MIXED) { U(abase_km64) U(rv0_64) U(sOc64) U(cOc64) U(sinio64) U(cosio64) }
#undef U
            az_wave_lds_fence();
            FastCarry f0;
            az_seed_fast(p.el, p.n_pad, s, fma((double)(t_lo + 2 * lane) - 128.0, step, t_first), k.tc, f0);
            az_seed_fast32(f0, k1, fc);
        }
        __shared__ __attribute__((aligned(8))) float dl_lds[DELTA ? AZ_DELTA_SEG : 2];
        if (DELTA) {
#pragma unroll
            for (unsigned j = lane; j < AZ_DELTA_SEG; j += 64) dl_lds[j] = p.delta[t_lo + j];
            az_wave_lds_fence();
        }
#pragma unroll 1
        for (; window_ok && base < t_hi; base += 128) {
            const unsigned i = base + 2 * lane;
            const bool live_a = i < t_hi, live_b = i + 1 < t_hi;
            const double t = fma((double)i, step, t_first);
            unsigned zero = 0;
            asm volatile("" : "+v"(zero));
            k.once = once_lds + zero;
            az_f2 r[3], v[3];
#if defined(AZ_ABLATE) && AZ_ABLATE == 2
            r[0] = az_splat2((float)t); r[1] = r[0] + 1.0f; r[2] = r[0] + 2.0f; v[0] = r[0] + 3.0f; v[1] = r[0] + 4.0f; v[2] = r[0] + 5.0f;
#else
            az_f2 dl = az_splat2(0.0f);
            if (DELTA) dl = *reinterpret_cast<const az_f2 *>(dl_lds + (i - t_lo));
            if (MIXED) az_sgp4_fast_step_f32p<VEL, DELTA>(k, p.g, t, fc, r, v, dl);
            else az_sgp4_fast_step_f32<VEL, DELTA>(k, p.g, t, fc, r, v, dl);
#endif
#if defined(AZ_ABLATE) && AZ_ABLATE == 1
            if (!(live_a && (r[0].x + r[1].x + r[2].x + r[0].y + r[1].y + r[2].y +
                             (VEL ? v[0].x + v[1].x + v[2].x + v[0].y + v[1].y + v[2].y : 0.0f)) == 1.2345e30f)) continue;
#endif
            if (staged && base + 128 <= t_hi) {
                az_stage_pair3(stage_w, r);
                az_flush_pair3(stage_r, prow + (size_t)base * 3, lane);
                if (VEL) {
                    az_stage_pair3(stage_w + 1536, v);
                    az_flush_pair3(stage_r + 1536, vrow + (size_t)base * 3, lane);
                }
            } else {
                if (live_a) {
                    const az_f3s a = {r[0].x, r[1].x, r[2].x};
                    __builtin_nontemporal_store(a, reinterpret_cast<az_f3s *>(prow + (size_t)i * 3));
                    if (VEL) {
                        const az_f3s b = {v[0].x, v[1].x, v[2].x};
                        __builtin_nontemporal_store(b, reinterpret_cast<az_f3s *>(vrow + (size_t)i * 3));
                    }
                }
                if (live_b) {
                    const az_f3s a = {r[0].y, r[1].y, r[2].y};
                    __builtin_nontemporal_store(a, reinterpret_cast<az_f3s *>(prow + (size_t)(i + 1) * 3));
                    if (VEL) {
                        const az_f3s b = {v[0].y, v[1].y, v[2].y};
                        __builtin_nontemporal_store(b, reinterpret_cast<az_f3s *>(vrow + (size_t)(i + 1) * 3));
                    }
                }
            }
        }
    }
}

template <bool VEL, int FRAME, int SINK, bool REDO = false>
__global__ void __launch_bounds__(64, AZ_ROWS_WAVES) k_rows(PropArgs p)
{
    typedef typename std::conditional<SINK == AZ_SINK_F32, float, double>::type out_t;
    const unsigned lane = threadIdx.x;
    __shared__ __attribute__((aligned(16))) double rows_lds[AZ_ROWS_TLDS + C_NUM_MAX + 2 + 8];
    static_assert(F_nodeo < 8 && F_argpo < 8 && F_mo < 8, "the epoch angles sit in the first eight rows of the element table");
    constexpr bool redo = REDO;
    const unsigned n_items = redo ? *p.redo_count : 1u;
#pragma unroll 1
    for (unsigned item = redo ? blockIdx.x : 0u; item < n_items; item += redo ? gridDim.x : 1u) {
    unsigned row, t_lo, t_hi;
    if (redo) {
        row = p.redo_items[3 * (size_t)item];
        const unsigned b0 = p.redo_items[3 * (size_t)item + 1], b1 = p.redo_items[3 * (size_t)item + 2];
        const unsigned quarter = (((b1 - b0 + 63) / 64 + gridDim.y - 1) / gridDim.y) * 64;
        t_lo = b0 + blockIdx.y * quarter;
        t_hi = min(t_lo + quarter, b1);
        if (t_lo >= b1) continue;
    } else {
        row = az_list_slot(p);
        if (row >= az_list_end(p)) return;
        t_lo = blockIdx.y * p.tile;
        t_hi = min(t_lo + p.tile, p.n_times);
    }
    const unsigned s = p.list[row];
    const unsigned fl = p.flags[s];
    if (SINK != AZ_SINK_SCREEN && ((p.mask != nullptr && p.mask[s] == 0) || s < p.row_lo || s >= p.row_hi)) continue;
    const double off = az_uniform(p.offsets ? p.offsets[s] : 0.0);
    const RotK rk = az_rotk();
#if defined(AZ_ABLATE) && AZ_ABLATE == 3
    const size_t srow = s & 63u;
#else
    const size_t srow = s;
#endif
    out_t *prow = reinterpret_cast<out_t *>(p.pos) + srow * p.n_times * 3;
    out_t *vrow = VEL ? reinterpret_cast<out_t *>(p.vel) + srow * p.n_times * 3 : nullptr;
    double best_d2 = __builtin_inf();
    unsigned best_t = 0xffffffffu;
    az_wave_lds_fence();
    Sgp4Lane e;
    typedef ColdBroadcast ColdT;
    const ColdT cold{rows_lds + AZ_ROWS_TLDS};
    az_load_sgp4(p.el, p.n_pad, s, fl, e, cold);
    e.mdot = az_uniform(e.mdot); e.argpdot = az_uniform(e.argpdot); e.nodedot = az_uniform(e.nodedot);
    e.xnodcf = az_uniform(e.xnodcf); e.aycof = az_uniform(e.aycof); e.xlcof = az_uniform(e.xlcof);
    e.sinio = az_uniform(e.sinio); e.cosio = az_uniform(e.cosio); e.k_mrt = az_uniform(e.k_mrt);
    e.k_c2u = az_uniform(e.k_c2u); e.k_su = az_uniform(e.k_su); e.k_node = az_uniform(e.k_node);
    e.k_inc = az_uniform(e.k_inc); e.x1mth2 = az_uniform(e.x1mth2); e.k_rv = az_uniform(e.k_rv);
    double *seed_lds = rows_lds + AZ_ROWS_TLDS + C_NUM_MAX + 2;
    if (lane < 8) seed_lds[lane] = p.el[(size_t)lane * p.n_pad + s];
    az_wave_lds_fence();
    Sgp4Carry c;
    c.t_prev = 0.0;
    c.sW = c.sO = c.sA = 0.0;
    c.cW = c.cO = c.cA = 1.0;
    c.dt_c = -1.0e300;
    c.sdA = c.pW = c.qW = 0.0;
    c.cdA = 1.0;
#pragma unroll 1
    for (unsigned base = t_lo; base < t_hi; base += 64) {
        const unsigned i = base + lane;
        const bool live = i < t_hi;
        const unsigned kk = (base - t_lo) & (AZ_ROWS_TLDS - 1u);
        if (kk == 0) {
            az_wave_lds_fence();
#pragma unroll
            for (unsigned j = 0; j < AZ_ROWS_TLDS; j += 64) rows_lds[j + lane] = p.times[min(i + j, t_hi - 1)];
            az_wave_lds_fence();
        }
        const double t = rows_lds[kk + lane] + off;
        double r[3], v[3];
        const bool first = ((base - t_lo) & (64u * 64u - 1u)) == 0;
#if defined(AZ_ABLATE) && AZ_ABLATE == 2
        r[0] = t; r[1] = t + 1.0; r[2] = t + 2.0; v[0] = t + 3.0; v[1] = t + 4.0; v[2] = t + 5.0;
        (void)first;
#else
        az_sgp4_step<VEL, ColdT, true>(e, cold, seed_lds, 1, 0, p.g, rk, t, first, c, r, v, p.grid_exact_uniform != 0);
#endif
        if (SINK == AZ_SINK_SCREEN) {
            const double *q = p.screen_target + (size_t)(live ? i : t_hi - 1) * 3;
            const double dx = q[0] - r[0], dy = q[1] - r[1], dz = q[2] - r[2];
            const double d2 = dx * dx + dy * dy + dz * dz;
            if (live && d2 < best_d2) {
                best_d2 = d2;
                best_t = i;
            }
            continue;
        }
        if (FRAME == 3) az_epilogue_topo<VEL>(r, v, p, live ? i : t_hi - 1);
        else if (FRAME) az_epilogue(r, v, p.mode, VEL, p.sin_g, p.cos_g, live ? i : t_hi - 1);
#if defined(AZ_ABLATE) && AZ_ABLATE == 1
        if (!(live && (r[0] + r[1] + r[2] + (VEL ? v[0] + v[1] + v[2] : 0.0)) == 1.2345e300)) continue;
#endif
        if (live && redo && p.tm_rows) {
            const size_t ob = ((size_t)i * p.stride_sats + s) * 3;
            az_put3(reinterpret_cast<out_t *>(p.pos) + ob, r);
            if (VEL) az_put3(reinterpret_cast<out_t *>(p.vel) + ob, v);
        } else if (live) {
            az_put3_stream(prow + (size_t)i * 3, r);
            if (VEL) az_put3_stream(vrow + (size_t)i * 3, v);
        }
    }
    if (SINK == AZ_SINK_SCREEN) {
        az_wave_argmin(best_d2, best_t);
        if (lane == 0) {
            size_t part = blockIdx.y;
            if (redo) part = p.screen_nseg + 4u * (p.redo_items[3 * (size_t)item + 1] / (row < p.n_circ ? p.tile : p.tile_e)) + blockIdx.y;
            p.part_d2[part * p.n_list + row] = best_d2;
            p.part_t[part * p.n_list + row] = best_t;
        }
    }
    }
    if (redo && lane == 0 && blockIdx.x == 0 && blockIdx.y == 0) *p.redo_next = *p.redo_static;
}

#ifndef AZ_ROWSD_WAVES
#define AZ_ROWSD_WAVES 3
#endif
#define AZ_DEEP_SEED_MAX 64
template <bool VEL, int FRAME, int SINK>
__global__ void __launch_bounds__(64, AZ_ROWSD_WAVES) k_rows_deep(PropArgs p)
{
    typedef typename std::conditional<SINK == AZ_SINK_F32, float, double>::type out_t;
    constexpr unsigned TL = 512;
    const unsigned lane = threadIdx.x;
    const unsigned row = az_list_slot(p);
    if (row >= az_list_end(p)) return;
    const unsigned s = p.list[row];
    const unsigned fl = p.flags[s];
    if (SINK != AZ_SINK_SCREEN && ((p.mask != nullptr && p.mask[s] == 0) || s < p.row_lo || s >= p.row_hi)) return;
    const unsigned t_lo = blockIdx.y * p.tile;
    const unsigned t_hi = min(t_lo + p.tile, p.n_times);
    __shared__ double lds[TL + H_NUM + D_NUM + 3 * AZ_DEEP_SEED_MAX + MC_NUM];
    double *seed_lds = lds + TL + H_NUM + D_NUM;
    int irez;
    {
        Sdp4Bcast e0{lds + TL, 0};
        az_load_sdp4(p.el, p.n_pad, s, fl, e0, ColdBroadcastLit{lds + TL + H_NUM});
        irez = e0.irez;
        if (lane < MC_NUM) lds[TL + H_NUM + D_NUM + 3 * AZ_DEEP_SEED_MAX + lane] = az_mc_table[lane];
    }
    const bool res = irez != 0;
    const unsigned n_chunks = (t_hi - t_lo + 63u) >> 6;
    if (res && p.seeds) {
        for (unsigned j = lane; j < 3u * n_chunks; j += 64u) {
            const unsigned c = j / 3u, f = j - 3u * c;
            seed_lds[j] = p.seeds[((size_t)((t_lo >> 6) + c) * 3 + f) * p.n_list + row];
        }
    }
    const double off = az_uniform(p.offsets ? p.offsets[s] : 0.0);
    const bool uniform = p.uniform_step != 0.0 && p.delta == nullptr && p.delta64 == nullptr;
    const double step = p.uniform_step, t_first = uniform ? p.times[0] + off : 0.0;
    const RotK rk = az_rotk();
    const size_t out_row = p.rows_compact ? row : s;
    out_t *prow = reinterpret_cast<out_t *>(p.pos) + out_row * p.n_times * 3;
    out_t *vrow = VEL ? reinterpret_cast<out_t *>(p.vel) + out_row * p.n_times * 3 : nullptr;
    double best_d2 = __builtin_inf();
    unsigned best_t = 0xffffffffu;
    Sdp4Acc acc;
    acc.atime = __builtin_nan("");
    acc.xndt = acc.xnddt = acc.xldot = 0.0;
    az_wave_lds_fence();
#pragma unroll 1
    for (unsigned base = t_lo; base < t_hi; base += 64) {
        const unsigned i = base + lane;
        const bool live = i < t_hi;
        double t;
        if (uniform) {
            t = fma((double)i, step, t_first);
        } else {
            const unsigned kk = (base - t_lo) & (TL - 1u);
            if (kk == 0) {
                az_wave_lds_fence();
#pragma unroll
                for (unsigned j = 0; j < TL; j += 64) lds[j + lane] = p.times[min(i + j, t_hi - 1)];
                az_wave_lds_fence();
            }
            t = lds[kk + lane] + off;
        }
        const double *lds_now = az_opaque_lds(lds + TL);
        const Sdp4Bcast e{const_cast<double *>(lds_now), irez};
        const ColdBroadcast cold{const_cast<double *>(lds_now) + H_NUM, lds_now + H_NUM + D_NUM + 3 * AZ_DEEP_SEED_MAX};
        Sdp4Carry cy;
        if (res && p.seeds) {
            const double *sd = lds_now + H_NUM + D_NUM + 3u * ((base - t_lo) >> 6);
            cy.atime = sd[0];
            cy.xli = sd[1];
            cy.xni = sd[2];
        } else {
            cy.atime = 0.0;
            cy.xli = e(H_xlamo);
            cy.xni = e(H_no_unkozai);
        }
        double r[3], v[3];
        if (res) az_resonance_cached(e, cold, t, cy, acc);
        int rc = az_sdp4_step_pre<VEL>(e, cold, p.g, rk, t, cy, r, v, acc);
        if (SINK == AZ_SINK_SCREEN) {
            const double *q = p.screen_target + (size_t)(live ? i : t_hi - 1) * 3;
            const double dx = q[0] - r[0], dy = q[1] - r[1], dz = q[2] - r[2];
            const double d2 = dx * dx + dy * dy + dz * dz;
            if (live && rc == 0 && d2 < best_d2) {
                best_d2 = d2;
                best_t = i;
            }
            continue;
        }
        if (FRAME == 3) az_epilogue_topo<VEL>(r, v, p, live ? i : t_hi - 1);
        else if (FRAME) az_epilogue(r, v, p.mode, VEL, p.sin_g, p.cos_g, live ? i : t_hi - 1);
        if (rc != 0) {
            r[0] = r[1] = r[2] = 0.0;
            v[0] = v[1] = v[2] = 0.0;
            if (p.err && live) p.err[(size_t)s * p.n_times + i] = (unsigned char)rc;
        }
        if (live) {
            az_put3_stream(prow + (size_t)i * 3, r);
            if (VEL) az_put3_stream(vrow + (size_t)i * 3, v);
        }
    }
    if (SINK == AZ_SINK_SCREEN) {
        az_wave_argmin(best_d2, best_t);
// ... 384 lines not shown
```

bindings/zig/astroz_hip.zig:

```

pub const HipError = error{
    BadTleLength,
    BadChecksum,
    DeepSpaceNotSupported,
    InvalidEccentricity,
    SatelliteDecayed,
    ValueError,
    OutOfMemory,
    NullPointer,
    NotInitialized,
    DeviceFailure,
    Unknown,
};

pub fn check(rc: i32) HipError!void {
    return switch (rc) {
        0 => {},
        -1 => HipError.BadTleLength,
        -2 => HipError.BadChecksum,
        -10 => HipError.DeepSpaceNotSupported,
        -11 => HipError.InvalidEccentricity,
        -12 => HipError.SatelliteDecayed,
        -20 => HipError.ValueError,
        -100 => HipError.OutOfMemory,
        -101 => HipError.NullPointer,
        -102 => HipError.NotInitialized,
        -200 => HipError.DeviceFailure,
        else => HipError.Unknown,
    };
}

pub const Handle = opaque {};

pub const Err = enum(i32) {
    ok = 0,
    bad_tle_length = -1,
    bad_checksum = -2,
    deep_space_not_supported = -10,
    invalid_eccentricity = -11,
    satellite_decayed = -12,
    value_error = -20,
    alloc_failed = -100,
    null_pointer = -101,
    not_initialized = -102,
    hip = -200,
    unknown = -999,
};

pub extern "c" fn azh_device_count() c_int;
pub extern "c" fn azh_last_error() [*:0]const u8;
pub extern "c" fn azh_parse_tle_lines(line1: [*:0]const u8, line2: [*:0]const u8, out16: [*]f64) i32;
pub extern "c" fn azh_constellation_from_tle_text(text: [*]const u8, len: usize, grav: i32, device: i32, out: *?*Handle) i32;
pub extern "c" fn azh_constellation_from_tle_lines(line1: [*]const [*:0]const u8, line2: [*]const [*:0]const u8, n: usize, grav: i32, device: i32, out: *?*Handle) i32;
pub extern "c" fn azh_constellation_from_elements(n: usize, epoch_jd: [*]const f64, mm_revday: [*]const f64, ecc: [*]const f64, incl_deg: [*]const f64, raan_deg: [*]const f64, argp_deg: [*]const f64, ma_deg: [*]const f64, bstar: [*]const f64, grav: i32, device: i32, out: *?*Handle) i32;
pub extern "c" fn azh_constellation_free(h: ?*Handle) void;
pub extern "c" fn azh_num_satellites(h: ?*const Handle) usize;
pub extern "c" fn azh_num_sgp4(h: ?*const Handle) usize;
pub extern "c" fn azh_num_sdp4(h: ?*const Handle) usize;
pub extern "c" fn azh_get_epochs(h: ?*const Handle, out: [*]f64) i32;
pub extern "c" fn azh_get_status(h: ?*const Handle, err: ?[*]u8, is_deep: ?[*]u8, irez: ?[*]u8) i32;
pub extern "c" fn azh_get_field(h: ?*const Handle, name: [*:0]const u8, out: [*]f64) i32;
pub extern "c" fn azh_propagate_host(h: ?*Handle, times_min: [*]const f64, n_times: usize, epoch_offsets_min: ?[*]const f64, pos: [*]f64, vel: ?[*]f64, output_mode: i32, reference_jd: f64, sat_mask: ?[*]const u8, layout: i32, out_stride_sats: usize, err: ?[*]u8) i32;
pub extern "c" fn azh_propagate_device(h: ?*Handle, times_min: [*]const f64, n_times: usize, epoch_offsets_min: ?[*]const f64, d_pos: [*]f64, d_vel: ?[*]f64, output_mode: i32, reference_jd: f64, sat_mask: ?[*]const u8, layout: i32, out_stride_sats: usize, d_err: ?[*]u8, stream: ?*anyopaque) i32;
pub extern "c" fn azh_propagate_device_cached(h: ?*Handle, d_pos: [*]f64, d_vel: ?[*]f64, layout: i32, out_stride_sats: usize, d_err: ?[*]u8, stream: ?*anyopaque) i32;
pub extern "c" fn azh_propagate_jd_host(h: ?*Handle, jd: [*]const f64, fr: [*]const f64, n_times: usize, pos: [*]f64, vel: ?[*]f64, output_mode: i32, layout: i32, err: ?[*]u8) i32;
pub extern "c" fn azh_propagate_one_host(h: ?*Handle, sat_index: usize, tsince_min: [*]const f64, n: usize, pos: [*]f64, vel: ?[*]f64, err: ?[*]u8) i32;
pub extern "c" fn azh_synchronize(h: ?*Handle) i32;
pub extern "c" fn azh_set_time_tile(h: ?*Handle, sgp4_tile: u32, sdp4_tile: u32) i32;
pub extern "c" fn azh_set_timing(h: ?*Handle, enabled: i32) i32;
pub extern "c" fn azh_last_kernel_ms(h: ?*Handle) f64;

pub extern "c" fn azh_propagate_device_f32(h: ?*Handle, times_min: [*]const f64, n_times: usize, epoch_offsets_min: ?[*]const f64,
    d_pos: [*]f32, d_vel: ?[*]f32, output_mode: i32, reference_jd: f64, sat_mask: ?[*]const u8, layout: i32,
    out_stride_sats: usize, d_err: ?[*]u8, stream: ?*anyopaque) i32;
pub extern "c" fn azh_propagate_device_cached_f32(h: ?*Handle, d_pos: [*]f32, d_vel: ?[*]f32, layout: i32,
    out_stride_sats: usize, d_err: ?[*]u8, stream: ?*anyopaque) i32;

pub extern "c" fn azh_screen_target_host(h: ?*Handle, times_min: [*]const f64, n_times: usize, epoch_offsets_min: ?[*]const f64,
    target_index: usize, threshold_km: f64, reference_jd: f64, min_dist_km: [*]f64, min_t_index: [*]u32) i32;
pub extern "c" fn azh_screen_target_device(h: ?*Handle, times_min: [*]const f64, n_times: usize, epoch_offsets_min: ?[*]const f64,
    target_index: usize, threshold_km: f64, reference_jd: f64, d_min_dist_km: [*]f64, d_min_t_index: [*]u32, stream: ?*anyopaque) i32;
pub extern "c" fn azh_screen_track_device(h: ?*Handle, times_min: [*]const f64, n_times: usize, epoch_offsets_min: ?[*]const f64,
    d_track: [*]const f64, exclude_index: usize, threshold_km: f64, d_min_dist_km: [*]f64, d_min_t_index: [*]u32, stream: ?*anyopaque) i32;
pub extern "c" fn azh_coarse_screen_device(d_pos: [*]const f64, n_sats: usize, n_times: usize, layout: i32, stride_sats: usize,
    threshold_km: f64, valid_mask: ?[*]const u8, out_pairs: [*]u32, out_t_index: [*]u32, max_results: usize, n_found: *usize,
    stream: ?*anyopaque) i32;
pub extern "c" fn azh_coarse_screen_host(pos: [*]const f64, n_sats: usize, n_times: usize, layout: i32, stride_sats: usize,
    threshold_km: f64, valid_mask: ?[*]const u8, out_pairs: [*]u32, out_t_index: [*]u32, max_results: usize, n_found: *usize,
    device: i32) i32;
pub extern "c" fn azh_screen_all_host(h: ?*Handle, times_min: [*]const f64, n_times: usize, epoch_offsets_min: ?[*]const f64,
    threshold_km: f64, out_pairs: [*]u32, out_t_index: [*]u32, max_results: usize, n_found: *usize) i32;

pub extern "c" fn azh_parse_tle_text(text: [*]const u8, len: usize, out16: [*]f64, max_records: usize, n_found: *usize) i32;
pub extern "c" fn azh_parse_omm_json(text: [*]const u8, len: usize, out16: [*]f64, max_records: usize, n_found: *usize) i32;
pub extern "c" fn azh_set_parse_threads(n: i32) void;
pub extern "c" fn azh_constellation_from_omm_json(text: [*]const u8, len: usize, grav: i32, device: i32, out: *?*Handle) i32;
pub extern "c" fn azh_constellation_subset(h: ?*const Handle, indices: [*]const u32, n: usize, device: i32, out: *?*Handle) i32;

pub extern "c" fn azh_propagate_device_window(h: ?*Handle, row_lo: usize, row_hi: usize, d_pos: [*]f64, d_vel: ?[*]f64, layout: i32,
    out_stride_sats: usize, d_err: ?[*]u8, stream: ?*anyopaque) i32;
pub extern "c" fn azh_set_f32_mode(h: ?*Handle, mode: i32) i32;
pub extern "c" fn azh_set_f32_arithmetic(h: ?*Handle, enabled: i32) i32;
pub extern "c" fn azh_set_fast_path(h: ?*Handle, enabled: i32) i32;
pub extern "c" fn azh_set_tile_kernel(h: ?*Handle, enabled: i32) i32;
pub extern "c" fn azh_set_graphs(h: ?*Handle, enabled: i32) i32;
pub extern "c" fn azh_set_host_points(n: usize) void;
pub extern "c" fn azh_get_host_points() usize;
pub extern "c" fn azh_set_host_copy_threads(n: i32) void;
pub extern "c" fn azh_host_alloc(bytes: usize, out: *?*anyopaque) i32;
pub extern "c" fn azh_host_free(p: ?*anyopaque) void;
pub extern "c" fn azh_host_pool_stats(live_bytes: ?*usize, free_bytes: ?*usize) void;
pub extern "c" fn azh_host_pool_trim() void;
pub extern "c" fn azh_last_path(h: ?*const Handle) u32;
pub extern "c" fn azh_last_one_stats(h: ?*Handle, n_segments: ?*u32, n_handed_over: ?*u32) i32;
pub extern "c" fn azh_propagate_one_device(h: ?*Handle, sat_index: usize, d_tsince_min: [*]const f64, n: usize, d_pos: [*]f64,
    d_vel: ?[*]f64, d_err: ?[*]u8, stream: ?*anyopaque) i32;
pub extern "c" fn azh_selftest_math(x: [*]const f64, n: usize, out6n: [*]f64, device: i32) i32;
pub extern "c" fn azh_selftest_host_step(el: [*]const f64, n_pad: usize, sat: usize, flags: u32, grav: i32, tsince_min: [*]const f64, n: usize,
    out6n: [*]f64, err: ?[*]u8) i32;
pub extern "c" fn azh_selftest_coords(op: i32, in: *const [4]f64, out: *[5]f64) i32;

pub extern "c" fn coords_julian_to_gmst(jd: f64) f64;
pub extern "c" fn coords_eci_to_ecef(eci: *const [3]f64, gmst: f64, ecef: *[3]f64) void;
pub extern "c" fn coords_ecef_to_geodetic(ecef: *const [3]f64, lla: *[3]f64) void;
pub extern "c" fn azh_coords_topocentric(r_teme: *const [3]f64, v_teme: ?*const [3]f64, gmst: f64, observer_lla: *const [3]f64,
    aer: *[3]f64, aer_rate: ?*[3]f64) void;

pub const OUT_TOPOCENTRIC: i32 = 3;
pub const Pass = extern struct {
    t_rise_min: f64,
    t_culm_min: f64,
    t_set_min: f64,
    max_elevation_rad: f64,
    rise_azimuth_rad: f64,
    set_azimuth_rad: f64,
    flags: u32,
    grid_rise: u32,
    grid_culm: u32,
    grid_set: u32,
};
pub const PASS_UP_AT_START: u32 = 1;
pub const PASS_UP_AT_END: u32 = 2;
pub const PASS_CUT_BY_ERROR: u32 = 4;
pub extern "c" fn azh_set_observer(h: ?*Handle, lat_deg: f64, lon_deg: f64, alt_km: f64) i32;
pub extern "c" fn azh_find_passes_host(h: ?*Handle, times_min: [*]const f64, n_times: usize, epoch_offsets_min: ?[*]const f64,
    reference_jd: f64, min_elevation_deg: f64, out: [*]Pass, max_passes: usize, n_passes: [*]u32) i32;
pub extern "c" fn azh_find_passes_device(h: ?*Handle, times_min: [*]const f64, n_times: usize, epoch_offsets_min: ?[*]const f64,
    reference_jd: f64, min_elevation_deg: f64, d_out: [*]Pass, max_passes: usize, d_n_passes: [*]u32, stream: ?*anyopaque) i32;
pub extern "c" fn azh_find_passes_stations_host(h: ?*Handle, times_min: [*]const f64, n_times: usize,
    epoch_offsets_min: ?[*]const f64, reference_jd: f64, stations_lla: [*]const [3]f64, min_elevation_deg: [*]const f64,
    n_stations: usize, out: [*]Pass, max_passes: usize, n_passes: [*]u32) i32;
pub extern "c" fn azh_find_passes_stations_device(h: ?*Handle, times_min: [*]const f64, n_times: usize,
    epoch_offsets_min: ?[*]const f64, reference_jd: f64, stations_lla: [*]const [3]f64, min_elevation_deg: [*]const f64,
    n_stations: usize, d_out: [*]Pass, max_passes: usize, d_n_passes: [*]u32, stream: ?*anyopaque) i32;

pub const Coverage = extern struct {
    mean_in_view: f64,
    max_gap_min: f64,
    n_covered: u32,
    min_in_view: u32,
    max_in_view: u32,
    n_gaps: u32,
    grid_gap_start: u32,
    grid_gap_end: u32,
    flags: u32,
    reserved: u32,
};
pub const COVERAGE_GAP_AT_START: u32 = 1;
pub const COVERAGE_GAP_AT_END: u32 = 2;
pub extern "c" fn azh_coverage_host(h: ?*Handle, times_min: [*]const f64, n_times: usize, epoch_offsets_min: ?[*]const f64,
    reference_jd: f64, points_lla: [*]const [3]f64, min_elevation_deg: [*]const f64, n_points: usize, min_satellites: u32,
    stats: [*]Coverage, counts_or_null: ?[*]u32) i32;
pub extern "c" fn azh_coverage_device(h: ?*Handle, times_min: [*]const f64, n_times: usize, epoch_offsets_min: ?[*]const f64,
    reference_jd: f64, points_lla: [*]const [3]f64, min_elevation_deg: [*]const f64, n_points: usize, min_satellites: u32,
    d_stats: [*]Coverage, d_counts_or_null: ?[*]u32, stream: ?*anyopaque) i32;

pub extern "c" fn azh_sun_position_teme(jd: f64, sun_km: *[3]f64) void;
pub extern "c" fn azh_selftest_sun(jd: [*]const f64, n: usize, out3n: [*]f64, device: i32) i32;
pub extern "c" fn azh_shadow_state(r_teme: *const [3]f64, sun_km: *const [3]f64, f_umbra: ?*f64, f_penumbra: ?*f64) i32;
pub const Eclipse = extern struct {
    t_entry_min: f64,
    t_exit_min: f64,
    flags: u32,
    grid_entry: u32,
    grid_exit: u32,
    reserved: u32,
};
pub const ECLIPSE_IN_AT_START: u32 = 1;
pub const ECLIPSE_IN_AT_END: u32 = 2;
pub const ECLIPSE_CUT_BY_ERROR: u32 = 4;
pub const SHADOW_UMBRA: i32 = 0;
pub const SHADOW_PENUMBRA: i32 = 1;
pub extern "c" fn azh_find_eclipses_host(h: ?*Handle, times_min: [*]const f64, n_times: usize, epoch_offsets_min: ?[*]const f64,
    reference_jd: f64, kind: i32, out: ?[*]Eclipse, max_eclipses: usize, n_eclipses: [*]u32, state_or_null: ?[*]u8) i32;
pub extern "c" fn azh_find_eclipses_device(h: ?*Handle, times_min: [*]const f64, n_times: usize, epoch_offsets_min: ?[*]const f64,
    reference_jd: f64, kind: i32, d_out: ?[*]Eclipse, max_eclipses: usize, d_n_eclipses: [*]u32, d_state_or_null: ?[*]u8,
    stream: ?*anyopaque) i32;

pub extern "c" fn azh_line_of_sight(r1: *const [3]f64, r2: *const [3]f64, grazing_alt_km: f64, clearance_km: ?*f64, range_km: ?*f64) i32;
pub const Access = extern struct {
    t_start_min: f64,
    t_end_min: f64,
    min_range_km: f64,
    flags: u32,
    grid_start: u32,
    grid_end: u32,
    grid_min_range: u32,
};
pub const ACCESS_OPEN_AT_START: u32 = 1;
pub const ACCESS_OPEN_AT_END: u32 = 2;
pub const ACCESS_CUT_BY_ERROR: u32 = 4;
pub const NO_TARGET: usize = ~@as(usize, 0);
pub extern "c" fn azh_find_access_host(h: ?*Handle, times_min: [*]const f64, n_times: usize, epoch_offsets_min: ?[*]const f64,
    target_index: usize, grazing_alt_km: f64, max_range_km: f64, out: ?[*]Access, max_windows: usize, n_windows: [*]u32,
    state_or_null: ?[*]u8) i32;
pub extern "c" fn azh_find_access_device(h: ?*Handle, times_min: [*]const f64, n_times: usize, epoch_offsets_min: ?[*]const f64,
    target_index: usize, grazing_alt_km: f64, max_range_km: f64, d_out: ?[*]Access, max_windows: usize, d_n_windows: [*]u32,
    d_state_or_null: ?[*]u8, stream: ?*anyopaque) i32;
pub extern "c" fn azh_find_access_track_device(h: ?*Handle, times_min: [*]const f64, n_times: usize, epoch_offsets_min: ?[*]const f64,
    d_track_pos: [*]const f64, d_track_vel: [*]const f64, exclude_index: usize, grazing_alt_km: f64, max_range_km: f64,
    d_out: ?[*]Access, max_windows: usize, d_n_windows: [*]u32, d_state_or_null: ?[*]u8, stream: ?*anyopaque) i32;

pub extern "c" fn azh_closest_approach(d0: *const [3]f64, w0: *const [3]f64, d1: *const [3]f64, w1: *const [3]f64, dt_min: f64,
    sigma: ?*f64, miss_km: ?*f64, rel_speed_km_s: ?*f64) i32;
pub const Conjunction = extern struct {
    t_tca_min: f64,
    miss_km: f64,
    rel_speed_km_s: f64,
    target: u32,
    sat: u32,
    grid_index: u32,
    reserved: u32,
};
pub extern "c" fn azh_find_conjunctions_host(h: ?*Handle, times_min: [*]const f64, n_times: usize, epoch_offsets_min: ?[*]const f64,
    targets: [*]const usize, n_targets: usize, threshold_km: f64, out: ?[*]Conjunction, max_events: usize, n_events: *u32) i32;
pub extern "c" fn azh_find_conjunctions_device(h: ?*Handle, times_min: [*]const f64, n_times: usize, epoch_offsets_min: ?[*]const f64,
    targets: [*]const usize, n_targets: usize, threshold_km: f64, d_out: ?[*]Conjunction, max_events: usize, d_n_events: *u32,
    stream: ?*anyopaque) i32;

pub const Group = opaque {};
pub extern "c" fn azh_group_create_from_tle_text(text: [*]const u8, len: usize, grav: i32, devices: [*]const i32, n_devices: i32,
    n_chunks: i32, out: *?*Group) i32;
pub extern "c" fn azh_group_create_from_omm_json(text: [*]const u8, len: usize, grav: i32, devices: [*]const i32, n_devices: i32,
    n_chunks: i32, out: *?*Group) i32;
pub extern "c" fn azh_group_free(g: ?*Group) void;
pub extern "c" fn azh_group_num_satellites(g: ?*const Group) usize;
pub extern "c" fn azh_group_num_devices(g: ?*const Group) i32;
pub extern "c" fn azh_group_padded_rows(g: ?*const Group) usize;
pub extern "c" fn azh_group_get_epochs(g: ?*const Group, out: [*]f64) i32;
pub extern "c" fn azh_group_propagate_host(g: ?*Group, times_min: [*]const f64, n_times: usize, epoch_offsets_min: ?[*]const f64,
    n_offsets: usize, pos: [*]f64, vel: ?[*]f64, output_mode: i32, reference_jd: f64, err: ?[*]u8) i32;
pub extern "c" fn azh_group_propagate_allgather(g: ?*Group, times_min: [*]const f64, n_times: usize,
    epoch_offsets_min: ?[*]const f64, n_offsets: usize, d_pos: [*]const [*]f64, d_vel: ?[*]const [*]f64) i32;
pub extern "c" fn azh_group_screen_target_host(g: ?*Group, times_min: [*]const f64, n_times: usize, epoch_offsets_min: ?[*]const f64,
    n_offsets: usize, target_index: usize, threshold_km: f64, reference_jd: f64, min_dist_km: [*]f64, min_t_index: [*]u32) i32;
pub extern "c" fn azh_group_screen_target_device(g: ?*Group, times_min: [*]const f64, n_times: usize, epoch_offsets_min: ?[*]const f64,
    n_offsets: usize, target_index: usize, threshold_km: f64, reference_jd: f64, d_min_dist_km: [*]const [*]f64, d_min_t_index: [*]const [*]u32) i32;
pub extern "c" fn azh_group_shard_size(g: ?*const Group, device_slot: i32) usize;
pub extern "c" fn azh_group_shard_rows(g: ?*const Group, device_slot: i32, out_rows: [*]u32) i32;
pub extern "c" fn azh_group_synchronize(g: ?*Group) i32;
```

include/astroz_hip.h:

```cpp
#ifndef ASTROZ_HIP_H
#define ASTROZ_HIP_H

#include <stddef.h>
#include <stdint.h>

#ifdef __cplusplus
extern "C" {
#endif

enum {
    AZ_OK = 0,
    AZ_ERR_BAD_TLE_LENGTH = -1,
    AZ_ERR_BAD_CHECKSUM = -2,
    AZ_ERR_DEEP_SPACE_NOT_SUPPORTED = -10,
    AZ_ERR_INVALID_ECCENTRICITY = -11,
    AZ_ERR_SATELLITE_DECAYED = -12,
    AZ_ERR_VALUE = -20,
    AZ_ERR_ALLOC_FAILED = -100,
    AZ_ERR_NULL_POINTER = -101,
    AZ_ERR_NOT_INITIALIZED = -102,
    AZ_ERR_HIP = -200,
    AZ_ERR_UNKNOWN = -999
};

// ... 132 lines not shown
int32_t azh_coverage_host(azh_constellation *c, const double *times_min, size_t n_times, const double *epoch_offsets_min,
                          double reference_jd, const double *points_lla, const double *min_elevation_deg, size_t n_points,
                          uint32_t min_satellites, azh_coverage *stats, uint32_t *counts_or_null);
int32_t azh_coverage_device(azh_constellation *c, const double *times_min, size_t n_times, const double *epoch_offsets_min,
                            double reference_jd, const double *points_lla, const double *min_elevation_deg, size_t n_points,
                            uint32_t min_satellites, azh_coverage *d_stats, uint32_t *d_counts_or_null, void *stream);

void azh_sun_position_teme(double jd, double sun_km[3]);
int32_t azh_selftest_sun(const double *jd, size_t n, double *out3n, int32_t device);

int32_t azh_shadow_state(const double r_teme[3], const double sun_km[3], double *f_umbra, double *f_penumbra);

typedef struct azh_eclipse {
    double t_entry_min, t_exit_min;
    uint32_t flags;
    uint32_t grid_entry, grid_exit;
    uint32_t reserved;
} azh_eclipse;
#define AZH_ECLIPSE_IN_AT_START 1u
#define AZH_ECLIPSE_IN_AT_END 2u
#define AZH_ECLIPSE_CUT_BY_ERROR 4u
enum { AZH_SHADOW_UMBRA = 0, AZH_SHADOW_PENUMBRA = 1 };
int32_t azh_find_eclipses_host(azh_constellation *c, const double *times_min, size_t n_times, const double *epoch_offsets_min,
                               double reference_jd, int32_t kind, azh_eclipse *out, size_t max_eclipses, uint32_t *n_eclipses,
                               uint8_t *state_or_null);
int32_t azh_find_eclipses_device(azh_constellation *c, const double *times_min, size_t n_times, const double *epoch_offsets_min,
                                 double reference_jd, int32_t kind, azh_eclipse *d_out, size_t max_eclipses,
                                 uint32_t *d_n_eclipses, uint8_t *d_state_or_null, void *stream);

int32_t azh_line_of_sight(const double r1[3], const double r2[3], double grazing_alt_km, double *clearance_km, double *range_km);

typedef struct azh_access {
    double t_start_min, t_end_min;
    double min_range_km;
    uint32_t flags;
    uint32_t grid_start, grid_end, grid_min_range;
} azh_access;
#define AZH_ACCESS_OPEN_AT_START 1u
#define AZH_ACCESS_OPEN_AT_END 2u
#define AZH_ACCESS_CUT_BY_ERROR 4u
int32_t azh_find_access_host(azh_constellation *c, const double *times_min, size_t n_times, const double *epoch_offsets_min,
                             size_t target_index, double grazing_alt_km, double max_range_km, azh_access *out, size_t max_windows,
                             uint32_t *n_windows, uint8_t *state_or_null);
int32_t azh_find_access_device(azh_constellation *c, const double *times_min, size_t n_times, const double *epoch_offsets_min,
                               size_t target_index, double grazing_alt_km, double max_range_km, azh_access *d_out,
                               size_t max_windows, uint32_t *d_n_windows, uint8_t *d_state_or_null, void *stream);
int32_t azh_find_access_track_device(azh_constellation *c, const double *times_min, size_t n_times, const double *epoch_offsets_min,
                                     const double *d_track_pos, const double *d_track_vel, size_t exclude_index,
                                     double grazing_alt_km, double max_range_km, azh_access *d_out, size_t max_windows,
                                     uint32_t *d_n_windows, uint8_t *d_state_or_null, void *stream);

int32_t azh_closest_approach(const double d0[3], const double w0[3], const double d1[3], const double w1[3], double dt_min,
                             double *sigma, double *miss_km, double *rel_speed_km_s);

typedef struct azh_conjunction {
    double t_tca_min, miss_km, rel_speed_km_s;
    uint32_t target;
    uint32_t sat;
    uint32_t grid_index;
    uint32_t reserved;
} azh_conjunction;
int32_t azh_find_conjunctions_host(azh_constellation *c, const double *times_min, size_t n_times, const double *epoch_offsets_min,
                                   const size_t *targets, size_t n_targets, double threshold_km, azh_conjunction *out,
                                   size_t max_events, uint32_t *n_events);
int32_t azh_find_conjunctions_device(azh_constellation *c, const double *times_min, size_t n_times, const double *epoch_offsets_min,
                                     const size_t *targets, size_t n_targets, double threshold_km, azh_conjunction *d_out,
                                     size_t max_events, uint32_t *d_n_events, void *stream);

int32_t azh_screen_target_host(azh_constellation *c, const double *times_min, size_t n_times,
                               const double *epoch_offsets_min, size_t target_index, double threshold_km,
                               double reference_jd, double *min_dist_km, uint32_t *min_t_index);
int32_t azh_screen_target_device(azh_constellation *c, const double *times_min, size_t n_times,
                                 const double *epoch_offsets_min, size_t target_index, double threshold_km,
                                 double reference_jd, double *d_min_dist_km, uint32_t *d_min_t_index, void *stream);

int32_t azh_screen_track_device(azh_constellation *c, const double *times_min, size_t n_times,
                                const double *epoch_offsets_min, const double *d_track, size_t exclude_index,
                                double threshold_km, double *d_min_dist_km, uint32_t *d_min_t_index, void *stream);

int32_t azh_coarse_screen_device(const double *d_pos, size_t n_sats, size_t n_times, int32_t layout,
                                 size_t stride_sats, double threshold_km, const uint8_t *valid_mask,
                                 uint32_t *out_pairs, uint32_t *out_t_index, size_t max_results, size_t *n_found,
                                 void *stream);
int32_t azh_coarse_screen_host(const double *pos, size_t n_sats, size_t n_times, int32_t layout, size_t stride_sats,
                               double threshold_km, const uint8_t *valid_mask, uint32_t *out_pairs,
                               uint32_t *out_t_index, size_t max_results, size_t *n_found, int32_t device);
int32_t azh_screen_all_host(azh_constellation *c, const double *times_min, size_t n_times,
                            const double *epoch_offsets_min, double threshold_km, uint32_t *out_pairs,
                            uint32_t *out_t_index, size_t max_results, size_t *n_found);

typedef struct azh_group azh_group;
int32_t azh_group_create_from_tle_text(const char *text, size_t len, int32_t grav, const int32_t *devices,
                                       int32_t n_devices, int32_t n_chunks, azh_group **out);
int32_t azh_group_create_from_omm_json(const char *text, size_t len, int32_t grav, const int32_t *devices,
                                       int32_t n_devices, int32_t n_chunks, azh_group **out);
void azh_group_free(azh_group *g);
size_t azh_group_num_satellites(const azh_group *g);
int32_t azh_group_num_devices(const azh_group *g);
size_t azh_group_padded_rows(const azh_group *g);
int32_t azh_group_get_epochs(const azh_group *g, double *out_n);
int32_t azh_group_propagate_host(azh_group *g, const double *times_min, size_t n_times, const double *epoch_offsets_min,
                                 size_t n_offsets, double *pos, double *vel, int32_t output_mode, double reference_jd,
                                 uint8_t *err);
int32_t azh_group_propagate_allgather(azh_group *g, const double *times_min, size_t n_times,
                                      const double *epoch_offsets_min, size_t n_offsets, double *const *d_pos,
                                      double *const *d_vel);

int32_t azh_group_screen_target_host(azh_group *g, const double *times_min, size_t n_times, const double *epoch_offsets_min,
                                     size_t n_offsets, size_t target_index, double threshold_km, double reference_jd,
                                     double *min_dist_km, uint32_t *min_t_index);
int32_t azh_group_screen_target_device(azh_group *g, const double *times_min, size_t n_times, const double *epoch_offsets_min,
                                       size_t n_offsets, size_t target_index, double threshold_km, double reference_jd,
                                       double *const *d_min_dist_km, uint32_t *const *d_min_t_index);
size_t azh_group_shard_size(const azh_group *g, int32_t device_slot);
int32_t azh_group_shard_rows(const azh_group *g, int32_t device_slot, uint32_t *out_rows);
int32_t azh_group_synchronize(azh_group *g);

int32_t azh_propagate_jd_host(azh_constellation *c, const double *jd, const double *fr, size_t n_times,
                              double *pos, double *vel, int32_t output_mode, int32_t layout, uint8_t *err);
int32_t azh_synchronize(azh_constellation *c);

int32_t azh_propagate_one_host(azh_constellation *c, size_t sat_index, const double *tsince_min, size_t n,
                               double *pos, double *vel, uint8_t *err);

int32_t azh_propagate_one_device(azh_constellation *c, size_t sat_index, const double *d_tsince_min, size_t n,
                                 double *d_pos, double *d_vel, uint8_t *d_err, void *stream);
int32_t azh_selftest_math(const double *x, size_t n, double *out6n, int32_t device);
int32_t azh_selftest_coords(int32_t op, const double in[4], double out[5]);
int32_t azh_selftest_host_step(const double *el, size_t n_pad, size_t sat, uint32_t flags, int32_t grav, const double *tsince_min,
                               size_t n, double *out6n, uint8_t *err);

int32_t azh_set_time_tile(azh_constellation *c, uint32_t sgp4_tile, uint32_t sdp4_tile);
int32_t azh_set_fast_path(azh_constellation *c, int32_t enabled);
int32_t azh_set_tile_kernel(azh_constellation *c, int32_t enabled);
int32_t azh_set_graphs(azh_constellation *c, int32_t enabled);
void azh_set_host_copy_threads(int32_t n);
void azh_set_host_points(size_t n);
size_t azh_get_host_points(void);
int32_t azh_host_alloc(size_t bytes, void **out);
void azh_host_free(void *p);
void azh_host_pool_stats(size_t *live_bytes, size_t *free_bytes);
void azh_host_pool_trim(void);
int32_t azh_set_timing(azh_constellation *c, int32_t enabled);
double azh_last_kernel_ms(azh_constellation *c);
#define AZH_PATH_ROWS_FAST 1u
#define AZH_PATH_TILES_FAST 2u
#define AZH_PATH_ROWS_GENERIC 4u
#define AZH_PATH_LANE_SAT 8u
#define AZH_PATH_DEEP_ROWS 16u
#define AZH_PATH_COLS_FAST 64u
#define AZH_PATH_QUASI_UNIFORM 32u
#define AZH_PATH_HOST_STEP 128u
uint32_t azh_last_path(const azh_constellation *c);
int32_t azh_last_one_stats(azh_constellation *c, uint32_t *n_segments, uint32_t *n_handed_over);

#ifdef __cplusplus
}
#endif
#endif
```

Measured before the change: 94.83 billion.

## Freeze redo-pass item counts from async snapshot to skip or right-size redo launches

After a fast-path launch, the redo counter and item list are copied asynchronously to pinned host memory. Later calls poll the copy and freeze the number of redo items, so the redo kernel can be skipped when no items exist, skipped per window when no redo row falls in the range, and launched with a grid sized to the actual item count. The ecc side stream fork is also skipped when it would have nothing to do. The redo kernel variant gets a smaller LDS time buffer and a higher waves-per-EU launch bound to raise occupancy. The frozen count is used in the graph signature, and the risk is stale counts if the redo set changes between calls without a plan reset.

```diff
diff --git a/astroz_amd/_native.py b/astroz_amd/_native.py
--- a/astroz_amd/_native.py
+++ b/astroz_amd/_native.py
@@ -42,7 +42,7 @@
     "azh_num_satellites", "azh_num_sgp4", "azh_num_sdp4", "azh_get_epochs", "azh_get_status",
     "azh_get_field", "azh_propagate_host", "azh_propagate_device", "azh_propagate_device_cached", "azh_propagate_device_window",
     "azh_propagate_jd_host", "azh_synchronize", "azh_propagate_one_host", "azh_set_time_tile", "azh_set_timing", "azh_set_fast_path", "azh_set_tile_kernel", "azh_set_graphs", "azh_set_f32_arithmetic", "azh_set_f32_mode",
-    "azh_last_kernel_ms", "azh_last_path", "azh_last_one_stats", "azh_set_host_copy_threads", "azh_set_host_points", "azh_get_host_points", "azh_selftest_coords", "azh_selftest_host_step", "azh_host_alloc", "azh_host_free", "azh_host_pool_stats", "azh_host_pool_trim", "azh_propagate_device_f32", "azh_propagate_device_cached_f32",
+    "azh_last_kernel_ms", "azh_last_path", "azh_last_redo_items", "azh_last_one_stats", "azh_set_host_copy_threads", "azh_set_host_points", "azh_get_host_points", "azh_selftest_coords", "azh_selftest_host_step", "azh_host_alloc", "azh_host_free", "azh_host_pool_stats", "azh_host_pool_trim", "azh_propagate_device_f32", "azh_propagate_device_cached_f32",
     "azh_screen_target_host", "azh_screen_target_device", "azh_coarse_screen_device", "azh_coarse_screen_host",
     "azh_screen_all_host", "azh_constellation_from_omm_json", "azh_propagate_one_device", "azh_selftest_math",
     "azh_parse_tle_text", "azh_parse_omm_json", "azh_set_parse_threads", "coords_julian_to_gmst",
@@ -248,6 +248,8 @@
     L.azh_host_pool_trim.restype = None
     L.azh_last_path.argtypes = [vp]
     L.azh_last_path.restype = u32
+    L.azh_last_redo_items.argtypes = [vp, vp]
+    L.azh_last_redo_items.restype = C.c_int32
     L.azh_last_one_stats.argtypes = [vp, vp, vp]
     L.azh_last_one_stats.restype = C.c_int32
     L.azh_propagate_device_f32.argtypes = L.azh_propagate_device.argtypes
@@ -686,6 +688,11 @@
     def last_path(self):
         return int(lib().azh_last_path(self._h))
 
+    def last_redo_items(self):
+        launched = C.c_int32(0)
+        n = int(lib().azh_last_redo_items(self._h, C.byref(launched)))
+        return n, bool(launched.value)
+
     def last_one_stats(self):
         a, b = C.c_uint32(0), C.c_uint32(0)
         check(lib().azh_last_one_stats(self._h, C.byref(a), C.byref(b)), "azh_last_one_stats")
diff --git a/astroz_amd/csrc/astroz_hip.hip b/astroz_amd/csrc/astroz_hip.hip
--- a/astroz_amd/csrc/astroz_hip.hip
+++ b/astroz_amd/csrc/astroz_hip.hip
@@ -196,7 +196,20 @@
         DevBuf<double> win;
         DevBuf<unsigned char> flag;
         DevBuf<unsigned> redo;
+        unsigned list_off = 0;
+        int frozen_items = -1;
+        bool rows_known = false;
+        std::vector<unsigned> item_rows;
+        unsigned gen = 0;
+        struct Snap {
+            PinnedBuf buf;
+            Event ev;
+            bool pending = false;
+            unsigned gen = 0;
+        } snap[2];
     } plan[4];
+    int last_redo_items = -1;
+    bool last_redo_launched = false;
     DevBuf<double> d_inc;
     DevBuf<double> d_fast_rec;
     double uniform_step = 0.0;
@@ -267,6 +280,8 @@
         unsigned fails;
         hipGraph_t graph;
         hipGraphExec_t exec;
+        int redo_items = -1;
+        bool redo_launched = false;
     };
     std::vector<LaunchGraph> graphs;
     int graphs_on = 0;
@@ -315,6 +330,7 @@
 }
 
 void drop_graphs(azh_constellation *c);
+void plan_unfreeze(azh_constellation::FastPlan &pl);
 
 int32_t build(const std::vector<double> (&cols)[AZ_NUM_RAW], size_t n, int grav, int device, azh_constellation **out)
 {
@@ -614,7 +630,12 @@
     hipLaunchKernelGGL((k_rows<VEL, gen_frame(FRAME), SINK, true>), grid, dim3(64), 0, st, a);
 }
 
-int32_t launch_near_fast(const PropArgs &a, bool vel, const FastShape &shape, dim3 rgrid, hipStream_t st, const EccSide &side)
+struct RedoPass {
+    dim3 grid;
+    bool launch = true;
+};
+
+int32_t launch_near_fast(const PropArgs &a, bool vel, const FastShape &shape, const RedoPass &redo, hipStream_t st, const EccSide &side)
 {
     PropArgs e = ecc_part(a, shape.tile_e), c = a;
     c.n_list = a.n_circ;
@@ -626,13 +647,13 @@
         if (c.slot_hi == 0) c.n_list = n_c = 0;
         if (e.slot_hi == 0) e.n_list = n_e = 0;
     }
-    const bool beside = side.stream != nullptr && n_c;
+    const bool beside = side.stream != nullptr && n_c && (n_e || redo.launch);
     const hipStream_t se = beside ? side.stream : st;
     if (beside)
         if (int32_t rc = stream_after(se, st, side.fork); rc != AZ_OK) return rc;
     with_outputs(a, vel, [&](auto VEL, auto FRAME, auto SINK) {
         if (n_e) launch_rows_fast<VEL, FRAME, SINK, true>(e, n_e, se);
-        launch_redo<VEL, FRAME, SINK>(a, rgrid, se);
+        if (redo.launch) launch_redo<VEL, FRAME, SINK>(a, redo.grid, se);
         if (n_c && FRAME == 0 && shape.packed32)
             with_bool(shape.mixed32, [&](auto MIXED) {
                 with_bool(a.delta != nullptr, [&](auto DELTA) {
@@ -645,7 +666,7 @@
     return beside ? stream_after(st, se, side.join) : AZ_OK;
 }
 
-void launch_tiles(const PropArgs &a0, bool vel, hipStream_t st, const FastShape &shape)
+void launch_tiles(const PropArgs &a0, bool vel, hipStream_t st, const FastShape &shape, const RedoPass &redo)
 {
     PropArgs a = a0, r = a0;
     a.tile = r.tile = shape.tile_c;
@@ -655,7 +676,7 @@
         with_bool(a.delta64 != nullptr, [&](auto WIDE) {
             hipLaunchKernelGGL((k_tiles_fast<VEL, FRAME, WIDE ? 2 : 0>), grid, dim3(1024), 0, st, a);
         });
-        launch_redo<VEL, FRAME, AZ_SINK_F64>(r, dim3(256, 4), st);
+        if (redo.launch) launch_redo<VEL, FRAME, AZ_SINK_F64>(r, redo.grid, st);
     });
 }
 unsigned cols_tile(unsigned n_rows, unsigned n_times, unsigned forced, double step)
@@ -678,7 +699,7 @@
     f.kind = 3;
     return f;
 }
-int32_t launch_cols(const PropArgs &a0, bool vel, hipStream_t st, const FastShape &shape, const EccSide &side, unsigned ecc_row0)
+int32_t launch_cols(const PropArgs &a0, bool vel, hipStream_t st, const FastShape &shape, const RedoPass &redo, const EccSide &side, unsigned ecc_row0)
 {
     PropArgs a = a0;
     PropArgs e = ecc_part(a, shape.tile_e);
@@ -703,7 +724,7 @@
         with_bool(a.delta64 != nullptr, [&](auto WIDE) {
             hipLaunchKernelGGL((k_cols_fast<VEL, FRAME, WIDE ? 2 : 0>), grid, dim3(64), 0, st, a);
         });
-        launch_redo<VEL, FRAME, AZ_SINK_F64>(r, dim3(256, 4), st);
+        if (redo.launch) launch_redo<VEL, FRAME, AZ_SINK_F64>(r, redo.grid, st);
     });
     return AZ_OK;
 }
@@ -772,7 +793,10 @@
     c->cached_mode = mode;
     c->seeds_valid = false;
     drop_graphs(c);
-    for (auto &pl : c->plan) pl.valid = false;
+    for (auto &pl : c->plan) {
+        pl.valid = false;
+        plan_unfreeze(pl);
+    }
     c->uniform_step = 0.0;
     c->delta_max = 0.0;
     c->delta_wide = false;
@@ -880,11 +904,95 @@
     return AZ_OK;
 }
 
+constexpr unsigned kSnapItems = 1024;
+
+void plan_unfreeze(azh_constellation::FastPlan &pl)
+{
+    pl.frozen_items = -1;
+    pl.rows_known = false;
+    pl.item_rows.clear();
+    pl.gen += 1;
+}
+
+void plan_poll(const azh_constellation *c, azh_constellation::FastPlan &pl)
+{
+    for (auto &sn : pl.snap) {
+        if (!sn.pending) continue;
+        if (hipEventQuery(sn.ev) != hipSuccess) {
+            (void)hipGetLastError();
+            continue;
+        }
+        sn.pending = false;
+        if (sn.gen != pl.gen || !pl.valid || pl.frozen_items >= 0) continue;
+        const unsigned *h = static_cast<const unsigned *>(sn.buf.p);
+        const unsigned n_static = h[2], total = std::max(h[0], h[1]);
+        if (total < n_static || total > 0x7fffffffu) continue;
+        try {
+            pl.item_rows.clear();
+            pl.rows_known = total <= kSnapItems && 4 + 3 * (size_t)total <= pl.redo.cap;
+            if (pl.rows_known) {
+                for (unsigned k = 0; k < total; ++k) {
+                    const unsigned slot = h[4 + 3 * (size_t)k];
+                    if (slot >= pl.n_list) { pl.rows_known = false; break; }
+                    pl.item_rows.push_back(c->h_list[pl.list_off + slot]);
+                }
+                std::sort(pl.item_rows.begin(), pl.item_rows.end());
+            }
+        } catch (const std::bad_alloc &) {
+            pl.rows_known = false;
+        }
+        pl.frozen_items = (int)total;
+    }
+}
+
+int32_t plan_snapshot(azh_constellation *c, azh_constellation::FastPlan &pl, hipStream_t st)
+{
+    if (c->capturing || !pl.valid || pl.frozen_items >= 0) return AZ_OK;
+    for (auto &sn : pl.snap) {
+        if (sn.pending) continue;
+        const size_t words = std::min<size_t>(pl.redo.cap, 4 + 3 * (size_t)kSnapItems);
+        if (sn.buf.ensure(words * sizeof(unsigned)) != AZ_OK) return AZ_ERR_HIP;
+        if (!sn.ev && !hip_ok(sn.ev.create(hipEventDisableTiming), "hipEventCreate")) return AZ_ERR_HIP;
+        HIP_TRY(hipMemcpyAsync(sn.buf.p, pl.redo.p, words * sizeof(unsigned), hipMemcpyDeviceToHost, st));
+        HIP_TRY(hipEventRecord(sn.ev, st));
+        sn.pending = true;
+        sn.gen = pl.gen;
+        break;
+    }
+    return AZ_OK;
+}
+
+unsigned redo_split(const FastShape &shape)
+{
+    return std::min(16u, std::max(1u, (std::max(shape.tile_c, shape.tile_e) + 63u) / 64u));
+}
+
+RedoPass redo_pass(azh_constellation *c, azh_constellation::FastPlan &pl, dim3 conservative, bool windowed, size_t row_lo, size_t row_hi,
+                   unsigned split = 4)
+{
+    RedoPass r;
+    r.grid = conservative;
+    if (pl.frozen_items >= 0) {
+        const unsigned n = (unsigned)pl.frozen_items;
+        r.launch = n > 0;
+        if (r.launch && windowed && pl.rows_known) {
+            const auto it = std::lower_bound(pl.item_rows.begin(), pl.item_rows.end(), (unsigned)std::min<size_t>(row_lo, 0xffffffffu));
+            r.launch = it != pl.item_rows.end() && *it < row_hi;
+        }
+        r.grid = dim3(std::min(8192u, std::max(n, 1u)), std::max(split, 1u));
+    }
+    c->last_redo_items = pl.frozen_items;
+    c->last_redo_launched = r.launch;
+    if (r.launch) pl.parity ^= 1u;
+    return r;
+}
+
 int32_t ensure_plan(azh_constellation *c, PropArgs &a, const FastShape &shape, hipStream_t st)
 {
     azh_constellation::FastPlan &pl = c->plan[shape.kind];
     const unsigned n_list = a.n_list;
     const unsigned n_seg = (a.n_times + std::min(shape.tile_c, shape.tile_e) - 1) / std::min(shape.tile_c, shape.tile_e);
+    if (!c->capturing) plan_poll(c, pl);
     if (!pl.valid || pl.tile_c != shape.tile_c || pl.tile_e != shape.tile_e || pl.n_list != n_list || pl.mixed32 != shape.mixed32) {
         if (c->capturing) return AZ_RC_EAGER;
         drop_graphs(c);
@@ -908,6 +1016,8 @@
         hipLaunchKernelGGL(k_plan_arm, dim3(1), dim3(64), 0, st, q.redo_static, q.redo_c0, q.redo_c1);
         HIP_TRY(hipGetLastError());
         pl.valid = true;
+        plan_unfreeze(pl);
+        pl.list_off = (unsigned)(a.list - c->d_list.p);
         pl.tile_c = shape.tile_c; pl.tile_e = shape.tile_e; pl.n_list = n_list; pl.n_seg = n_seg; pl.parity = 0; pl.mixed32 = shape.mixed32;
     }
     a.plan_win = pl.win.p;
@@ -917,12 +1027,12 @@
     a.redo_count = pl.redo.p + pl.parity;
     a.redo_next = pl.redo.p + (pl.parity ^ 1u);
     a.redo_items = pl.redo.p + 4;
-    pl.parity ^= 1u;
     return AZ_OK;
 }
 
 void drop_graphs(azh_constellation *c)
 {
+    for (auto &pl : c->plan) plan_unfreeze(pl);
     if (c->graphs.empty()) return;
     if (hipEventSynchronize(c->ev_graph) != hipSuccess) (void)hipGetLastError();
     for (auto &g : c->graphs) {
@@ -943,7 +1053,7 @@
 unsigned plan_sig(const azh_constellation *c)
 {
     unsigned s = 0;
-    for (unsigned k = 0; k < 4; ++k) s |= (c->plan[k].parity & 1u) << k;
+    for (unsigned k = 0; k < 4; ++k) s |= ((c->plan[k].parity & 1u) << k) | ((c->plan[k].frozen_items >= 0 ? 1u : 0u) << (4 + k));
     return s;
 }
 
@@ -1009,6 +1119,10 @@
     }
 
     unsigned path = 0;
+    c->last_redo_items = -1;
+    c->last_redo_launched = false;
+    azh_constellation::FastPlan *used_plan = nullptr;
+    bool snap_full = !windowed;
     if (c->timing) HIP_TRY(hipEventRecord(c->ev_t0, st));
     if (d_err) HIP_TRY(hipMemsetAsync(d_err + row_lo * (size_t)n_times, 0, (row_hi - row_lo) * (size_t)n_times, st));
     const bool tiles = c->n_sgp4 > 0 && c->tile_kernel && a.inc != nullptr && layout == AZ_LAYOUT_TIME_MAJOR && !f32 &&
@@ -1080,18 +1194,22 @@
             shape = cols ? fast_shape_cols(a, (unsigned)c->n, c->n_sgp4, c->n_circ)
                          : (tiles ? fast_shape_tiles(a, (unsigned)c->n) : fast_shape_rows(a, c->n_sgp4, c->n_circ));
             if (int32_t rc = ensure_plan(c, a, shape, st); rc != AZ_OK) return rc;
+            used_plan = &c->plan[shape.kind];
         }
         const EccSide side{c->s_ecc, c->ev_fork2, c->ev_join2};
         if (a.n_list > 0 && cols) {
-            if (int32_t rc = launch_cols(a, d_vel != nullptr, st, shape, side, c->n_sdp4); rc != AZ_OK) return rc;
+            const RedoPass redo = redo_pass(c, *used_plan, dim3(256, 4), windowed, row_lo, row_hi, redo_split(shape));
+            if (int32_t rc = launch_cols(a, d_vel != nullptr, st, shape, redo, side, c->n_sdp4); rc != AZ_OK) return rc;
             path |= AZH_PATH_COLS_FAST;
         } else if (a.n_list > 0 && tiles) {
-            launch_tiles(a, d_vel != nullptr, st, shape);
+            launch_tiles(a, d_vel != nullptr, st, shape, redo_pass(c, *used_plan, dim3(256, 4), windowed, row_lo, row_hi, redo_split(shape)));
             path |= AZH_PATH_TILES_FAST;
         } else if (a.n_list > 0 && fast) {
             const dim3 rgrid(std::min(8192u, std::max(256u, (a.n_list * cgrid_y(a.n_times, shape.tile_c) + 63u) / 64u)), 4);
-            if (int32_t rc = launch_near_fast(a, d_vel != nullptr, shape, rgrid, st, side); rc != AZ_OK) return rc;
+            const RedoPass redo = redo_pass(c, *used_plan, rgrid, windowed, row_lo, row_hi, redo_split(shape));
+            if (int32_t rc = launch_near_fast(a, d_vel != nullptr, shape, redo, st, side); rc != AZ_OK) return rc;
             path |= AZH_PATH_ROWS_FAST;
+            snap_full = !windowed || (a.win_ecc_lo == 0 && a.win_ecc_hi >= n_ecc);
         } else if (a.n_list > 0) {
             path |= launch_propagate(a, layout, d_vel != nullptr, false, st);
         }
@@ -1110,6 +1228,8 @@
         HIP_TRY(hipEventRecord(c->ev_t1, st));
         c->timed = true;
     }
+    if (used_plan && snap_full)
+        if (int32_t rc = plan_snapshot(c, *used_plan, st); rc != AZ_OK) return rc;
     return AZ_OK;
 }
 
@@ -1117,6 +1237,7 @@
                       int f32 = 0, size_t row_lo = 0, size_t row_hi = ~(size_t)0)
 {
     if (!c->graphs_on || c->timing || c->cached_n_times == 0 || !c->s_main.owned()) return launch_all(c, d_pos, d_vel, layout, stride, d_err, st, f32, row_lo, row_hi);
+    for (auto &pl : c->plan) plan_poll(c, pl);
     const unsigned sig = plan_sig(c);
     azh_constellation::LaunchGraph *hit = nullptr, *pending = nullptr;
     for (auto &g : c->graphs)
@@ -1130,6 +1251,8 @@
         HIP_TRY(hipGraphLaunch(hit->exec, st));
         for (unsigned k = 0; k < 4; ++k) c->plan[k].parity = (hit->sig_after >> k) & 1u;
         c->last_path = hit->path;
+        c->last_redo_items = hit->redo_items;
+        c->last_redo_launched = hit->redo_launched;
         HIP_TRY(hipEventRecord(c->ev_graph, st));
         return AZ_OK;
     }
@@ -1168,6 +1291,8 @@
     pending->exec = exec;
     pending->sig_after = plan_sig(c);
     pending->path = c->last_path;
+    pending->redo_items = c->last_redo_items;
+    pending->redo_launched = c->last_redo_launched;
     HIP_TRY(hipGraphLaunch(exec, st));
     HIP_TRY(hipEventRecord(c->ev_graph, st));
     return AZ_OK;
@@ -1979,7 +2104,10 @@
         }
         if (c->n_sgp4 > 0) {
             if (fast_screen) {
-                if ((rc = launch_near_fast(near, false, shape, dim3(256, 4), st, EccSide{c->s_ecc, c->ev_fork2, c->ev_join2})) != AZ_OK) return rc;
+                azh_constellation::FastPlan &pl = c->plan[shape.kind];
+                const RedoPass redo = redo_pass(c, pl, dim3(256, 4), false, 0, c->n);
+                if ((rc = launch_near_fast(near, false, shape, redo, st, EccSide{c->s_ecc, c->ev_fork2, c->ev_join2})) != AZ_OK) return rc;
+                if ((rc = plan_snapshot(c, pl, st)) != AZ_OK) return rc;
                 c->last_path = AZH_PATH_ROWS_FAST | ((near.delta || near.delta64) ? AZH_PATH_QUASI_UNIFORM : 0u);
             } else {
                 c->last_path = launch_propagate(near, AZ_LAYOUT_SAT_MAJOR, false, false, st);
@@ -3065,6 +3193,12 @@
 }
 
 uint32_t azh_last_path(const azh_constellation *c) { return c ? c->last_path : 0u; }
+
+int32_t azh_last_redo_items(const azh_constellation *c, int32_t *launched)
+{
+    if (launched) *launched = c && c->last_redo_launched ? 1 : 0;
+    return c ? c->last_redo_items : -1;
+}
 
 int32_t azh_last_one_stats(azh_constellation *c, uint32_t *n_segments, uint32_t *n_handed_over)
 {
diff --git a/astroz_amd/csrc/kernels.h b/astroz_amd/csrc/kernels.h
--- a/astroz_amd/csrc/kernels.h
+++ b/astroz_amd/csrc/kernels.h
@@ -19,6 +19,9 @@
 #endif
 #ifndef AZ_ROWS_WAVES
 #define AZ_ROWS_WAVES 3
+#endif
+#ifndef AZ_REDO_WAVES
+#define AZ_REDO_WAVES 6
 #endif
 #ifndef AZ_DEEP_WAVES
 #define AZ_DEEP_WAVES 2
@@ -1277,11 +1280,12 @@
 }
 
 template <bool VEL, int FRAME, int SINK, bool REDO = false>
-__global__ void __launch_bounds__(64, AZ_ROWS_WAVES) k_rows(PropArgs p)
+__global__ void __launch_bounds__(64, REDO ? AZ_REDO_WAVES : AZ_ROWS_WAVES) k_rows(PropArgs p)
 {
     typedef typename std::conditional<SINK == AZ_SINK_F32, float, double>::type out_t;
     const unsigned lane = threadIdx.x;
-    __shared__ __attribute__((aligned(16))) double rows_lds[AZ_ROWS_TLDS + C_NUM_MAX + 2 + 8];
+    constexpr unsigned TLDS = REDO ? 256u : (unsigned)AZ_ROWS_TLDS;
+    __shared__ __attribute__((aligned(16))) double rows_lds[TLDS + C_NUM_MAX + 2 + 8];
     static_assert(F_nodeo < 8 && F_argpo < 8 && F_mo < 8, "the epoch angles sit in the first eight rows of the element table");
     constexpr bool redo = REDO;
     const unsigned n_items = redo ? *p.redo_count : 1u;
@@ -1318,14 +1322,14 @@
     az_wave_lds_fence();
     Sgp4Lane e;
     typedef ColdBroadcast ColdT;
-    const ColdT cold{rows_lds + AZ_ROWS_TLDS};
+    const ColdT cold{rows_lds + TLDS};
     az_load_sgp4(p.el, p.n_pad, s, fl, e, cold);
     e.mdot = az_uniform(e.mdot); e.argpdot = az_uniform(e.argpdot); e.nodedot = az_uniform(e.nodedot);
     e.xnodcf = az_uniform(e.xnodcf); e.aycof = az_uniform(e.aycof); e.xlcof = az_uniform(e.xlcof);
     e.sinio = az_uniform(e.sinio); e.cosio = az_uniform(e.cosio); e.k_mrt = az_uniform(e.k_mrt);
     e.k_c2u = az_uniform(e.k_c2u); e.k_su = az_uniform(e.k_su); e.k_node = az_uniform(e.k_node);
     e.k_inc = az_uniform(e.k_inc); e.x1mth2 = az_uniform(e.x1mth2); e.k_rv = az_uniform(e.k_rv);
-    double *seed_lds = rows_lds + AZ_ROWS_TLDS + C_NUM_MAX + 2;
+    double *seed_lds = rows_lds + TLDS + C_NUM_MAX + 2;
     if (lane < 8) seed_lds[lane] = p.el[(size_t)lane * p.n_pad + s];
     az_wave_lds_fence();
     Sgp4Carry c;
@@ -1339,11 +1343,11 @@
     for (unsigned base = t_lo; base < t_hi; base += 64) {
         const unsigned i = base + lane;
         const bool live = i < t_hi;
-        const unsigned kk = (base - t_lo) & (AZ_ROWS_TLDS - 1u);
+        const unsigned kk = (base - t_lo) & (TLDS - 1u);
         if (kk == 0) {
             az_wave_lds_fence();
 #pragma unroll
-            for (unsigned j = 0; j < AZ_ROWS_TLDS; j += 64) rows_lds[j + lane] = p.times[min(i + j, t_hi - 1)];
+            for (unsigned j = 0; j < TLDS; j += 64) rows_lds[j + lane] = p.times[min(i + j, t_hi - 1)];
             az_wave_lds_fence();
         }
         const double t = rows_lds[kk + lane] + off;
diff --git a/bindings/zig/astroz_hip.zig b/bindings/zig/astroz_hip.zig
--- a/bindings/zig/astroz_hip.zig
+++ b/bindings/zig/astroz_hip.zig
@@ -112,6 +112,7 @@
 pub extern "c" fn azh_host_pool_stats(live_bytes: ?*usize, free_bytes: ?*usize) void;
 pub extern "c" fn azh_host_pool_trim() void;
 pub extern "c" fn azh_last_path(h: ?*const Handle) u32;
+pub extern "c" fn azh_last_redo_items(h: ?*const Handle, launched: ?*i32) i32;
 pub extern "c" fn azh_last_one_stats(h: ?*Handle, n_segments: ?*u32, n_handed_over: ?*u32) i32;
 pub extern "c" fn azh_propagate_one_device(h: ?*Handle, sat_index: usize, d_tsince_min: [*]const f64, n: usize, d_pos: [*]f64,
     d_vel: ?[*]f64, d_err: ?[*]u8, stream: ?*anyopaque) i32;
diff --git a/include/astroz_hip.h b/include/astroz_hip.h
--- a/include/astroz_hip.h
+++ b/include/astroz_hip.h
@@ -308,6 +308,7 @@
 #define AZH_PATH_QUASI_UNIFORM 32u
 #define AZH_PATH_HOST_STEP 128u
 uint32_t azh_last_path(const azh_constellation *c);
+int32_t azh_last_redo_items(const azh_constellation *c, int32_t *launched);
 int32_t azh_last_one_stats(azh_constellation *c, uint32_t *n_segments, uint32_t *n_handed_over);
 
 #ifdef __cplusplus
```

Measured after the change: 95.62 billion (median of 6 runs). About the same (+0.8%).
